# fferflo/semantic-meshes

Measured on AMD Instinct MI355X. Metric: views/sec fused (1080p, 19 classes, 1M-tri mesh), higher is better.
Workload: dtype f32; 1 GPU; cfg2: 1000000-triangle grid mesh, 11763 views/GPU at 1920x1080, 19 classes, probs resident in HBM; views_per_call=8, group_pipeline=True, repeats=1, allreduce=none, exchange=allreduce, nranks=1, allreduce_bytes=0, exchange_parts=1, held_views=0

## Files before the change

semantic_meshes_amd/_lib.py:

```python
import ctypes
import os
import threading

_HERE = os.path.dirname(os.path.abspath(__file__))
LIB_PATH = os.environ.get("SMESH_LIB_PATH") or os.path.join(_HERE, "csrc", "libsmesh_hip.so")

OK, ERR_INVALID, ERR_RUNTIME, ERR_NODEVICE = 0, 1, 2, 3
MEM_HOST, MEM_DEVICE = 0, 1
IDX_U32, IDX_I32, IDX_U64, IDX_I64 = 0, 1, 2, 3
AGG_KINDS = {"Sum": 0, "Summax": 1, "Mul": 2}
PROF_FUSE_SCATTER, PROF_FUSE_HIST, PROF_RASTER, PROF_FINALIZE, PROF_EXCHANGE = 0, 1, 2, 3, 4

c_void_p, c_int, c_u64, c_u32, c_float = ctypes.c_void_p, ctypes.c_int, ctypes.c_uint64, ctypes.c_uint32, ctypes.c_float
P = ctypes.POINTER


class CameraPOD(ctypes.Structure):
    _fields_ = [
        ("rotation", ctypes.c_float * 9),
        ("translation", ctypes.c_float * 3),
        ("focal", ctypes.c_double * 2),
        ("principal", ctypes.c_double * 2),
        ("width", ctypes.c_uint64),
        ("height", ctypes.c_uint64),
    ]


SIGNATURES = {
    "smesh_backend": (ctypes.c_char_p, []),
    "smesh_last_error": (ctypes.c_char_p, []),
    "smesh_device_count": (c_int, [P(c_int)]),
    "smesh_synchronize": (c_int, [c_int]),
    "smesh_stream_wait": (c_int, [c_int, c_void_p]),
    "smesh_stream_release": (c_int, [c_int, c_void_p]),
    "smesh_stream_handle": (c_int, [c_int, P(c_void_p)]),
    "smesh_token_record": (c_int, [c_int, P(c_u64)]),
    "smesh_token_done": (c_int, [c_int, c_u64, P(c_int)]),
    "smesh_stream_mark": (c_int, [c_int, c_int]),
    "smesh_stream_mark_elapsed": (c_int, [c_int, c_int, c_int, P(ctypes.c_double)]),
    "smesh_renderer_create_triangles": (c_int, [c_void_p, c_u64, c_void_p, c_u64, c_int, P(c_void_p)]),
    "smesh_renderer_create_texels": (c_int, [c_void_p, c_u64, c_void_p, c_u64, c_void_p, c_u64, c_float, c_int, P(c_void_p)]),
    "smesh_renderer_destroy": (c_int, [c_void_p]),
    "smesh_renderer_num_primitives": (c_int, [c_void_p, P(c_u64)]),
    "smesh_renderer_texel_layout": (c_int, [c_void_p, c_void_p, c_void_p, c_void_p]),
    "smesh_renderer_render": (c_int, [c_void_p, P(CameraPOD), c_void_p, c_void_p]),
    "smesh_renderer_render_device": (c_int, [c_void_p, P(CameraPOD), P(c_void_p), P(c_void_p)]),
    "smesh_renderer_release_image": (c_int, [c_void_p, c_void_p, c_void_p]),
    "smesh_aggregator_create": (c_int, [c_u64, c_u32, c_int, c_float, c_int, P(c_void_p)]),
    "smesh_aggregator_destroy": (c_int, [c_void_p]),
    "smesh_aggregator_reset": (c_int, [c_void_p]),
    "smesh_aggregator_add": (c_int, [c_void_p, c_void_p, c_int, P(ctypes.c_int64), c_int,
                                     c_void_p, P(ctypes.c_int64), c_int,
                                     c_void_p, P(ctypes.c_int64), c_int, c_u64, c_u64]),
    "smesh_aggregator_add_async": (c_int, [c_void_p, c_void_p, c_int, P(ctypes.c_int64), c_int,
                                           c_void_p, P(ctypes.c_int64), c_int,
                                           c_void_p, P(ctypes.c_int64), c_int, c_u64, c_u64]),
    "smesh_aggregator_add_many": (c_int, [c_void_p, c_u64, P(c_void_p), c_int, P(ctypes.c_int64), c_int,
                                          P(c_void_p), P(ctypes.c_int64), c_int,
                                          P(c_void_p), P(ctypes.c_int64), c_int, c_u64, c_u64]),
    "smesh_aggregator_add_rendered": (c_int, [c_void_p, c_void_p, c_void_p,
                                              c_void_p, P(ctypes.c_int64), c_int,
                                              c_void_p, P(ctypes.c_int64), c_int, c_u64, c_u64]),
    "smesh_aggregator_get": (c_int, [c_void_p, c_void_p, c_int]),
    "smesh_aggregator_get_rows": (c_int, [c_void_p, c_u64, c_u64, c_void_p, c_int]),
    "smesh_aggregator_get_raw": (c_int, [c_void_p, c_void_p, c_int]),
    "smesh_aggregator_set_raw": (c_int, [c_void_p, c_void_p, c_int]),
    "smesh_aggregator_raw_pointer": (c_int, [c_void_p, P(c_void_p), P(c_u64)]),
    "smesh_aggregator_row_stride": (c_int, [c_void_p, P(c_u32)]),
    "smesh_comm_unique_id": (c_int, [c_void_p]),
    "smesh_comm_create": (c_int, [c_int, c_int, c_int, c_void_p, P(c_void_p)]),
    "smesh_comm_create_all": (c_int, [P(c_int), c_int, P(c_void_p)]),
    "smesh_comm_destroy": (c_int, [c_void_p]),
    "smesh_comm_rank": (c_int, [c_void_p, P(c_int), P(c_int)]),
    "smesh_allreduce": (c_int, [P(c_void_p), P(c_void_p), c_int]),
    "smesh_reduce_scatter": (c_int, [c_void_p, c_void_p, P(c_u64), P(c_u64)]),
    "smesh_fuse_views_begin": (c_int, [c_void_p, c_void_p, c_void_p, c_u64, P(c_void_p), P(c_void_p), c_int, c_int, P(c_u64), P(c_u64)]),
    "smesh_fuse_views_continue": (c_int, [c_void_p, c_void_p, c_int, P(c_u64), P(c_u64)]),
    "smesh_allreduce_rows": (c_int, [c_void_p, c_void_p, c_u64, c_u64]),
    "smesh_exchange_join": (c_int, [c_void_p]),
    "smesh_aggregator_get_raw_rows": (c_int, [c_void_p, c_u64, c_u64, c_int, c_void_p, c_int]),
    "smesh_aggregator_set_raw_rows": (c_int, [c_void_p, c_u64, c_u64, c_int, c_void_p, c_int]),
    "smesh_comm_allreduce_f64": (c_int, [c_void_p, P(ctypes.c_double), c_int, c_int]),
    "smesh_aggregator_renderer": (c_int, [c_void_p, P(c_void_p)]),
    "smesh_annotation_renderer_render": (c_int, [c_void_p, c_void_p, c_int, P(ctypes.c_int64), c_int, c_void_p, c_void_p, c_int, c_u64, c_u64]),
    "smesh_annotation_renderer_destroy": (c_int, [c_void_p]),
    "smesh_fuse_view": (c_int, [c_void_p, c_void_p, P(CameraPOD), c_void_p, c_void_p, c_int]),
    "smesh_fuse_views": (c_int, [c_void_p, c_void_p, P(CameraPOD), c_u64, P(c_void_p), P(c_void_p), c_int]),
    "smesh_aggregator_add_matched": (c_int, [c_void_p, c_void_p, c_void_p, c_int, P(ctypes.c_int64), c_int,
                                             c_void_p, P(ctypes.c_int64), c_int,
                                             c_void_p, P(ctypes.c_int64), c_int, c_u64, c_u64, P(c_int)]),
    "smesh_renderer_seal_render": (c_int, [c_void_p, c_void_p]),
    "smesh_renderer_render_stats": (c_int, [c_void_p, c_void_p, c_void_p, c_void_p]),
    "smesh_box_extent_bound": (c_int, [c_void_p, c_u64, c_void_p, c_u64, c_void_p, c_void_p]),
    "smesh_last_fuse_kernel": (ctypes.c_char_p, []),
    "smesh_last_add_path": (ctypes.c_char_p, []),
    "smesh_profile_enable": (c_int, [c_int, c_int]),
    "smesh_profile_sample_every": (c_int, [c_int, ctypes.c_uint32]),
    "smesh_profile_read": (c_int, [c_int, c_int, P(ctypes.c_double), P(c_u64)]),
    "smesh_profile_read_ex": (c_int, [c_int, c_int, P(ctypes.c_double), P(c_u64), P(c_u64), P(c_u64)]),
    "smesh_profile_regions": (c_int, [c_int, c_int, P(c_u64)]),
    "smesh_profile_reset": (c_int, [c_int]),
    "smesh_synth_probs": (c_int, [c_void_p, c_u64, c_u32, c_u64, c_float, c_int, c_int]),
    "smesh_device_malloc": (c_int, [c_int, c_u64, P(c_void_p)]),
    "smesh_device_free": (c_int, [c_int, c_void_p]),
    "smesh_device_trim": (c_int, [c_int, P(c_u64)]),
    "smesh_set_option": (c_int, [ctypes.c_char_p, ctypes.c_int64]),
    "smesh_get_option": (c_int, [ctypes.c_char_p, P(ctypes.c_int64)]),
    "smesh_host_malloc": (c_int, [c_u64, P(c_void_p)]),
    "smesh_host_free": (c_int, [c_void_p]),
    "smesh_memcpy": (c_int, [c_void_p, c_void_p, c_u64, c_int, c_int, c_int]),
}

LBL_CODES = {"uint8": 0, "int8": 1, "uint16": 2, "int16": 3, "uint32": 4, "int32": 5, "uint64": 6, "int64": 7}

VTX_SUMS, VTX_ANNOTATIONS = 0, 1

EXT_SIGNATURES = {
    "smesh_fuse_view_labels": (c_int, [c_void_p, c_void_p, P(CameraPOD), c_void_p, c_int, P(ctypes.c_int64), c_void_p, c_int]),
    "smesh_fuse_views_labels": (c_int, [c_void_p, c_void_p, P(CameraPOD), c_u64, P(c_void_p), c_int, P(ctypes.c_int64), P(c_void_p), c_int]),
    "smesh_aggregator_add_labels": (c_int, [c_void_p, c_void_p, c_void_p, c_int, P(ctypes.c_int64), c_int,
                                            c_void_p, c_int, P(ctypes.c_int64), c_int,
                                            c_void_p, P(ctypes.c_int64), c_int, c_u64, c_u64]),
}

VERTEX_SIGNATURES = {
    "smesh_vertex_map_create": (c_int, [c_void_p, c_u64, c_u64, c_int, P(c_void_p)]),
    "smesh_vertex_map_destroy": (c_int, [c_void_p]),
    "smesh_vertex_map_size": (c_int, [c_void_p, P(c_u64), P(c_u64), P(c_u64)]),
    "smesh_vertex_map_adjacency": (c_int, [c_void_p, c_void_p, c_void_p]),
    "smesh_vertex_map_gather": (c_int, [c_void_p, c_void_p, c_int, c_u32, c_int, c_float, c_void_p, c_void_p, c_int]),
    "smesh_aggregator_vertex_annotations": (c_int, [c_void_p, c_void_p, c_int, c_float, c_void_p, c_void_p, c_int]),
    "smesh_renderer_texel_face_rows": (c_int, [c_void_p, c_void_p, c_int, c_u32, c_int, c_float, c_void_p, c_int]),
}

PROF_CONFUSION = 5
EVAL_SIGNATURES = {
    "smesh_confusion_create": (c_int, [c_u32, c_int, P(c_void_p)]),
    "smesh_confusion_destroy": (c_int, [c_void_p]),
    "smesh_confusion_reset": (c_int, [c_void_p]),
    "smesh_confusion_get": (c_int, [c_void_p, c_void_p, P(c_u64)]),
    "smesh_confusion_add_counts": (c_int, [c_void_p, c_void_p, c_u64]),
    "smesh_confusion_add_labels": (c_int, [c_void_p, c_void_p, c_int, c_void_p, c_int, c_int, c_u64]),
    "smesh_aggregator_labels": (c_int, [c_void_p, c_float, c_void_p, c_int]),
    "smesh_confusion_add_image": (c_int, [c_void_p, c_void_p, c_int, P(ctypes.c_int64), c_int, c_void_p, c_u64, c_int,
                                          c_void_p, c_int, P(ctypes.c_int64), c_int, c_u64, c_u64]),
    "smesh_confusion_add_view": (c_int, [c_void_p, c_void_p, P(CameraPOD), c_void_p, c_u64, c_void_p, c_int, P(ctypes.c_int64), c_int]),
    "smesh_confusion_add_views": (c_int, [c_void_p, c_void_p, P(CameraPOD), c_u64, c_void_p, c_u64, P(c_void_p), c_int,
                                          P(ctypes.c_int64), c_int]),
}

PROF_LABEL_IMAGES = 6
LAYOUT_WH, LAYOUT_HW = 0, 1
LABEL_IMAGE_SIGNATURES = {
    "smesh_label_renderer_create": (c_int, [c_void_p, c_u64, c_int, c_u32, c_int, c_u32, c_void_p, c_void_p, c_int, P(c_void_p)]),
    "smesh_label_renderer_destroy": (c_int, [c_void_p]),
    "smesh_label_renderer_render_image": (c_int, [c_void_p, c_void_p, c_int, P(ctypes.c_int64), c_int, c_u64, c_u64, c_int,
                                                  c_void_p, c_void_p, c_int]),
    "smesh_label_renderer_render_views": (c_int, [c_void_p, c_void_p, P(CameraPOD), c_u64, c_int, P(c_void_p), P(c_void_p), c_int]),
}

_lib = None
_lock = threading.Lock()


def _elf_dynamic_strings(path):
    import struct
    with open(path, "rb") as f:
        data = f.read()
    try:
        if data[:6] != b"\x7fELF\x02\x01":
            raise ValueError("not a little-endian ELF64 file")
        phoff, = struct.unpack_from("<Q", data, 0x20)
        phentsize, phnum = struct.unpack_from("<HH", data, 0x36)
        loads, dyn = [], None
        for k in range(phnum):
            typ, flags, off, vaddr, paddr, filesz, memsz, align = struct.unpack_from("<IIQQQQQQ", data, phoff + k * phentsize)
            if typ == 1:
                loads.append((vaddr, off, filesz))
            elif typ == 2:
                dyn = (off, filesz)
        if dyn is None:
            return None, []
        entries = []
        for e in range(dyn[0], dyn[0] + dyn[1], 16):
            tag, val = struct.unpack_from("<qQ", data, e)
            if tag == 0:
                break
            entries.append((tag, val))
        strtab = next((v for t, v in entries if t == 5), None)
        if strtab is None:
            return None, []
        stroff = next((off + strtab - vaddr for vaddr, off, filesz in loads if vaddr <= strtab < vaddr + filesz), None)
        if stroff is None:
            raise ValueError("DT_STRTAB outside every PT_LOAD segment")

        def cstr(o):
            end = data.index(b"\0", stroff + o)
            return data[stroff + o:end].decode()

        soname, needed = None, []
        for tag, val in entries:
            if tag == 1:
                needed.append(cstr(val))
            elif tag == 14:
                soname = cstr(val)
        return soname, needed
    except (struct.error, IndexError, UnicodeDecodeError) as e:
        raise ValueError("malformed ELF file %s: %s" % (path, e))


def _preload_note(msg):
    global PRELOAD_NOTE
    PRELOAD_NOTE = msg
    if os.environ.get("SMESH_DEBUG"):
        import sys
        print("semantic_meshes_amd: " + msg, file=sys.stderr)


PRELOAD_NOTE = None


def _preload_hip_runtime():
    import importlib.util
    import sys
    choice = os.environ.get("SMESH_HIP_RUNTIME", "auto")
    if choice == "system" or "torch" in sys.modules:
        return
    libdir = choice if choice not in ("auto", "torch") else None
    if libdir is None:
        try:
            spec = importlib.util.find_spec("torch")
        except (ImportError, ValueError):
            spec = None
        if spec is None or not spec.origin:
            return
        libdir = os.path.join(os.path.dirname(spec.origin), "lib")
    hip = os.path.join(libdir, "libamdhip64.so")
    if not os.path.exists(hip):
        return
    try:
        wanted = [n for n in _elf_dynamic_strings(LIB_PATH)[1] if n.startswith("libamdhip64.so")]
        offered = _elf_dynamic_strings(hip)[0]
    except (OSError, ValueError) as e:
        _preload_note("HIP runtime preload skipped: %s" % e)
        return
    if not wanted or offered != wanted[0]:
        _preload_note("HIP runtime preload skipped: %s offers SONAME %r, libsmesh_hip.so needs %r" % (hip, offered, wanted[:1]))
        return
    for name in ("libhsa-runtime64.so", "libamdhip64.so"):
        path = os.path.join(libdir, name)
        if os.path.exists(path):
            try:
                ctypes.CDLL(path, mode=ctypes.RTLD_GLOBAL)
            except OSError:
                return
    rccl = os.path.join(libdir, "librccl.so")
    if os.path.exists(rccl):
        os.environ.setdefault("SMESH_RCCL_LIB", rccl)


def lib():
    global _lib
    if _lib is None:
        with _lock:
            if _lib is None:
                if not os.path.exists(LIB_PATH):
                    raise RuntimeError(
                        "semantic_meshes_amd: %s not found -- build it with `make -C semantic_meshes_amd/csrc` "
                        "(or `python -c 'import __graft_entry__ as g; g.build()'`). There is no CPU fallback." % LIB_PATH)
                _preload_hip_runtime()
                L = ctypes.CDLL(LIB_PATH)
                for name, (res, args) in list(SIGNATURES.items()) + list(EXT_SIGNATURES.items()) + list(VERTEX_SIGNATURES.items()) + list(EVAL_SIGNATURES.items()) + list(LABEL_IMAGE_SIGNATURES.items()):
                    fn = getattr(L, name)
                    fn.restype = res
                    fn.argtypes = args
                _lib = L
    return _lib


def check(status):
    if status == OK:
        return
    msg = lib().smesh_last_error().decode(errors="replace")
    if status == ERR_INVALID:
        raise ValueError(msg)
    raise RuntimeError(msg)


def device_count():
    n = c_int(0)
    check(lib().smesh_device_count(ctypes.byref(n)))
    return n.value


_flush_hooks = []


def flush_pending(device=None):
    for hook in list(_flush_hooks):
        hook(device)


def last_fuse_kernel():
    flush_pending()
    return lib().smesh_last_fuse_kernel().decode()


def last_add_path():
    flush_pending()
    return lib().smesh_last_add_path().decode()


def synchronize(device=0):
    flush_pending(device)
    check(lib().smesh_synchronize(device))
```

semantic_meshes_amd/csrc/common.hpp:

```cpp
#pragma once

#include <hip/hip_runtime.h>

#include <cstdint>
#include <cstdio>
#include <cstdlib>
#include <functional>
#include <mutex>
#include <string>
#include <vector>

#include "../../include/smesh.h"

namespace smesh {

int fail(int code, const std::string& msg);
int fail_hip(hipError_t e, const char* what, const char* file, int line);

#define SMESH_HIP(expr)                                                         \
  do {                                                                          \
    hipError_t _e = (expr);                                                     \
    if (_e != hipSuccess) return ::smesh::fail_hip(_e, #expr, __FILE__, __LINE__); \
  } while (0)

#define SMESH_TRY(expr)              \
  do {                               \
    int _s = (expr);                 \
    if (_s != SMESH_OK) return _s;   \
  } while (0)

struct ProfSlot {
  std::vector<std::pair<hipEvent_t, hipEvent_t>> pending;
  std::vector<std::pair<hipEvent_t, hipEvent_t>> pool;
  double total_ms = 0.0;
  uint64_t launches = 0;
  uint64_t seen = 0;
  int depth = 0;
  bool open_timed = false;
  uint64_t timed_launches = 0;
  uint64_t timed_views = 0;
};

struct DeviceCtx {
  int device = -1;
  hipStream_t stream = nullptr;
  hipStream_t raster_stream = nullptr;
  hipStream_t exchange_stream = nullptr;
  hipEvent_t ev_order = nullptr;
  hipEvent_t ev_release = nullptr;
  int num_cus = 256;
  unsigned profiling = 0;
  unsigned profile_every = 1;
  ProfSlot slots[SMESH_PROF_SLOTS];
  hipEvent_t marks[SMESH_STREAM_MARKS] = {};
  std::vector<hipEvent_t> token_pool;
  std::recursive_mutex mu;
};

int get_ctx(int device, DeviceCtx** out);

struct ProfScope {
  DeviceCtx* ctx;
  int slot;
  hipEvent_t start = nullptr, stop = nullptr;
  hipStream_t st;
  bool counted = false;
  ProfScope(DeviceCtx* c, int s, hipStream_t stream = nullptr);
  ~ProfScope();
};

void prof_note(DeviceCtx* ctx, int slot, uint64_t launches, uint64_t views);

hipError_t dev_malloc(void** out, size_t bytes);
hipError_t dev_free(void* p, bool foreign = false);
uint64_t dev_cached_bytes(int device);
void dev_trim(int device);
void dev_cache_stats(uint64_t* live_blocks, uint64_t* cached_blocks, uint64_t* cached_bytes);

bool opt_group_pipeline();
bool opt_confusion_wave_aggregate();

constexpr uint32_t kConfusionLdsMaxC = 180;

struct Scratch {
  void* ptr = nullptr;
  size_t bytes = 0;
  int reserve(size_t need);
  void release();
};

inline uint64_t div_up(uint64_t a, uint64_t b) { return (a + b - 1) / b; }

inline int env_int(const char* name, int def) {
  const char* e = getenv(name);
  return e ? atoi(e) : def;
}

struct TriFrag {
  uint16_t x0, y0;
  uint16_t kind;
  uint16_t pad;
  unsigned long long mask;
};
static_assert(sizeof(TriFrag) == 16, "TriFrag must be 16 bytes");

struct TriFuseArgs {
  const TriFrag* frags;
  const uint32_t* idx;
  const float* probs;
  const float* weights;
  float* acc;
  float* acc_lo;
  uint64_t F;
  uint32_t C, W, H;
  float iew;
  const uint32_t* big_queue;
  const uint32_t* big_len;
  uint32_t big_capacity;
  uint32_t tri_blocks;
  uint32_t big_blocks;
  const uint32_t* prim_id;
  const uint32_t* tex_first;
  const uint32_t* tex_res;
  const uint8_t* tex_kinds;
  uint32_t* count;
  double* acc_d;
  int mid;
  uint32_t ps0, ps1;
  uint32_t blk_first;
  uint32_t f_lo, f_hi;
  uint32_t lds_pad;
};

struct TriView {
  const TriFrag* frags;
  const uint32_t* idx;
  const float* probs;
  const float* weights;
  const uint32_t* big_queue;
  const uint32_t* big_len;
  uint32_t W, H;
  uint32_t ps0, ps1;
  const uint8_t* kinds;
};
template <int NV>
struct TriViews {
  TriView v[NV];
};

struct RenderedView {
  const TriFrag* frags;
  const uint32_t* big_queue;
  const uint32_t* big_len;
  const uint32_t* idx;
  const float* probs;
  const float* weights;
  uint64_t W, H;
  int64_t ps0 = 0, ps1 = 0;
  bool mid_queue = false;
  bool no_big = false;
  const uint8_t* kinds = nullptr;
  bool fine = false;
  const void* labels = nullptr;
};

constexpr int kMidBox = 256;

struct ImageRecords {
  TriFrag* frags = nullptr;
  uint32_t* cand = nullptr;
  uint4* big4 = nullptr;
  uint32_t* big_queue = nullptr;
  uint32_t* big_count = nullptr;
  unsigned long long* mom = nullptr;
  uint64_t P = 0;
  bool clean = false;
  bool moments = false;
  uint32_t tag = 2;
  void release();
};
int image_records_build(DeviceCtx* ctx, ImageRecords& r, const uint32_t* d_idx, uint64_t W, uint64_t H, uint64_t P);
int image_records_pending(DeviceCtx* ctx, ImageRecords& r, const uint32_t* d_idx, uint64_t W, uint64_t H, hipStream_t st);
int image_records_scatter_sparse(DeviceCtx* ctx, ImageRecords& r, int kind, const uint32_t* d_idx, const float* d_probs, const float* d_w,
                                 uint64_t W, uint64_t H, uint32_t C, float iew, float* acc, float* acc_lo, double* acc_d, hipStream_t st);
int image_records_clear(DeviceCtx* ctx, ImageRecords& r, const uint32_t* d_idx, uint64_t W, uint64_t H, hipStream_t st);
bool image_records_build_group(DeviceCtx* ctx, ImageRecords* const* recs, const uint32_t* const* d_idx, int n, uint64_t W, uint64_t H, uint64_t P,
                               int* status);
int image_records_scatter_sparse_group(DeviceCtx* ctx, ImageRecords* const* recs, int n, int kind, const uint32_t* const* d_idx,
                                       const float* const* d_probs, const float* const* d_w, uint64_t W, uint64_t H, uint32_t C, float iew,
                                       float* acc, float* acc_lo, double* acc_d, hipStream_t st);

}

struct smesh_aggregator;
struct smesh_renderer;
int smesh_aggregator_with_final_rows(smesh_aggregator* a,
                                     const std::function<int(smesh::DeviceCtx* ctx, const float* rows, uint64_t P, uint32_t C)>& use);
int smesh_renderer_texel_tables(const smesh_renderer* r, smesh::DeviceCtx** ctx, uint64_t* F, uint64_t* P, const uint32_t** first,
                                const uint32_t** res);
int smesh_rows_labels(smesh::DeviceCtx* ctx, const float* d_rows, uint64_t n, uint32_t C, float dont_care_threshold, int32_t* out_labels,
                      int out_memkind);
int smesh_renderer_with_index_planes(smesh_renderer* r, const smesh_camera_t* cams, int n, uint64_t P, smesh::DeviceCtx* ctx,
                                     const std::function<int(int view, const uint32_t* idx, uint64_t W, uint64_t H)>& use);
```

semantic_meshes_amd/csrc/context.cpp:

```cpp
#include "common.hpp"
#include "labels_scratch.hpp"

#include <algorithm>
#include <atomic>

#include <cstdlib>
#include <cstring>
#include <map>
#include <memory>
#include <unordered_map>
#include <vector>

namespace smesh {

static thread_local std::string g_err;

int fail(int code, const std::string& msg) {
  g_err = msg;
  return code;
}

int fail_hip(hipError_t e, const char* what, const char* file, int line) {
  char buf[512];
  snprintf(buf, sizeof buf, "HIP error %d (%s) at %s:%d: %s", (int)e, hipGetErrorString(e), file, line, what);
  g_err = buf;
  (void)hipGetLastError();
  return (e == hipErrorNoDevice || e == hipErrorInvalidDevice) ? SMESH_ERR_NODEVICE : SMESH_ERR_RUNTIME;
}

static std::atomic<int> g_confusion_wave_aggregate{1};
bool opt_confusion_wave_aggregate() { return g_confusion_wave_aggregate.load() != 0; }

static std::atomic<int> g_group_pipeline{-1};
bool opt_group_pipeline() {
  int v = g_group_pipeline.load();
  if (v < 0) {
    const char* e = getenv("SMESH_GROUP_PIPELINE");
    v = e ? (atoi(e) != 0 ? 1 : 0) : 1;
    g_group_pipeline.store(v);
  }
  return v != 0;
}

static std::mutex g_ctx_mu;
static std::vector<std::unique_ptr<DeviceCtx>> g_ctx;

DeviceCtx* peek_ctx(int device) {
  std::lock_guard<std::mutex> lock(g_ctx_mu);
  return (device >= 0 && device < (int)g_ctx.size()) ? g_ctx[device].get() : nullptr;
}

int get_ctx(int device, DeviceCtx** out) {
  std::lock_guard<std::mutex> lock(g_ctx_mu);
  int n = 0;
  hipError_t e = hipGetDeviceCount(&n);
  if (e != hipSuccess || n <= 0) {
    (void)hipGetLastError();
    return fail(SMESH_ERR_NODEVICE, "no HIP device available (libsmesh_hip has no CPU fallback)");
  }
  if (device < 0 || device >= n) return fail(SMESH_ERR_INVALID, "device index out of range");
  if ((int)g_ctx.size() < n) g_ctx.resize(n);
  if (!g_ctx[device]) {
    SMESH_HIP(hipSetDevice(device));
    auto ctx = std::make_unique<DeviceCtx>();
    ctx->device = device;
    hipDeviceProp_t prop;
    SMESH_HIP(hipGetDeviceProperties(&prop, device));
    ctx->num_cus = prop.multiProcessorCount > 0 ? prop.multiProcessorCount : 256;
    SMESH_HIP(hipStreamCreateWithFlags(&ctx->stream, hipStreamNonBlocking));
    SMESH_HIP(hipStreamCreateWithFlags(&ctx->raster_stream, hipStreamNonBlocking));
    {
      int least = 0, greatest = 0;
      if (hipDeviceGetStreamPriorityRange(&least, &greatest) != hipSuccess) { (void)hipGetLastError(); least = greatest = 0; }
      if (hipStreamCreateWithPriority(&ctx->exchange_stream, hipStreamNonBlocking, greatest) != hipSuccess) {
        (void)hipGetLastError();
        SMESH_HIP(hipStreamCreateWithFlags(&ctx->exchange_stream, hipStreamNonBlocking));
      }
    }
    g_ctx[device] = std::move(ctx);
  }
  *out = g_ctx[device].get();
  return SMESH_OK;
}

ProfScope::ProfScope(DeviceCtx* c, int s, hipStream_t stream) : ctx(c), slot(s), st(stream ? stream : c->stream) {
  if (!(ctx->profiling & (1u << slot))) return;
  ProfSlot& ps = ctx->slots[slot];
  if (ps.depth++ > 0) { counted = true; return; }
  counted = true;
  if (ps.seen++ % (slot <= SMESH_PROF_RASTER ? std::max(1u, ctx->profile_every) : 1u) != 0) return;
  if (!ps.pool.empty()) {
    start = ps.pool.back().first;
    stop = ps.pool.back().second;
    ps.pool.pop_back();
  } else {
    if (hipEventCreate(&start) != hipSuccess || hipEventCreate(&stop) != hipSuccess) {
      start = stop = nullptr;
      return;
    }
  }
  (void)hipEventRecord(start, st);
  ps.open_timed = true;
}

void prof_note(DeviceCtx* ctx, int slot, uint64_t launches, uint64_t views) {
  ProfSlot& ps = ctx->slots[slot];
  if (ps.depth > 0 && ps.open_timed) { ps.timed_launches += launches; ps.timed_views += views; }
}

ProfScope::~ProfScope() {
  if (counted && --ctx->slots[slot].depth == 0 && !start) ctx->slots[slot].open_timed = false;
  if (!start) return;
  ctx->slots[slot].open_timed = false;
  (void)hipEventRecord(stop, st);
  ctx->slots[slot].pending.emplace_back(start, stop);
}

namespace {
struct DevBlock { int device; size_t bytes; };
struct CachedBlock { void* ptr; int device; unsigned long long stamp; };
std::mutex g_alloc_mu;
std::unordered_map<void*, DevBlock> g_live;
std::multimap<size_t, CachedBlock> g_cached;
std::map<int, size_t> g_cached_bytes;
unsigned long long g_alloc_stamp = 0;

size_t size_class(size_t n) {
  if (n == 0) n = 1;
  const size_t g = n <= (1u << 20) ? (size_t)4096 : (size_t)2 << 20;
  return (n + g - 1) / g * g;
}
size_t cache_cap(int device) {
  static std::map<int, size_t> caps;
  auto it = caps.find(device);
  if (it != caps.end()) return it->second;
  size_t cap;
  if (const char* e = getenv("SMESH_ALLOC_CACHE_MB")) cap = (size_t)std::max(0ll, atoll(e)) << 20;
  else {
    int cur = 0;
    (void)hipGetDevice(&cur);
    if (cur != device) (void)hipSetDevice(device);
    size_t free_b = 0, total = 0;
    if (hipMemGetInfo(&free_b, &total) != hipSuccess) { (void)hipGetLastError(); total = (size_t)64 << 30; }
    if (cur != device) (void)hipSetDevice(cur);
    cap = std::min<size_t>(total / 16, (size_t)8 << 30);
  }
  caps[device] = cap;
  return cap;
}
void really_free_locked(std::multimap<size_t, CachedBlock>::iterator it) {
  int cur = 0;
  (void)hipGetDevice(&cur);
  if (cur != it->second.device) (void)hipSetDevice(it->second.device);
  (void)hipFree(it->second.ptr);
  if (cur != it->second.device) (void)hipSetDevice(cur);
  g_cached_bytes[it->second.device] -= it->first;
  g_cached.erase(it);
}
void evict_locked(int device, size_t need, size_t cap) {
  for (;;) {
    size_t held = 0;
    if (device >= 0) held = g_cached_bytes[device];
    else for (auto& kv : g_cached_bytes) held += kv.second;
    if (held == 0 || held + need <= cap) return;
    auto oldest = g_cached.end();
    for (auto it = g_cached.begin(); it != g_cached.end(); ++it)
      if ((device < 0 || it->second.device == device) && (oldest == g_cached.end() || it->second.stamp < oldest->second.stamp)) oldest = it;
    if (oldest == g_cached.end()) return;
    really_free_locked(oldest);
  }
}
}

hipError_t dev_malloc(void** out, size_t bytes) {
  *out = nullptr;
  int dev = 0;
  hipError_t e = hipGetDevice(&dev);
  if (e != hipSuccess) return e;
  const size_t sz = size_class(bytes);
  std::lock_guard<std::mutex> lock(g_alloc_mu);
  for (auto it = g_cached.lower_bound(sz); it != g_cached.end() && it->first <= sz + sz / 8; ++it) {
    if (it->second.device != dev) continue;
    *out = it->second.ptr;
    g_live[*out] = DevBlock{dev, it->first};
    g_cached_bytes[dev] -= it->first;
    g_cached.erase(it);
    return hipSuccess;
  }
  e = hipMalloc(out, sz);
  if (e != hipSuccess) {
    (void)hipGetLastError();
    evict_locked(dev, 0, 0);
    e = hipMalloc(out, sz);
  }
  if (e == hipSuccess) g_live[*out] = DevBlock{dev, sz};
  return e;
}

hipError_t dev_free(void* p, bool foreign) {
  if (!p) return hipSuccess;
  int owner = -1;
  {
    std::lock_guard<std::mutex> lock(g_alloc_mu);
    auto it = g_live.find(p);
    if (it != g_live.end()) owner = it->second.device;
  }
  int cur = 0;
  (void)hipGetDevice(&cur);
  if (owner >= 0 && owner != cur) (void)hipSetDevice(owner);
  DeviceCtx* ctx = (owner >= 0 && !foreign) ? peek_ctx(owner) : nullptr;
  hipError_t e = hipSuccess;
  if (ctx) {
    for (hipStream_t st : {ctx->raster_stream, ctx->stream, ctx->exchange_stream})
      if (st && e == hipSuccess) e = hipStreamSynchronize(st);
  } else {
    e = hipDeviceSynchronize();
  }
  if (e != hipSuccess) (void)hipGetLastError();
  hipError_t ret = hipSuccess;
  {
    std::lock_guard<std::mutex> lock(g_alloc_mu);
    auto it = g_live.find(p);
    if (it == g_live.end()) ret = hipFree(p);
    else {
      const DevBlock b = it->second;
      g_live.erase(it);
      const size_t cap = cache_cap(b.device);
      if (b.bytes > cap) ret = hipFree(p);
      else {
        evict_locked(b.device, b.bytes, cap);
        g_cached.emplace(b.bytes, CachedBlock{p, b.device, g_alloc_stamp++});
        g_cached_bytes[b.device] += b.bytes;
      }
    }
  }
  if (owner >= 0 && owner != cur) (void)hipSetDevice(cur);
  return ret;
}

void dev_trim(int device) {
  std::lock_guard<std::mutex> lock(g_alloc_mu);
  for (auto it = g_cached.begin(); it != g_cached.end();) {
    if (device >= 0 && it->second.device != device) { ++it; continue; }
    auto victim = it++;
    really_free_locked(victim);
  }
}

void dev_cache_stats(uint64_t* live_blocks, uint64_t* cached_blocks, uint64_t* cached_bytes) {
  std::lock_guard<std::mutex> lock(g_alloc_mu);
  if (live_blocks) *live_blocks = g_live.size();
  if (cached_blocks) *cached_blocks = g_cached.size();
  if (cached_bytes) { *cached_bytes = 0; for (auto& kv : g_cached_bytes) *cached_bytes += kv.second; }
}
uint64_t dev_cached_bytes(int device) {
  std::lock_guard<std::mutex> lock(g_alloc_mu);
  uint64_t n = 0;
  for (auto& kv : g_cached_bytes) if (device < 0 || kv.first == device) n += kv.second;
  return n;
}

int Scratch::reserve(size_t need) {
  if (need <= bytes) return SMESH_OK;
  if (ptr) SMESH_HIP(dev_free(ptr));
  ptr = nullptr;
  bytes = 0;
  size_t want = need + need / 8 + 256;
  SMESH_HIP(dev_malloc(&ptr, want));
  bytes = want;
  return SMESH_OK;
}

void Scratch::release() {
  if (ptr) (void)dev_free(ptr);
  ptr = nullptr;
  bytes = 0;
}

}

using namespace smesh;

void smesh_last_fuse_instance(int* slot, int* views);

extern "C" {

const char* smesh_backend(void) { return "hip-gfx950"; }

const char* smesh_last_error(void) { return g_err.c_str(); }

int smesh_set_option(const char* name, int64_t value) {
  if (!name) return fail(SMESH_ERR_INVALID, "option name is NULL");
  if (!strcmp(name, "group_pipeline")) { g_group_pipeline.store(value != 0 ? 1 : 0); return SMESH_OK; }
  if (!strcmp(name, "confusion_wave_aggregate")) { g_confusion_wave_aggregate.store(value != 0 ? 1 : 0); return SMESH_OK; }
  return fail(SMESH_ERR_INVALID, std::string("unknown option: ") + name);
}
int smesh_get_option(const char* name, int64_t* value) {
  if (!name || !value) return fail(SMESH_ERR_INVALID, "NULL argument");
  if (!strcmp(name, "group_pipeline")) { *value = opt_group_pipeline() ? 1 : 0; return SMESH_OK; }
  if (!strcmp(name, "labels_lds_max_classes")) { *value = (int64_t)kLabelsLdsMaxC; return SMESH_OK; }
  if (!strcmp(name, "confusion_lds_max_classes")) { *value = (int64_t)kConfusionLdsMaxC; return SMESH_OK; }
  if (!strcmp(name, "confusion_wave_aggregate")) { *value = opt_confusion_wave_aggregate() ? 1 : 0; return SMESH_OK; }
  const bool want_slot = !strcmp(name, "last_fuse_slot");
  if (want_slot || !strcmp(name, "last_fuse_views")) {
    int slot, views;
    smesh_last_fuse_instance(&slot, &views);
    *value = want_slot ? slot : views;
    return SMESH_OK;
  }
  return fail(SMESH_ERR_INVALID, std::string("unknown option: ") + name);
}

int smesh_device_count(int* count) {
  if (!count) return fail(SMESH_ERR_INVALID, "count is NULL");
  int n = 0;
  if (hipGetDeviceCount(&n) != hipSuccess) {
    (void)hipGetLastError();
    n = 0;
  }
  *count = n;
  return SMESH_OK;
}

int smesh_synchronize(int device) {
  DeviceCtx* ctx;
  SMESH_TRY(get_ctx(device, &ctx));
  SMESH_HIP(hipSetDevice(device));
  SMESH_HIP(hipStreamSynchronize(ctx->raster_stream));
  SMESH_HIP(hipStreamSynchronize(ctx->stream));
  SMESH_HIP(hipStreamSynchronize(ctx->exchange_stream));
  return SMESH_OK;
}

int smesh_stream_wait(int device, void* producer_stream) {
  DeviceCtx* ctx;
  SMESH_TRY(get_ctx(device, &ctx));
  std::lock_guard<std::recursive_mutex> lock(ctx->mu);
  SMESH_HIP(hipSetDevice(device));
  hipStream_t ps = static_cast<hipStream_t>(producer_stream);
  if (ps == ctx->raster_stream) return SMESH_OK;
  if (!ctx->ev_order) SMESH_HIP(hipEventCreateWithFlags(&ctx->ev_order, hipEventDisableTiming));
  SMESH_HIP(hipEventRecord(ctx->ev_order, ps));
  if (ps != ctx->stream) SMESH_HIP(hipStreamWaitEvent(ctx->stream, ctx->ev_order, 0));
  SMESH_HIP(hipStreamWaitEvent(ctx->raster_stream, ctx->ev_order, 0));
  return SMESH_OK;
}

int smesh_stream_release(int device, void* consumer_stream) {
  DeviceCtx* ctx;
  SMESH_TRY(get_ctx(device, &ctx));
  std::lock_guard<std::recursive_mutex> lock(ctx->mu);
  SMESH_HIP(hipSetDevice(device));
  hipStream_t cs = static_cast<hipStream_t>(consumer_stream);
  if (cs == ctx->stream) return SMESH_OK;
  if (!ctx->ev_release) SMESH_HIP(hipEventCreateWithFlags(&ctx->ev_release, hipEventDisableTiming));
  SMESH_HIP(hipEventRecord(ctx->ev_release, ctx->stream));
  SMESH_HIP(hipStreamWaitEvent(cs, ctx->ev_release, 0));
  return SMESH_OK;
}

int smesh_stream_handle(int device, void** stream) {
  if (!stream) return fail(SMESH_ERR_INVALID, "stream is NULL");
  DeviceCtx* ctx;
  SMESH_TRY(get_ctx(device, &ctx));
  *stream = ctx->stream;
  return SMESH_OK;
}

int smesh_stream_mark(int device, int id) {
  if (id < 0 || id >= SMESH_STREAM_MARKS) return fail(SMESH_ERR_INVALID, "bad mark id");
  DeviceCtx* ctx;
  SMESH_TRY(get_ctx(device, &ctx));
  std::lock_guard<std::recursive_mutex> lock(ctx->mu);
  SMESH_HIP(hipSetDevice(device));
  if (!ctx->marks[id]) SMESH_HIP(hipEventCreate(&ctx->marks[id]));
  SMESH_HIP(hipEventRecord(ctx->marks[id], ctx->stream));
  return SMESH_OK;
}

int smesh_stream_mark_elapsed(int device, int from, int to, double* ms) {
  if (from < 0 || from >= SMESH_STREAM_MARKS || to < 0 || to >= SMESH_STREAM_MARKS || !ms) return fail(SMESH_ERR_INVALID, "bad mark id");
  DeviceCtx* ctx;
  SMESH_TRY(get_ctx(device, &ctx));
  hipEvent_t a, b;
  {
    std::lock_guard<std::recursive_mutex> lock(ctx->mu);
    a = ctx->marks[from];
    b = ctx->marks[to];
  }
  if (!a || !b) return fail(SMESH_ERR_INVALID, "mark was never recorded");
  SMESH_HIP(hipSetDevice(device));
  SMESH_HIP(hipEventSynchronize(b));
  float f = 0.f;
  SMESH_HIP(hipEventElapsedTime(&f, a, b));
  *ms = (double)f;
  return SMESH_OK;
}

int smesh_token_record(int device, uint64_t* token) {
  if (!token) return fail(SMESH_ERR_INVALID, "token is NULL");
  *token = 0;
  DeviceCtx* ctx;
  SMESH_TRY(get_ctx(device, &ctx));
  std::lock_guard<std::recursive_mutex> lock(ctx->mu);
  SMESH_HIP(hipSetDevice(device));
  hipEvent_t ev = nullptr;
  if (!ctx->token_pool.empty()) { ev = ctx->token_pool.back(); ctx->token_pool.pop_back(); }
  else SMESH_HIP(hipEventCreateWithFlags(&ev, hipEventDisableTiming));
  SMESH_HIP(hipEventRecord(ev, ctx->stream));
  *token = (uint64_t)reinterpret_cast<uintptr_t>(ev);
  return SMESH_OK;
}

int smesh_token_done(int device, uint64_t token, int* done) {
  if (!done) return fail(SMESH_ERR_INVALID, "done is NULL");
  *done = 1;
  if (!token) return SMESH_OK;
  DeviceCtx* ctx;
  SMESH_TRY(get_ctx(device, &ctx));
  std::lock_guard<std::recursive_mutex> lock(ctx->mu);
  hipEvent_t ev = reinterpret_cast<hipEvent_t>((uintptr_t)token);
  const hipError_t e = hipEventQuery(ev);
  if (e == hipErrorNotReady) { (void)hipGetLastError(); *done = 0; return SMESH_OK; }
  if (e != hipSuccess) return fail_hip(e, "hipEventQuery", __FILE__, __LINE__);
  ctx->token_pool.push_back(ev);
  return SMESH_OK;
}

int smesh_profile_enable(int device, int enabled) {
  DeviceCtx* ctx;
  SMESH_TRY(get_ctx(device, &ctx));
  std::lock_guard<std::recursive_mutex> lock(ctx->mu);
  ctx->profiling = enabled < 0 ? 0xFFu : (unsigned)enabled;
  return SMESH_OK;
}

int smesh_profile_sample_every(int device, uint32_t n) {
  DeviceCtx* ctx;
  SMESH_TRY(get_ctx(device, &ctx));
  std::lock_guard<std::recursive_mutex> lock(ctx->mu);
  ctx->profile_every = n ? n : 1u;
  return SMESH_OK;
}

static int drain(DeviceCtx* ctx) {
  SMESH_HIP(hipSetDevice(ctx->device));
  SMESH_HIP(hipStreamSynchronize(ctx->raster_stream));
  SMESH_HIP(hipStreamSynchronize(ctx->stream));
  SMESH_HIP(hipStreamSynchronize(ctx->exchange_stream));
  for (auto& ps : ctx->slots) {
    for (auto& ev : ps.pending) {
      float ms = 0.f;
      if (hipEventElapsedTime(&ms, ev.first, ev.second) == hipSuccess) {
        ps.total_ms += ms;
        ps.launches += 1;
      }
      ps.pool.push_back(ev);
    }
    ps.pending.clear();
  }
  return SMESH_OK;
}

int smesh_profile_read(int device, int slot, double* total_ms, uint64_t* launches) {
  if (slot < 0 || slot >= SMESH_PROF_SLOTS) return fail(SMESH_ERR_INVALID, "bad profile slot");
  DeviceCtx* ctx;
  SMESH_TRY(get_ctx(device, &ctx));
  std::lock_guard<std::recursive_mutex> lock(ctx->mu);
  SMESH_TRY(drain(ctx));
  if (total_ms) *total_ms = ctx->slots[slot].total_ms;
  if (launches) *launches = ctx->slots[slot].launches;
  return SMESH_OK;
}

int smesh_profile_read_ex(int device, int slot, double* total_ms, uint64_t* regions, uint64_t* launches, uint64_t* views) {
  if (slot < 0 || slot >= SMESH_PROF_SLOTS) return fail(SMESH_ERR_INVALID, "bad profile slot");
  DeviceCtx* ctx;
  SMESH_TRY(get_ctx(device, &ctx));
  std::lock_guard<std::recursive_mutex> lock(ctx->mu);
  SMESH_TRY(drain(ctx));
  const ProfSlot& ps = ctx->slots[slot];
  if (total_ms) *total_ms = ps.total_ms;
  if (regions) *regions = ps.launches;
  if (launches) *launches = ps.timed_launches;
  if (views) *views = ps.timed_views;
  return SMESH_OK;
}

int smesh_profile_regions(int device, int slot, uint64_t* entered) {
  if (slot < 0 || slot >= SMESH_PROF_SLOTS) return fail(SMESH_ERR_INVALID, "bad profile slot");
  DeviceCtx* ctx;
  SMESH_TRY(get_ctx(device, &ctx));
  std::lock_guard<std::recursive_mutex> lock(ctx->mu);
  if (entered) *entered = ctx->slots[slot].seen;
  return SMESH_OK;
}

int smesh_profile_reset(int device) {
  DeviceCtx* ctx;
  SMESH_TRY(get_ctx(device, &ctx));
  std::lock_guard<std::recursive_mutex> lock(ctx->mu);
  SMESH_TRY(drain(ctx));
  for (auto& ps : ctx->slots) {
    ps.total_ms = 0.0;
    ps.launches = 0;
    ps.seen = 0;
    ps.timed_launches = 0;
    ps.timed_views = 0;
  }
  return SMESH_OK;
}

int smesh_device_malloc(int device, uint64_t bytes, void** out) {
  if (!out) return fail(SMESH_ERR_INVALID, "out is NULL");
  DeviceCtx* ctx;
  SMESH_TRY(get_ctx(device, &ctx));
  SMESH_HIP(hipSetDevice(device));
  SMESH_HIP(dev_malloc(out, bytes ? bytes : 1));
  return SMESH_OK;
}

int smesh_device_free(int device, void* ptr) {
  if (!ptr) return SMESH_OK;
  DeviceCtx* ctx;
  SMESH_TRY(get_ctx(device, &ctx));
  SMESH_HIP(hipSetDevice(device));
  SMESH_HIP(dev_free(ptr, true));
  return SMESH_OK;
}

int smesh_device_trim(int device, uint64_t* cached_bytes) {
  if (cached_bytes) *cached_bytes = dev_cached_bytes(device);
  if (device >= 0) {
    DeviceCtx* ctx;
    SMESH_TRY(get_ctx(device, &ctx));
    SMESH_HIP(hipSetDevice(device));
  }
  (void)hipDeviceSynchronize();
  dev_trim(device);
  return SMESH_OK;
}

int smesh_host_malloc(uint64_t bytes, void** out) {
  if (!out) return fail(SMESH_ERR_INVALID, "out is NULL");
  DeviceCtx* ctx;
  SMESH_TRY(get_ctx(0, &ctx));
  SMESH_HIP(hipHostMalloc(out, bytes ? bytes : 1, hipHostMallocDefault));
  return SMESH_OK;
}

int smesh_host_free(void* ptr) {
  if (!ptr) return SMESH_OK;
  SMESH_HIP(hipHostFree(ptr));
  return SMESH_OK;
}

int smesh_memcpy(void* dst, const void* src, uint64_t bytes, int dst_memkind, int src_memkind, int device) {
  if (bytes == 0) return SMESH_OK;
  if (!dst || !src) return fail(SMESH_ERR_INVALID, "NULL pointer");
  if (dst_memkind == SMESH_MEM_HOST && src_memkind == SMESH_MEM_HOST) {
    memmove(dst, src, bytes);
    return SMESH_OK;
  }
  DeviceCtx* ctx;
  SMESH_TRY(get_ctx(device, &ctx));
  std::lock_guard<std::recursive_mutex> lock(ctx->mu);
  SMESH_HIP(hipSetDevice(device));
  hipMemcpyKind kind = dst_memkind == SMESH_MEM_HOST ? hipMemcpyDeviceToHost
                       : (src_memkind == SMESH_MEM_HOST ? hipMemcpyHostToDevice : hipMemcpyDeviceToDevice);
  SMESH_HIP(hipMemcpyAsync(dst, src, bytes, kind, ctx->stream));
  SMESH_HIP(hipStreamSynchronize(ctx->stream));
  return SMESH_OK;
}

}
```

semantic_meshes_amd/csrc/raster.hip:

```cpp
#include "common.hpp"

#include <algorithm>
#include <cmath>
#include <cstdlib>
#include <cstring>
#include <new>
#include <string>
#include <utility>
#include <vector>

#pragma clang fp contract(off)

using namespace smesh;

struct smesh_aggregator;
int smesh_aggregator_add_device_contig(smesh_aggregator* a, const uint32_t* d_idx, const float* d_probs,
                                       const float* d_w, uint64_t W, uint64_t H);
bool smesh_aggregator_can_fuse_triangles(smesh_aggregator* a, uint64_t F);
bool smesh_aggregator_can_fuse_pair(smesh_aggregator* a);
int smesh_aggregator_max_fused_views(smesh_aggregator* a);
bool smesh_aggregator_takes_strided_probs(smesh_aggregator* a, int64_t ps0, int64_t ps1, int nviews);
int smesh_aggregator_dense_probs(smesh_aggregator* a, const float* d_probs, const int64_t ps[3], uint64_t W, uint64_t H, const float** out);
bool smesh_aggregator_fuses_small_views_by_mask(smesh_aggregator* a);
int smesh_aggregator_fuse_triangles(smesh_aggregator* a, uint64_t F, const uint32_t* prim_id, uint32_t big_capacity,
                                    const RenderedView* views, int nviews, int part = 0, int nparts = 1);
void smesh_fuse_part_rows(uint64_t F, int part, int nparts, uint64_t* f_lo, uint64_t* f_hi);
uint64_t smesh_aggregator_primitives(smesh_aggregator* a);
int smesh_aggregator_join_exchange(smesh_aggregator* a);
const char* smesh_aggregator_fuse_kernel_name(smesh_aggregator* a, bool reordered);
bool smesh_aggregator_can_fuse_texels(smesh_aggregator* a, uint64_t P);
int smesh_aggregator_fuse_texels(smesh_aggregator* a, const TriFrag* frags, const uint8_t* kinds, uint64_t F, const uint32_t* tex_first,
                                 const uint32_t* tex_res, const uint32_t* big_queue, const uint32_t* big_len,
                                 uint32_t big_capacity, const uint32_t* d_idx, const float* d_probs, const float* d_w, uint64_t H);
int smesh_aggregator_fuse_texels_multi(smesh_aggregator* a, uint64_t F, const uint32_t* tex_first, const uint32_t* tex_res, uint32_t big_capacity,
                                       const RenderedView* views, int nviews);
DeviceCtx* smesh_aggregator_ctx(smesh_aggregator* a);
uint32_t smesh_aggregator_classes(smesh_aggregator* a);
std::mutex& smesh_aggregator_mutex(smesh_aggregator* a);
Scratch& smesh_aggregator_stage_probs(smesh_aggregator* a);
Scratch& smesh_aggregator_stage_w(smesh_aggregator* a);
bool smesh_labels_native(smesh_aggregator* a, uint64_t F, uint64_t N);
int smesh_labels_fuse_triangles(smesh_aggregator* a, uint64_t F, uint32_t big_capacity, const RenderedView* views, int nviews, int label_bytes);
int smesh_labels_expand(smesh_aggregator* a, const void* plane, int label_bytes, uint64_t N, const float** probs);

namespace {

constexpr float kNear = 1e-6f;
constexpr unsigned long long kBackgroundKey = (0x7F800000ull << 32) | 0xFFFFFFFFull;

struct ScreenVertex {
  double u, v;
  double iz;
};
constexpr double kBehind = -1.0;

struct CameraArgs {
  float R[9];
  float t[3];
  double fx, fy, cx, cy;
  uint32_t W, H;
};

__device__ __forceinline__ ScreenVertex project_point(const CameraArgs& cam, const float X, const float Y, const float Z) {
  const float xc = ((cam.R[0] * X + cam.R[1] * Y) + cam.R[2] * Z) + cam.t[0];
  const float yc = ((cam.R[3] * X + cam.R[4] * Y) + cam.R[5] * Z) + cam.t[1];
  const float zc = ((cam.R[6] * X + cam.R[7] * Y) + cam.R[8] * Z) + cam.t[2];
  ScreenVertex s;
  s.u = 0.0; s.v = 0.0; s.iz = 0.0;
  const bool fin = isfinite(xc) && isfinite(yc) && isfinite(zc);
  if (zc > kNear && fin) {
    const double zd = (double)zc;
    const double u = cam.fx * ((double)xc / zd) + cam.cx;
    const double v = cam.fy * ((double)yc / zd) + cam.cy;
    if (isfinite(u) && isfinite(v)) {
      s.u = u; s.v = v; s.iz = 1.0 / zd;
    }
  } else if (fin) {
    s.iz = kBehind;
  }
  return s;
}

__device__ __forceinline__ void project_vertex(const float* __restrict__ verts, uint64_t V, const CameraArgs& cam,
                                               ScreenVertex* __restrict__ sv, uint32_t* __restrict__ big_count, const uint64_t i) {
  if (i == 0) { big_count[0] = 0u; big_count[1] = 0u; big_count[2] = 0u; big_count[3] = 0u; big_count[4] = 0u; big_count[5] = 0u; }
  if (i >= V) return;
  sv[i] = project_point(cam, verts[3 * i + 0], verts[3 * i + 1], verts[3 * i + 2]);
}

__global__ void k_project_vertices(const float* __restrict__ verts, uint64_t V, CameraArgs cam,
                                   ScreenVertex* __restrict__ sv, uint32_t* __restrict__ big_count) {
  project_vertex(verts, V, cam, sv, big_count, (uint64_t)blockIdx.x * blockDim.x + threadIdx.x);
}

constexpr int kMaxGroup = 8;
struct ProjectGroup {
  const float* verts;
  uint64_t V;
  CameraArgs cam[kMaxGroup];
  ScreenVertex* sv[kMaxGroup];
  uint32_t* big_count[kMaxGroup];
  uint32_t n;
};
__global__ void k_project_vertices_group(ProjectGroup g) {
  const uint64_t i = (uint64_t)blockIdx.x * blockDim.x + threadIdx.x;
  if (i == 0)
    for (uint32_t v = 0; v < g.n; v++)
      for (int k = 0; k < 6; k++) g.big_count[v][k] = 0u;
  if (i >= g.V) return;
  const float X = g.verts[3 * i + 0], Y = g.verts[3 * i + 1], Z = g.verts[3 * i + 2];
  for (uint32_t v = 0; v < g.n; v++) g.sv[v][i] = project_point(g.cam[v], X, Y, Z);
}

struct EdgeEq {
  double A, B, C;
};

__device__ __forceinline__ EdgeEq make_edge(double ax, double ay, double bx, double by) {
  EdgeEq e;
  const bool sw = (bx < ax) || (bx == ax && by < ay);
  const double lx = sw ? bx : ax, ly = sw ? by : ay;
  e.A = ay - by;
  e.B = bx - ax;
  const double c0 = e.B * ly;
  e.C = __builtin_fma(-e.A, lx, -c0);
  return e;
}

__device__ __forceinline__ double eval_edge(const EdgeEq& e, double px, double py) {
  return __builtin_fma(e.A, px, __builtin_fma(e.B, py, e.C));
}

__device__ __forceinline__ void flip_edge(EdgeEq& e) { e.A = -e.A; e.B = -e.B; e.C = -e.C; }

struct Tri {
  EdgeEq e0, e1, e2;
  int cls0, cls1, cls2;
  double iz0, iz1, iz2;
  int x0, x1, y0, y1;
};

__device__ __forceinline__ bool owns(const EdgeEq& e) { return e.A > 0.0 || (e.A == 0.0 && e.B > 0.0); }
constexpr int kClsPositive = 0x380, kClsZero = 0x060;
__device__ __forceinline__ int edge_classes(const EdgeEq& e) { return owns(e) ? (kClsPositive | kClsZero) : kClsPositive; }
__device__ __forceinline__ bool edge_accepts(double w, int cls) { return __builtin_amdgcn_class(w, cls); }

__device__ __forceinline__ bool setup_tri(const ScreenVertex& a, const ScreenVertex& b, const ScreenVertex& c,
                                          uint32_t W, uint32_t H, Tri& t) {
  if (!(a.iz > 0.0) || !(b.iz > 0.0) || !(c.iz > 0.0)) return false;
  const double minu = fmin(a.u, fmin(b.u, c.u)), maxu = fmax(a.u, fmax(b.u, c.u));
  const double minv = fmin(a.v, fmin(b.v, c.v)), maxv = fmax(a.v, fmax(b.v, c.v));
  t.x0 = max((int)ceil(minu - 0.5), 0); t.x1 = min((int)floor(maxu - 0.5), (int)W - 1);
  t.y0 = max((int)ceil(minv - 0.5), 0); t.y1 = min((int)floor(maxv - 0.5), (int)H - 1);
  if (t.x0 > t.x1 || t.y0 > t.y1) return false;
  t.e0 = make_edge(b.u, b.v, c.u, c.v);
  t.e1 = make_edge(c.u, c.v, a.u, a.v);
  t.e2 = make_edge(a.u, a.v, b.u, b.v);
  const double area2 = eval_edge(t.e2, c.u, c.v);
  if (!(area2 != 0.0) || !isfinite(area2)) return false;
  if (area2 < 0.0) { flip_edge(t.e0); flip_edge(t.e1); flip_edge(t.e2); }
  t.cls0 = edge_classes(t.e0);
  t.cls1 = edge_classes(t.e1);
  t.cls2 = edge_classes(t.e2);
  t.iz0 = a.iz; t.iz1 = b.iz; t.iz2 = c.iz;
  return true;
}

struct Shaded { bool ok; float z; double b1, b2; };
__device__ __forceinline__ Shaded shade(const Tri& t, int x, int y, bool want_bary) {
  Shaded r; r.ok = false; r.z = 0.0f; r.b1 = 0.0; r.b2 = 0.0;
  const double px = (double)x + 0.5, py = (double)y + 0.5;
  const double w0 = eval_edge(t.e0, px, py);
  if (!edge_accepts(w0, t.cls0)) return r;
  const double w1 = eval_edge(t.e1, px, py);
  if (!edge_accepts(w1, t.cls1)) return r;
  const double w2 = eval_edge(t.e2, px, py);
  if (!edge_accepts(w2, t.cls2)) return r;
  const double num = (w0 + w1) + w2;
  const double den = __builtin_fma(w2, t.iz2, __builtin_fma(w1, t.iz1, w0 * t.iz0));
  const float zf = (float)(num / den);
  if (!(zf > 0.0f) || !isfinite(zf)) return r;
  r.ok = true; r.z = zf;
  if (want_bary) { r.b1 = w1 / num; r.b2 = w2 / num; }
  return r;
}

__device__ __forceinline__ bool covered(const Tri& t, int x, int y) {
  const double px = (double)x + 0.5, py = (double)y + 0.5;
  const double w0 = eval_edge(t.e0, px, py);
  if (!edge_accepts(w0, t.cls0)) return false;
  const double w1 = eval_edge(t.e1, px, py);
  if (!edge_accepts(w1, t.cls1)) return false;
  const double w2 = eval_edge(t.e2, px, py);
  return edge_accepts(w2, t.cls2);
}

__device__ __forceinline__ uint32_t texel_of(uint32_t res, double b1, double b2) {
  const float u = (float)b1, v = (float)b2;
  const float fu = (u - 1e-6f) * (float)res, fv = (v - 1e-6f) * (float)res;
  int tu = (int)fu, tv = (int)fv;
  if (tu < 0) tu = 0;
  if (tv < 0) tv = 0;
  const int r1 = (int)res - 1;
  if (tu > r1) tu = r1;
  if (tv > r1 - tu) tv = r1 - tu;
  const int row = tu + tv;
  return (uint32_t)(row * (row + 1) / 2 + tu);
}

constexpr int kQW = 32, kQH = 64, kQPixels = kQW * kQH;
constexpr int kQSub = 4;
constexpr int kMedium = 64;
constexpr unsigned long long kNullKey = ~0ull;

struct FragQueues {
  unsigned long long* key = nullptr;
  uint16_t* pix = nullptr;
  uint32_t* count = nullptr;
  uint32_t* flag = nullptr;
  uint32_t cap = 0, tiles_y = 0;
};

struct RasterArgs {
  const int32_t* faces;
  const float* verts;
  CameraArgs cam;
  const ScreenVertex* sv;
  const uint32_t* prim_id;
  const uint32_t* tex_res;
  const uint32_t* tex_first;
  unsigned long long* keys;
  uint64_t F, V;
  uint32_t W, H;
  uint32_t* big_queue;
  uint32_t* huge_queue;
  uint32_t* big_count;
  uint32_t big_capacity;
  TriFrag* frags;
  uint8_t* kinds;
  FragQueues q;
  uint32_t tpw;
  uint32_t groups;
  uint32_t* med_queue;
  uint32_t balance;
  uint32_t wg_push;
  uint32_t spread;
  uint32_t idx_optional;
};

__device__ __forceinline__ uint64_t key_index(uint32_t x, uint32_t y, uint32_t H) { return (uint64_t)x * H + y; }

__device__ __forceinline__ bool load_tri(const RasterArgs& a, uint64_t f, Tri& t, const int32_t i0, const int32_t i1, const int32_t i2);
__device__ __forceinline__ bool load_tri(const RasterArgs& a, uint64_t f, Tri& t) {
  return load_tri(a, f, t, a.faces[3 * f + 0], a.faces[3 * f + 1], a.faces[3 * f + 2]);
}
__device__ __forceinline__ bool load_tri(const RasterArgs& a, uint64_t f, Tri& t, const int32_t i0, const int32_t i1, const int32_t i2) {
  if ((uint64_t)max((uint32_t)i0, max((uint32_t)i1, (uint32_t)i2)) >= a.V) return false;
  if (a.tex_res && a.tex_res[f] == 0) return false;
  const ScreenVertex va = a.sv[i0], vb = a.sv[i1], vc = a.sv[i2];
  return setup_tri(va, vb, vc, a.W, a.H, t);
}

struct CamPoint { float x, y, z; };
__device__ __forceinline__ CamPoint camera_point(const CameraArgs& cam, const float* __restrict__ verts, const int32_t i) {
  const float X = verts[3 * (uint64_t)i + 0], Y = verts[3 * (uint64_t)i + 1], Z = verts[3 * (uint64_t)i + 2];
  CamPoint c;
  c.x = ((cam.R[0] * X + cam.R[1] * Y) + cam.R[2] * Z) + cam.t[0];
  c.y = ((cam.R[3] * X + cam.R[4] * Y) + cam.R[5] * Z) + cam.t[1];
  c.z = ((cam.R[6] * X + cam.R[7] * Y) + cam.R[8] * Z) + cam.t[2];
  return c;
}
struct ClipVertex { ScreenVertex s; double b1, b2; };
__device__ __forceinline__ bool clip_edge(const CameraArgs& cam, const CamPoint& F, const double fb1, const double fb2,
                                          const CamPoint& B, const double bb1, const double bb2, ClipVertex& out) {
  const double zn = (double)kNear;
  const double t = ((double)F.z - zn) / ((double)F.z - (double)B.z);
  const double x = __builtin_fma(t, (double)B.x - (double)F.x, (double)F.x);
  const double y = __builtin_fma(t, (double)B.y - (double)F.y, (double)F.y);
  const double u = cam.fx * (x / zn) + cam.cx;
  const double v = cam.fy * (y / zn) + cam.cy;
  out.s.u = u; out.s.v = v; out.s.iz = 1.0 / zn;
  out.b1 = __builtin_fma(t, bb1 - fb1, fb1);
  out.b2 = __builtin_fma(t, bb2 - fb2, fb2);
  return isfinite(u) && isfinite(v);
}

__device__ __forceinline__ int clip_class(const ScreenVertex& va, const ScreenVertex& vb, const ScreenVertex& vc) {
  if (va.iz == 0.0 || vb.iz == 0.0 || vc.iz == 0.0) return -1;
  const int nfront = (va.iz > 0.0 ? 1 : 0) + (vb.iz > 0.0 ? 1 : 0) + (vc.iz > 0.0 ? 1 : 0);
  return nfront == 3 ? 0 : (nfront == 0 ? -1 : nfront);
}

__device__ __forceinline__ bool clip_piece(const RasterArgs& a, const int32_t i0, const int32_t i1, const int32_t i2,
                                           const ScreenVertex& va, const ScreenVertex& vb, const ScreenVertex& vc,
                                           const int nfront, const int p, ClipVertex& q0, ClipVertex& q1, ClipVertex& q2) {
  if (nfront == 1 && p != 0) return false;
  const int k = nfront == 1 ? (va.iz > 0.0 ? 0 : (vb.iz > 0.0 ? 1 : 2)) : (!(va.iz > 0.0) ? 0 : (!(vb.iz > 0.0) ? 1 : 2));
  const int32_t is = k == 0 ? i0 : (k == 1 ? i1 : i2), in = k == 0 ? i1 : (k == 1 ? i2 : i0), ip = k == 0 ? i2 : (k == 1 ? i0 : i1);
  const CamPoint cs = camera_point(a.cam, a.verts, is), cn = camera_point(a.cam, a.verts, in), cp = camera_point(a.cam, a.verts, ip);
  const double s1 = k == 1 ? 1.0 : 0.0, s2 = k == 2 ? 1.0 : 0.0;
  const double n1 = k == 0 ? 1.0 : 0.0, n2 = k == 1 ? 1.0 : 0.0;
  const double p1 = k == 2 ? 1.0 : 0.0, p2 = k == 0 ? 1.0 : 0.0;
  const ScreenVertex& ss = k == 0 ? va : (k == 1 ? vb : vc);
  const ScreenVertex& sn = k == 0 ? vb : (k == 1 ? vc : va);
  const ScreenVertex& sp = k == 0 ? vc : (k == 1 ? va : vb);
  if (nfront == 1) {
    q0.s = ss; q0.b1 = s1; q0.b2 = s2;
    const bool ok1 = clip_edge(a.cam, cs, s1, s2, cn, n1, n2, q1);
    const bool ok2 = clip_edge(a.cam, cs, s1, s2, cp, p1, p2, q2);
    return ok1 && ok2;
  }
  ClipVertex inb, ipb;
  const bool ok1 = clip_edge(a.cam, cn, n1, n2, cs, s1, s2, inb);
  const bool ok2 = clip_edge(a.cam, cp, p1, p2, cs, s1, s2, ipb);
  if (!ok1 || !ok2) return false;
  q0.s = sn; q0.b1 = n1; q0.b2 = n2;
  if (p == 0) { q1.s = sp; q1.b1 = p1; q1.b2 = p2; q2 = ipb; }
  else        { q1 = ipb; q2 = inb; }
  return true;
}

__device__ __forceinline__ bool clip_bbox(const RasterArgs& a, const int32_t i0, const int32_t i1, const int32_t i2,
                                          const ScreenVertex& va, const ScreenVertex& vb, const ScreenVertex& vc, const int nfront,
                                          int& x0, int& y0, int& x1, int& y1) {
  ClipVertex q0, q1, q2;
  if (!clip_piece(a, i0, i1, i2, va, vb, vc, nfront, nfront == 2 ? 1 : 0, q0, q1, q2)) return false;
  double minu = fmin(q0.s.u, fmin(q1.s.u, q2.s.u)), maxu = fmax(q0.s.u, fmax(q1.s.u, q2.s.u));
  double minv = fmin(q0.s.v, fmin(q1.s.v, q2.s.v)), maxv = fmax(q0.s.v, fmax(q1.s.v, q2.s.v));
  if (nfront == 2) {
    const int k = !(va.iz > 0.0) ? 0 : (!(vb.iz > 0.0) ? 1 : 2);
    const ScreenVertex& sp = k == 0 ? vc : (k == 1 ? va : vb);
    minu = fmin(minu, sp.u); maxu = fmax(maxu, sp.u); minv = fmin(minv, sp.v); maxv = fmax(maxv, sp.v);
  }
  x0 = max((int)ceil(minu - 0.5), 0); x1 = min((int)floor(maxu - 0.5), (int)a.W - 1);
  y0 = max((int)ceil(minv - 0.5), 0); y1 = min((int)floor(maxv - 0.5), (int)a.H - 1);
  return x0 <= x1 && y0 <= y1;
}

struct Piece {
  Tri t;
  double b1[3], b2[3];
  bool clipped;
};
__device__ __forceinline__ bool load_piece(const RasterArgs& a, const uint64_t f, const int p, Piece& pc) {
  const int32_t i0 = a.faces[3 * f + 0], i1 = a.faces[3 * f + 1], i2 = a.faces[3 * f + 2];
  if ((uint64_t)max((uint32_t)i0, max((uint32_t)i1, (uint32_t)i2)) >= a.V) return false;
  if (a.tex_res && a.tex_res[f] == 0) return false;
  const ScreenVertex va = a.sv[i0], vb = a.sv[i1], vc = a.sv[i2];
  const int cls = clip_class(va, vb, vc);
  pc.clipped = cls > 0;
  if (cls < 0) return false;
  if (cls == 0) return p == 0 && setup_tri(va, vb, vc, a.W, a.H, pc.t);
  ClipVertex q0, q1, q2;
  if (!clip_piece(a, i0, i1, i2, va, vb, vc, cls, p, q0, q1, q2)) return false;
  pc.b1[0] = q0.b1; pc.b1[1] = q1.b1; pc.b1[2] = q2.b1;
  pc.b2[0] = q0.b2; pc.b2[1] = q1.b2; pc.b2[2] = q2.b2;
  return setup_tri(q0.s, q1.s, q2.s, a.W, a.H, pc.t);
}

__device__ __forceinline__ unsigned long long shade_piece_key(const RasterArgs& a, const uint64_t f, const Piece& pc, const int x, const int y) {
  const Tri& t = pc.t;
  const double px = (double)x + 0.5, py = (double)y + 0.5;
  const double w0 = eval_edge(t.e0, px, py);
  if (!edge_accepts(w0, t.cls0)) return kNullKey;
  const double w1 = eval_edge(t.e1, px, py);
  if (!edge_accepts(w1, t.cls1)) return kNullKey;
  const double w2 = eval_edge(t.e2, px, py);
  if (!edge_accepts(w2, t.cls2)) return kNullKey;
  const double num = (w0 + w1) + w2;
  const double den = __builtin_fma(w2, t.iz2, __builtin_fma(w1, t.iz1, w0 * t.iz0));
  const float zf = (float)(num / den);
  if (!(zf > 0.0f) || !isfinite(zf)) return kNullKey;
  uint32_t prim = a.prim_id ? a.prim_id[f] : (uint32_t)f;
  if (a.tex_res) {
    double b1, b2;
    if (!pc.clipped) { b1 = w1 / num; b2 = w2 / num; }
    else {
      const double q0 = w0 * t.iz0, q1 = w1 * t.iz1, q2 = w2 * t.iz2;
      b1 = __builtin_fma(q2, pc.b1[2], __builtin_fma(q1, pc.b1[1], q0 * pc.b1[0])) / den;
      b2 = __builtin_fma(q2, pc.b2[2], __builtin_fma(q1, pc.b2[1], q0 * pc.b2[0])) / den;
    }
    prim = a.tex_first[f] + texel_of(a.tex_res[f], b1, b2);
  }
  return ((unsigned long long)__float_as_uint(zf) << 32) | prim;
}

__device__ __forceinline__ int load_tri_ex(const RasterArgs& a, uint64_t f, Tri& t, const int32_t i0, const int32_t i1, const int32_t i2) {
  if ((uint64_t)max((uint32_t)i0, max((uint32_t)i1, (uint32_t)i2)) >= a.V) return 0;
  if (a.tex_res && a.tex_res[f] == 0) return 0;
  const ScreenVertex va = a.sv[i0], vb = a.sv[i1], vc = a.sv[i2];
  const int cls = clip_class(va, vb, vc);
  if (cls == 0) return setup_tri(va, vb, vc, a.W, a.H, t) ? 1 : 0;
  if (cls < 0) return 0;
  return clip_bbox(a, i0, i1, i2, va, vb, vc, cls, t.x0, t.y0, t.x1, t.y1) ? 2 : 0;
}

__device__ __forceinline__ unsigned long long shade_key(const RasterArgs& a, uint64_t f, const Tri& t, int x, int y) {
  const Shaded sh = shade(t, x, y, a.tex_res != nullptr);
  if (!sh.ok) return kNullKey;
  uint32_t prim = a.prim_id ? a.prim_id[f] : (uint32_t)f;
  if (a.tex_res) prim = a.tex_first[f] + texel_of(a.tex_res[f], sh.b1, sh.b2);
  return ((unsigned long long)__float_as_uint(sh.z) << 32) | prim;
}

__device__ __forceinline__ void emit(const RasterArgs& a, uint64_t f, const Tri& t, int x, int y) {
  const unsigned long long key = shade_key(a, f, t, x, y);
  if (key == kNullKey) return;
  atomicMin(&a.keys[key_index((uint32_t)x, (uint32_t)y, a.H)], key);
}

__device__ __forceinline__ void push_mid(const RasterArgs& a, const uint64_t f, const int box_pixels) {
  if (box_pixels > kMidBox) return;
  const uint32_t slot = atomicAdd(a.big_count + 3, 1u);
  if (slot < a.big_capacity) a.big_queue[(uint64_t)a.big_capacity + slot] = (uint32_t)f;
}

__global__ void k_raster_small(RasterArgs a) {
  const uint64_t f = (uint64_t)blockIdx.x * blockDim.x + threadIdx.x;
  if (f >= a.F) return;
  TriFrag rec;
  rec.x0 = 0; rec.y0 = 0; rec.kind = 0; rec.pad = 0; rec.mask = 0ull;
  Tri t;
  const int have = load_tri_ex(a, f, t, a.faces[3 * f + 0], a.faces[3 * f + 1], a.faces[3 * f + 2]);
  if (have) {
    const int bw = t.x1 - t.x0 + 1, bh = t.y1 - t.y0 + 1;
    rec.x0 = (uint16_t)t.x0; rec.y0 = (uint16_t)t.y0;
    if (bw > 8 || bh > 8 || have == 2) {
      const uint32_t slot = atomicAdd(a.big_count, 1u);
      if (slot < a.big_capacity) a.big_queue[slot] = (uint32_t)f;
      push_mid(a, f, bw * bh);
      rec.kind = 2;
      rec.mask = (unsigned long long)(uint32_t)t.x1 | ((unsigned long long)(uint32_t)t.y1 << 16);
    } else {
      unsigned long long mask = 0ull;
      for (int dx = 0; dx < bw; dx++)
        for (int dy = 0; dy < bh; dy++) {
          const unsigned long long key = shade_key(a, f, t, t.x0 + dx, t.y0 + dy);
          if (key != kNullKey) {
            mask |= 1ull << (dx * 8 + dy);
            atomicMin(&a.keys[key_index((uint32_t)(t.x0 + dx), (uint32_t)(t.y0 + dy), a.H)], key);
          }
        }
      rec.kind = mask ? 1 : 0;
      rec.mask = mask;
    }
  }
  if (a.frags && (rec.kind != 0 || !a.kinds)) a.frags[f] = rec;
  if (a.kinds) a.kinds[f] = (uint8_t)rec.kind;
}

__global__ __launch_bounds__(256) void k_raster_big(RasterArgs a, uint32_t chunks_budget) {
  const uint32_t nbig = min(*a.big_count, a.big_capacity);
  for (uint32_t q = blockIdx.x; q < nbig; q += gridDim.x) {
    const uint64_t f = a.big_queue[q];
    for (int p = 0; p < 2; p++) {
      Piece pc;
      if (!load_piece(a, f, p, pc)) continue;
      const Tri& t = pc.t;
      const int bw = t.x1 - t.x0 + 1, bh = t.y1 - t.y0 + 1;
      const int ty = threadIdx.x & 63, tx = threadIdx.x >> 6;
      for (int cx = 0; cx < bw; cx += 4) {
        const int x = t.x0 + cx + tx;
        if (x > t.x1) continue;
        for (int cy = 0; cy < bh; cy += 64) {
          const int y = t.y0 + cy + ty;
          if (y > t.y1) continue;
          const unsigned long long key = shade_piece_key(a, f, pc, x, y);
          if (key != kNullKey) atomicMin(&a.keys[key_index((uint32_t)x, (uint32_t)y, a.H)], key);
        }
      }
    }
  }
  (void)chunks_budget;
}


__device__ __forceinline__ uint32_t wave_scan_incl(uint32_t v) {
  int s = (int)v;
  s += __builtin_amdgcn_update_dpp(0, s, 0x111, 0xF, 0xF, true);
  s += __builtin_amdgcn_update_dpp(0, s, 0x112, 0xF, 0xF, true);
  s += __builtin_amdgcn_update_dpp(0, s, 0x114, 0xF, 0xF, true);
  s += __builtin_amdgcn_update_dpp(0, s, 0x118, 0xF, 0xF, true);
  s += __builtin_amdgcn_update_dpp(0, s, 0x142, 0xA, 0xF, false);
  s += __builtin_amdgcn_update_dpp(0, s, 0x143, 0xC, 0xF, false);
  return (uint32_t)s;
}

struct Claim4 { uint32_t pre01, pre23, tot01, tot23; int leader; };
__device__ __forceinline__ Claim4 wave_claim_prepare4(uint32_t T0, uint32_t n01, uint32_t n23) {
  Claim4 c; c.pre01 = 0u; c.pre23 = 0u; c.tot01 = 0u; c.tot23 = 0u; c.leader = 0;
  const bool active = (n01 | n23) != 0u;
  unsigned long long todo = __ballot(active);
  while (todo) {
    const int first = __ffsll((long long)todo) - 1;
    const uint32_t t0 = (uint32_t)__builtin_amdgcn_readlane((int)T0, first);
    const bool in = active && T0 == t0;
    const unsigned long long same = __ballot(in);
    const uint32_t v01 = in ? n01 : 0u, v23 = in ? n23 : 0u;
    const uint32_t s01 = wave_scan_incl(v01), s23 = wave_scan_incl(v23);
    const uint32_t t01 = (uint32_t)__builtin_amdgcn_readlane((int)s01, 63), t23 = (uint32_t)__builtin_amdgcn_readlane((int)s23, 63);
    if (in) { c.pre01 = s01 - v01; c.pre23 = s23 - v23; c.tot01 = t01; c.tot23 = t23; c.leader = first; }
    todo &= ~same;
  }
  return c;
}

__device__ __forceinline__ unsigned long long walk_box(const Tri& t, const int X0, const int Y0, const int bw, const int bh) {
  unsigned long long cover = 0ull;
  const int area = bw * bh;
  int dx = 0, dy = 0;
  const double py0 = (double)Y0 + 0.5;
  double px = (double)X0 + 0.5, py = py0;
  for (int k = 0; k < area; k++) {
    const double w0 = eval_edge(t.e0, px, py);
    const double w1 = eval_edge(t.e1, px, py);
    const double w2 = eval_edge(t.e2, px, py);
    const bool in = edge_accepts(w0, t.cls0) && edge_accepts(w1, t.cls1) && edge_accepts(w2, t.cls2);
    if (in) cover |= 1ull << (dx * 8 + dy);
    py += 1.0;
    if (++dy == bh) { dy = 0; dx++; py = py0; px += 1.0; }
  }
  return cover;
}

template <bool TEX>
__device__ __forceinline__ unsigned long long emit_cover(const RasterArgs& a, const Tri& t, const uint64_t f, const uint32_t pid,
                                                         const int X0, const int Y0, unsigned long long cover, const uint32_t sub) {
  const int lane = threadIdx.x & 63;
  const uint32_t tx0 = (uint32_t)X0 / kQW, ty0 = (uint32_t)Y0 / kQH;
  const int bx = (int)(tx0 + 1) * kQW - X0, by = (int)(ty0 + 1) * kQH - Y0;
  const unsigned long long lox = bx >= 8 ? ~0ull : ((1ull << (8 * bx)) - 1ull);
  const unsigned long long loy = by >= 8 ? ~0ull : (0x0101010101010101ull * ((1ull << by) - 1ull));
  const uint32_t T0 = tx0 * a.q.tiles_y + ty0;
  const uint32_t n0 = (uint32_t)__popcll(cover & lox & loy), n1 = (uint32_t)__popcll(cover & ~lox & loy);
  const uint32_t n2 = (uint32_t)__popcll(cover & lox & ~loy), n3 = (uint32_t)__popcll(cover & ~lox & ~loy);
  const Claim4 c = wave_claim_prepare4(T0, n0 | (n1 << 16), n2 | (n3 << 16));
  const uint32_t tot0 = c.tot01 & 0xFFFFu, tot1 = c.tot01 >> 16, tot2 = c.tot23 & 0xFFFFu, tot3 = c.tot23 >> 16;
  uint32_t g0 = 0u, g1 = 0u, g2 = 0u, g3 = 0u;
  if (cover != 0ull && lane == c.leader) {
    if (tot0) g0 = atomicAdd(&a.q.count[T0 * kQSub + sub], tot0);
    if (tot1) g1 = atomicAdd(&a.q.count[(T0 + a.q.tiles_y) * kQSub + sub], tot1);
    if (tot2) g2 = atomicAdd(&a.q.count[(T0 + 1u) * kQSub + sub], tot2);
    if (tot3) g3 = atomicAdd(&a.q.count[(T0 + a.q.tiles_y + 1u) * kQSub + sub], tot3);
  }
  const uint32_t sq0 = (T0 * kQSub + sub) * a.q.cap, sq1 = ((T0 + a.q.tiles_y) * kQSub + sub) * a.q.cap,
                 sq2 = ((T0 + 1u) * kQSub + sub) * a.q.cap, sq3 = ((T0 + a.q.tiles_y + 1u) * kQSub + sub) * a.q.cap;
  uint32_t e0 = sq0 + (uint32_t)__shfl((int)g0, c.leader) + (c.pre01 & 0xFFFFu);
  uint32_t e1 = sq1 + (uint32_t)__shfl((int)g1, c.leader) + (c.pre01 >> 16);
  uint32_t e2 = sq2 + (uint32_t)__shfl((int)g2, c.leader) + (c.pre23 & 0xFFFFu);
  uint32_t e3 = sq3 + (uint32_t)__shfl((int)g3, c.leader) + (c.pre23 >> 16);
  unsigned long long mask = 0ull;
  for (unsigned long long m = cover; m; m &= m - 1ull) {
    const int bit = __ffsll((long long)m) - 1;
    const int dx = bit >> 3, dy = bit & 7;
    const int x = X0 + dx, y = Y0 + dy;
    const double px = (double)x + 0.5, py = (double)y + 0.5;
    const double w0 = eval_edge(t.e0, px, py);
    const double w1 = eval_edge(t.e1, px, py);
    const double w2 = eval_edge(t.e2, px, py);
    const double num = (w0 + w1) + w2;
    const double den = __builtin_fma(w2, t.iz2, __builtin_fma(w1, t.iz1, w0 * t.iz0));
    const float zf = (float)(num / den);
    unsigned long long key = kNullKey;
    if (zf > 0.0f && isfinite(zf)) {
      uint32_t prim = pid;
      if constexpr (TEX) prim = a.tex_first[f] + texel_of(a.tex_res[f], w1 / num, w2 / num);
      key = ((unsigned long long)__float_as_uint(zf) << 32) | prim;
      mask |= 1ull << bit;
    }
    const bool hx = dx >= bx, hy = dy >= by;
    const uint32_t e = hy ? (hx ? e3 : e2) : (hx ? e1 : e0);
    const uint32_t lim = (hy ? (hx ? sq3 : sq2) : (hx ? sq1 : sq0)) + a.q.cap;
    e0 += (!hx && !hy) ? 1u : 0u; e1 += (hx && !hy) ? 1u : 0u; e2 += (!hx && hy) ? 1u : 0u; e3 += (hx && hy) ? 1u : 0u;
    const uint16_t pin = (uint16_t)((((uint32_t)x & (kQW - 1)) * kQH) | ((uint32_t)y & (kQH - 1)));
    if (e < lim) {
      a.q.key[e] = key;
      a.q.pix[e] = pin;
    } else if (key != kNullKey) {
      atomicMin(&a.keys[key_index((uint32_t)x, (uint32_t)y, a.H)], key);
      atomicOr(&a.q.flag[(tx0 + (hx ? 1u : 0u)) * a.q.tiles_y + ty0 + (hy ? 1u : 0u)], 1u);
      a.big_count[1] = 1u;
    }
  }
  return mask;
}

constexpr int kLaneBox = 24;
constexpr int kLaneBoxMin = 20;
constexpr int kSpread = (kLaneBox / 8) * (kLaneBox / 8);
constexpr int kSpreadTris = 64 / kSpread;
__device__ __forceinline__ void coop_reserve(const RasterArgs& a, const Tri& t, const uint32_t sub, uint32_t (&rb)[6]) {
  const int tX0 = t.x0 / kQW, tY0 = t.y0 / kQH;
  const int ntx = t.x1 / kQW - tX0 + 1, nty = t.y1 / kQH - tY0 + 1;
  auto reserve = [&](int j) -> uint32_t {
    if (j >= ntx * nty) return 0u;
    const int jx = tX0 + j / nty, jy = tY0 + j % nty;
    const int wx = min(t.x1, jx * kQW + kQW - 1) - max(t.x0, jx * kQW) + 1, hy = min(t.y1, jy * kQH + kQH - 1) - max(t.y0, jy * kQH) + 1;
    return atomicAdd(&a.q.count[((uint32_t)jx * a.q.tiles_y + (uint32_t)jy) * kQSub + sub], (uint32_t)(wx * hy));
  };
#pragma unroll
  for (int j = 0; j < 6; j++) rb[j] = reserve(j);
}
template <bool TEX>
__device__ __forceinline__ void coop_walk(const RasterArgs& a, const Tri& t, const uint32_t (&rb)[6], const int src, const uint64_t fsrc,
                                          const uint32_t psrc, const uint32_t sub) {
  const int lane = threadIdx.x & 63;
  const uint32_t rb0 = rb[0], rb1 = rb[1], rb2 = rb[2], rb3 = rb[3], rb4 = rb[4], rb5 = rb[5];
    auto bi = [&](int v) -> int { return __builtin_amdgcn_readlane(v, src); };
    auto bd = [&](double v) -> double { return __hiloint2double(bi(__double2hiint(v)), bi(__double2loint(v))); };
    const int X0 = bi(t.x0), X1 = bi(t.x1), Y0 = bi(t.y0), Y1 = bi(t.y1);
    const double e0A = bd(t.e0.A), e0B = bd(t.e0.B), e0C = bd(t.e0.C);
    const double e1A = bd(t.e1.A), e1B = bd(t.e1.B), e1C = bd(t.e1.C);
    const double e2A = bd(t.e2.A), e2B = bd(t.e2.B), e2C = bd(t.e2.C);
    const double iz0 = bd(t.iz0), iz1 = bd(t.iz1), iz2 = bd(t.iz2);
    const int c0 = bi(t.cls0), c1 = bi(t.cls1), c2 = bi(t.cls2);
    const uint32_t fb = (uint32_t)bi((int)(uint32_t)fsrc);
    const uint32_t fbid = (uint32_t)bi((int)psrc);
    uint32_t tfirst = 0u, tres = 0u;
    if constexpr (TEX) { tfirst = a.tex_first[fb]; tres = a.tex_res[fb]; }
    const int tX0 = X0 / kQW, tY0 = Y0 / kQH, nty = Y1 / kQH - tY0 + 1;
    const uint32_t sb0 = (uint32_t)bi((int)rb0), sb1 = (uint32_t)bi((int)rb1), sb2 = (uint32_t)bi((int)rb2),
                   sb3 = (uint32_t)bi((int)rb3), sb4 = (uint32_t)bi((int)rb4), sb5 = (uint32_t)bi((int)rb5);
    const int bh = Y1 - Y0 + 1, area = (X1 - X0 + 1) * bh;
    const uint32_t bh_rcp = bh > 1 ? 0xFFFFFFFFu / (uint32_t)bh + 1u : 0u;
    for (int i = lane; i < area + lane; i += 64) {
      const bool in_box = i < area;
      const int col = bh > 1 ? (int)__umulhi((uint32_t)i, bh_rcp) : i;
      const int x = X0 + (in_box ? col : 0), y = Y0 + (in_box ? i - col * bh : 0);
      const double px = (double)x + 0.5, py = (double)y + 0.5;
      const double w0 = __builtin_fma(e0A, px, __builtin_fma(e0B, py, e0C));
      const double w1 = __builtin_fma(e1A, px, __builtin_fma(e1B, py, e1C));
      const double w2 = __builtin_fma(e2A, px, __builtin_fma(e2B, py, e2C));
      const bool cov = edge_accepts(w0, c0) && edge_accepts(w1, c1) && edge_accepts(w2, c2);
      unsigned long long key = kNullKey;
      if (in_box && cov) {
        const double num = (w0 + w1) + w2;
        const double den = __builtin_fma(w2, iz2, __builtin_fma(w1, iz1, w0 * iz0));
        const float zf = (float)(num / den);
        if (zf > 0.0f && isfinite(zf)) {
          uint32_t prim = fbid;
          if constexpr (TEX) prim = tfirst + texel_of(tres, w1 / num, w2 / num);
          key = ((unsigned long long)__float_as_uint(zf) << 32) | prim;
        }
      }
      const int jx = x / kQW, jy = y / kQH;
      const int xlo = max(X0, jx * kQW), ylo = max(Y0, jy * kQH), hy = min(Y1, jy * kQH + kQH - 1) - ylo + 1;
      const int jt = (jx - tX0) * nty + (jy - tY0);
      const uint32_t tb = jt == 0 ? sb0 : jt == 1 ? sb1 : jt == 2 ? sb2 : jt == 3 ? sb3 : jt == 4 ? sb4 : sb5;
      const uint32_t slot = tb + (uint32_t)((x - xlo) * hy + (y - ylo));
      const uint32_t tile = (uint32_t)jx * a.q.tiles_y + (uint32_t)jy;
      if (!in_box) continue;
      if (slot < a.q.cap) {
        const uint64_t e = ((uint64_t)tile * kQSub + sub) * a.q.cap + slot;
        a.q.key[e] = key;
        a.q.pix[e] = (uint16_t)((x - jx * kQW) * kQH + (y - jy * kQH));
      } else if (key != kNullKey) {
        atomicMin(&a.keys[key_index((uint32_t)x, (uint32_t)y, a.H)], key);
        atomicOr(&a.q.flag[tile], 1u);
        a.big_count[1] = 1u;
      }
    }
}

template <int MODE>
__device__ __forceinline__ void raster_frag_64(const RasterArgs& a, const uint64_t f, const int32_t i0, const int32_t i1, const int32_t i2,
                                               const uint32_t sub, const int part_in = -1, const bool listed = false) {
  constexpr bool kWgPush = (MODE & 1) != 0, kSpreadMode = (MODE & 2) != 0, kTex = (MODE & 4) != 0;
  const int lane = threadIdx.x & 63;
  const int part = kSpreadMode ? part_in : -1;
  const bool owner = part <= 0 && !listed;
  TriFrag rec;
  rec.x0 = 0; rec.y0 = 0; rec.kind = 0; rec.pad = 0; rec.mask = 0ull;
  Tri t;
  t.x0 = 0; t.y0 = 0; t.x1 = -1; t.y1 = -1;
  unsigned long long cover = 0ull;
  int CX0 = 0, CY0 = 0;
  bool medium = false, lanebox = false, small = false;
  bool q_big = false, q_mid = false, q_huge = false;
  const uint32_t pid = (a.prim_id && f < a.F) ? a.prim_id[f] : (uint32_t)f;
  const int have = f < a.F ? load_tri_ex(a, f, t, i0, i1, i2) : 0;
  if (have) {
    const int bw = t.x1 - t.x0 + 1, bh = t.y1 - t.y0 + 1;
    rec.x0 = (uint16_t)t.x0; rec.y0 = (uint16_t)t.y0;
    CX0 = t.x0; CY0 = t.y0;
    if (bw > 8 || bh > 8 || have == 2) {
      q_big = owner;
      q_mid = owner && bw * bh <= kMidBox;
      rec.kind = 2;
      rec.mask = (unsigned long long)(uint32_t)t.x1 | ((unsigned long long)(uint32_t)t.y1 << 16);
      if (bw <= kLaneBox && bh <= kLaneBox && have == 1) {
        if (part < 0) lanebox = true;
        else {
          constexpr int kSub = kLaneBox / 8;
          CX0 = t.x0 + 8 * (part / kSub); CY0 = t.y0 + 8 * (part % kSub);
          const int sw = min(t.x1 - CX0 + 1, 8), sh = min(t.y1 - CY0 + 1, 8);
          if (sw > 0 && sh > 0) cover = walk_box(t, CX0, CY0, sw, sh);
        }
      } else if (owner) {
        if (bw <= kMedium && bh <= kMedium && have == 1) medium = true;
        else q_huge = true;
      }
    } else if (owner) {
      small = true;
      cover = walk_box(t, t.x0, t.y0, bw, bh);
    }
  }
  {
    __shared__ uint32_t s_push[kWgPush ? 3 : 1][6];
    const int wv = (int)(threadIdx.x >> 6);
    (void)wv; (void)s_push;
    uint32_t* const counter[3] = {a.big_count, a.big_count + 3, a.big_count + 2};
    const bool want[3] = {q_big, q_mid, q_huge};
    uint32_t slot[3];
    if constexpr (kWgPush) {
      unsigned long long m[3];
#pragma unroll
      for (int q = 0; q < 3; q++) {
        m[q] = __ballot(want[q]);
        if (lane == 0) s_push[q][wv] = (uint32_t)__popcll(m[q]);
      }
      __syncthreads();
      if (threadIdx.x == 0u) {
        uint32_t total[3], base[3] = {0u, 0u, 0u};
#pragma unroll
        for (int q = 0; q < 3; q++) total[q] = s_push[q][0] + s_push[q][1] + s_push[q][2] + s_push[q][3];
        if (total[0]) base[0] = atomicAdd(a.big_count, total[0]);
        if (total[1]) base[1] = atomicAdd(a.big_count + 3, total[1]);
        if (total[2]) base[2] = atomicAdd(a.big_count + 2, total[2]);
#pragma unroll
        for (int q = 0; q < 3; q++) s_push[q][4] = base[q];
      }
      __syncthreads();
#pragma unroll
      for (int q = 0; q < 3; q++) {
        uint32_t before = s_push[q][4];
        for (int w = 0; w < wv; w++) before += s_push[q][w];
        slot[q] = want[q] ? before + (uint32_t)__popcll(m[q] & ((1ull << lane) - 1ull)) : 0xFFFFFFFFu;
      }
      __syncthreads();
    } else {
#pragma unroll
      for (int q = 0; q < 3; q++) {
        const unsigned long long m = __ballot(want[q]);
        slot[q] = 0xFFFFFFFFu;
        if (m == 0ull) continue;
        const int leader = __ffsll((long long)m) - 1;
        uint32_t base = 0u;
        if (lane == leader) base = atomicAdd(counter[q], (uint32_t)__popcll(m));
        base = (uint32_t)__shfl((int)base, leader);
        if (want[q]) slot[q] = base + (uint32_t)__popcll(m & ((1ull << lane) - 1ull));
      }
    }
    if (q_big && slot[0] < a.big_capacity) a.big_queue[slot[0]] = (uint32_t)f;
    if (q_mid && slot[1] < a.big_capacity) a.big_queue[(uint64_t)a.big_capacity + slot[1]] = (uint32_t)f;
    if (q_huge && slot[2] < a.big_capacity) a.huge_queue[slot[2]] = (uint32_t)f;
  }
  {
    const unsigned long long mask = emit_cover<kTex>(a, t, f, pid, CX0, CY0, cover, sub);
    if (mask && small) rec.kind = 1;
    if (rec.kind == 1) rec.mask = mask;
  }
  if (owner) {
    if (a.frags && f < a.F && (rec.kind != 0 || !a.kinds)) a.frags[f] = rec;
    if (a.kinds && f < a.F) a.kinds[f] = (uint8_t)rec.kind;
  }
  if constexpr (kWgPush && !kSpreadMode) {
    if (a.balance >= 2u) {
      const unsigned long long m = __ballot(lanebox);
      if (m != 0ull) {
        const int leader = __ffsll((long long)m) - 1;
        uint32_t base = 0u;
        if (lane == leader) base = atomicAdd(a.big_count + 5, (uint32_t)__popcll(m));
        base = (uint32_t)__shfl((int)base, leader);
        if (lanebox) a.med_queue[a.big_capacity - 1u - (base + (uint32_t)__popcll(m & ((1ull << lane) - 1ull)))] = (uint32_t)f;
      }
      lanebox = false;
    }
  }
  if ((int)__popcll(__ballot(lanebox)) < kLaneBoxMin) { medium = medium || lanebox; lanebox = false; }
  if (__ballot(lanebox) != 0ull) {
    constexpr int kSub = kLaneBox / 8;
    for (int k = 0; k < kSub * kSub; k++) {
      const int X0 = t.x0 + 8 * (k / kSub), Y0 = t.y0 + 8 * (k % kSub);
      const int bw = lanebox ? min(t.x1 - X0 + 1, 8) : 0, bh = lanebox ? min(t.y1 - Y0 + 1, 8) : 0;
      const bool on = bw > 0 && bh > 0;
      if (__ballot(on) == 0ull) continue;
      const unsigned long long cv = on ? walk_box(t, X0, Y0, bw, bh) : 0ull;
      (void)emit_cover<kTex>(a, t, f, pid, on ? X0 : 0, on ? Y0 : 0, cv, sub);
    }
  }

  uint32_t rb[6] = {0u, 0u, 0u, 0u, 0u, 0u};
  if constexpr (kWgPush) {
    if (a.balance) {
      const unsigned long long m = __ballot(medium);
      if (m != 0ull) {
        const int leader = __ffsll((long long)m) - 1;
        uint32_t base = 0u;
        if (lane == leader) base = atomicAdd(a.big_count + 4, (uint32_t)__popcll(m));
        base = (uint32_t)__shfl((int)base, leader);
        if (medium) a.med_queue[base + (uint32_t)__popcll(m & ((1ull << lane) - 1ull))] = (uint32_t)f;
      }
      return;
    }
  }
  if (medium) coop_reserve(a, t, sub, rb);
  unsigned long long todo = __ballot(medium);
  while (todo) {
    const int src = __ffsll((long long)todo) - 1;
    todo &= todo - 1ull;
    coop_walk<kTex>(a, t, rb, src, f, pid, sub);
  }
}

template <bool TEX>
__device__ __forceinline__ void raster_medium_wave(const RasterArgs& a, const uint32_t wave, const uint32_t nwaves) {
  const int lane = threadIdx.x & 63;
  const uint32_t n = min(a.big_count[4], a.big_capacity);
  for (uint32_t i = wave; i < n; i += nwaves) {
    const uint32_t g = a.med_queue[i];
    if (g >= a.F) continue;
    const int32_t g0 = a.faces[3 * (uint64_t)g + 0], g1 = a.faces[3 * (uint64_t)g + 1], g2 = a.faces[3 * (uint64_t)g + 2];
    Tri t;
    if (load_tri_ex(a, g, t, g0, g1, g2) != 1) continue;
    uint32_t rb[6] = {0u, 0u, 0u, 0u, 0u, 0u};
    if (lane == 0) coop_reserve(a, t, i & (kQSub - 1), rb);
    coop_walk<TEX>(a, t, rb, 0, g, a.prim_id ? a.prim_id[g] : g, i & (kQSub - 1));
  }
  constexpr int kLanes = kSpread, kTris = kSpreadTris;
  const uint32_t nl = min(a.big_count[5], a.big_capacity);
  const uint32_t turns = (nl + (uint32_t)kTris - 1u) / (uint32_t)kTris;
  for (uint32_t i = wave; i < turns; i += nwaves) {
    const int tri = lane / kLanes;
    const uint32_t e = i * (uint32_t)kTris + (uint32_t)tri;
    uint64_t fs = a.F;
    if (tri < kTris && e < nl) fs = a.med_queue[a.big_capacity - 1u - e];
    int32_t s0 = 0, s1 = 0, s2 = 0;
    if (fs < a.F) { s0 = a.faces[3 * fs + 0]; s1 = a.faces[3 * fs + 1]; s2 = a.faces[3 * fs + 2]; }
    raster_frag_64<TEX ? 6 : 2>(a, fs, s0, s1, s2, i & (kQSub - 1), lane % kLanes, true);
  }
}
template <bool TEX>
__global__ __launch_bounds__(256) void k_raster_medium(RasterArgs a) {
  raster_medium_wave<TEX>(a, (blockIdx.x * blockDim.x + threadIdx.x) >> 6, (gridDim.x * blockDim.x) >> 6);
}

template <bool LOOP, int MODE>
__device__ __forceinline__ void raster_frag_wave(const RasterArgs& a, const uint64_t wave_id) {
  const int lane = threadIdx.x & 63;
  if constexpr ((MODE & 2) != 0) {
    const int tri = lane / kSpread;
    uint64_t fs = wave_id * (uint64_t)kSpreadTris + (uint64_t)tri;
    if (tri >= kSpreadTris || fs >= a.F) fs = a.F;
    int32_t s0 = 0, s1 = 0, s2 = 0;
    if (fs < a.F) { s0 = a.faces[3 * fs + 0]; s1 = a.faces[3 * fs + 1]; s2 = a.faces[3 * fs + 2]; }
    raster_frag_64<MODE>(a, fs, s0, s1, s2, (uint32_t)wave_id & (kQSub - 1), lane % kSpread);
    return;
  } else {
  const uint32_t G = LOOP ? a.groups : 1u;
  uint64_t f = lane < (int)a.tpw ? wave_id * G * a.tpw + lane : a.F;
  int32_t n0 = 0, n1 = 0, n2 = 0;
  if (f < a.F) { n0 = a.faces[3 * f + 0]; n1 = a.faces[3 * f + 1]; n2 = a.faces[3 * f + 2]; }
  for (uint32_t g = 0; g < G; g++) {
    const int32_t i0 = n0, i1 = n1, i2 = n2;
    const uint64_t fn = f + 64u;
    if (g + 1 < G && fn < a.F) { n0 = a.faces[3 * fn + 0]; n1 = a.faces[3 * fn + 1]; n2 = a.faces[3 * fn + 2]; }
    raster_frag_64<MODE>(a, f, i0, i1, i2, (uint32_t)(wave_id * G + g) & (kQSub - 1));
    f = fn < a.F ? fn : a.F;
  }
  }
}

__device__ __forceinline__ uint32_t xcd_block(const uint32_t xcd, const uint32_t s, const uint32_t run) {
  const uint32_t q = s / run;
  return (q * 8u + xcd) * run + (s - q * run);
}
inline uint32_t xcd_slots(uint32_t nblocks, uint32_t run) { return (uint32_t)div_up(nblocks, 8u * run) * run; }

template <int MODE>
__global__ __launch_bounds__(256) __attribute__((amdgpu_waves_per_eu((MODE & 3) ? 4 : 5, 5))) void k_raster_frag(RasterArgs a, uint32_t nblocks, uint32_t chunk) {
  const uint32_t tb = chunk ? xcd_block(blockIdx.x & 7u, blockIdx.x >> 3, chunk) : blockIdx.x;
  if (tb >= nblocks) return;
  raster_frag_wave<false, MODE>(a, ((uint64_t)tb * blockDim.x + threadIdx.x) >> 6);
}
int raster_mode(const RasterArgs& a) { return (a.spread ? 3 : a.wg_push ? 1 : 0) | (a.tex_res ? 4 : 0); }

struct RasterGroup {
  RasterArgs view[kMaxGroup];
  uint32_t* idx[kMaxGroup];
  uint32_t tile_end[kMaxGroup];
  uint32_t n, blocks_per_view;
  uint32_t chunk;
};
template <int MODE>
__global__ __launch_bounds__(256) __attribute__((amdgpu_waves_per_eu((MODE & 3) ? 4 : 5, 5))) void k_raster_frag_group(RasterGroup g) {
  uint32_t v, tb;
  if (g.chunk) {
    const uint32_t k = blockIdx.x >> 3, sq = k / g.n;
    v = k - sq * g.n;
    tb = xcd_block(blockIdx.x & 7u, sq, g.chunk);
    if (tb >= g.blocks_per_view) return;
  } else {
    v = blockIdx.x / g.blocks_per_view;
    tb = blockIdx.x - v * g.blocks_per_view;
  }
  raster_frag_wave<true, MODE>(g.view[v], ((uint64_t)tb * blockDim.x + threadIdx.x) >> 6);
}
template <bool TEX>
__global__ __launch_bounds__(256) void k_raster_medium_group(RasterGroup g, uint32_t blocks_per_view) {
  const uint32_t v = blockIdx.x / blocks_per_view;
  raster_medium_wave<TEX>(g.view[v], ((blockIdx.x - v * blocks_per_view) * blockDim.x + threadIdx.x) >> 6, (blocks_per_view * blockDim.x) >> 6);
}
__device__ __forceinline__ void raster_huge_block(const RasterArgs& a, const uint32_t tile) {
  __shared__ uint32_t s_hits[256];
  __shared__ uint32_t s_nhits;
  const uint32_t nbig = min(a.big_count[2], a.big_capacity);
  if (nbig == 0u) return;
  const FragQueues& q = a.q;
  const int t = threadIdx.x;
  const uint32_t tx = tile / q.tiles_y, ty = tile - tx * q.tiles_y;
  const uint32_t x0 = tx * kQW, y0 = ty * kQH;
  const int tx1 = (int)min(x0 + kQW, a.W) - 1, ty1 = (int)min(y0 + kQH, a.H) - 1;
  bool any = false;
  if (t == 0) s_nhits = 0u;
  __syncthreads();
  for (uint32_t qb = 0; qb < nbig; qb += 256u) {
    const uint32_t qi = qb + (uint32_t)t;
    if (qi < nbig) {
      const uint32_t f = a.huge_queue[qi];
      const TriFrag rec = a.frags[f];
      const int bx1 = (int)(rec.mask & 0xFFFFu), by1 = (int)((rec.mask >> 16) & 0xFFFFu);
      if (rec.kind == 2 && (int)rec.x0 <= tx1 && bx1 >= (int)x0 && (int)rec.y0 <= ty1 && by1 >= (int)y0)
        s_hits[atomicAdd(&s_nhits, 1u)] = f;
    }
    __syncthreads();
    const uint32_t nh = s_nhits;
    for (uint32_t h = 0; h < nh; h++) {
      const uint64_t f = s_hits[h];
      for (int p = 0; p < 2; p++) {
        Piece pc;
        if (!load_piece(a, f, p, pc)) continue;
        const Tri& tr = pc.t;
        const int xa = max(tr.x0, (int)x0), xb = min(tr.x1, tx1), ya = max(tr.y0, (int)y0), yb = min(tr.y1, ty1);
        const int hh = yb - ya + 1, area = (xb - xa + 1) * hh;
        if (hh <= 0) continue;
        for (int i = t; i < area; i += 256) {
          const int x = xa + i / hh, y = ya + i % hh;
          const unsigned long long key = shade_piece_key(a, f, pc, x, y);
          if (key != kNullKey) { atomicMin(&a.keys[key_index((uint32_t)x, (uint32_t)y, a.H)], key); any = true; }
        }
      }
    }
    __syncthreads();
    if (t == 0) s_nhits = 0u;
    __syncthreads();
  }
  if (any) atomicOr(&q.flag[tile], 2u);
}

__global__ __launch_bounds__(256) void k_raster_huge(RasterArgs a, uint32_t ntiles) {
  if (min(a.big_count[2], a.big_capacity) == 0u) return;
  for (uint32_t tile = blockIdx.x; tile < ntiles; tile += gridDim.x) { raster_huge_block(a, tile); __syncthreads(); }
}

template <typename PlanesWanted>
__device__ __forceinline__ void tile_resolve_block(const RasterArgs& a, uint32_t* __restrict__ idx_out, float* __restrict__ depth_out,
                                                   const uint32_t tile, PlanesWanted planes_wanted) {
  __shared__ unsigned long long skeys[kQPixels];
  __shared__ uint32_t scount[kQSub];
  const FragQueues& q = a.q;
  const int t = threadIdx.x;
  const uint32_t W = a.W, H = a.H;
  const uint32_t tx = tile / q.tiles_y, ty = tile - tx * q.tiles_y;
  const uint32_t x0 = tx * kQW, y0 = ty * kQH;
  constexpr uint32_t kGroup = 256u / kQSub, kSpec = 6;
  const uint32_t sq = (uint32_t)t / kGroup, sq_lane = (uint32_t)t % kGroup;
  const uint64_t qbase = ((uint64_t)tile * kQSub + sq) * q.cap;
  unsigned long long spec_key[kSpec];
  uint16_t spec_pix[kSpec];
#pragma unroll
  for (uint32_t k = 0; k < kSpec; k++) {
    const uint32_t i = min(sq_lane + k * kGroup, q.cap - 1u);
    spec_key[k] = q.key[qbase + i];
    spec_pix[k] = q.pix[qbase + i];
  }
  const uint32_t n = min(q.count[tile * kQSub + sq], q.cap);
  if (sq_lane == 0u) scount[sq] = n;
  const uint32_t tile_flag = q.flag[tile];
  const bool merge = tile_flag != 0u;
  for (int p = t; p < kQPixels; p += 256) {
    const uint32_t gx = x0 + (uint32_t)(p >> 6), gy = y0 + (uint32_t)(p & 63);
    unsigned long long k = kBackgroundKey;
    if (merge && gx < W && gy < H) {
      const uint64_t g = key_index(gx, gy, H);
      k = a.keys[g];
      a.keys[g] = kBackgroundKey;
    }
    skeys[p] = k;
  }
  __syncthreads();
#pragma unroll
  for (uint32_t k = 0; k < kSpec; k++)
    if (sq_lane + k * kGroup < n) atomicMin(&skeys[spec_pix[k]], spec_key[k]);
  constexpr uint32_t kHead = kSpec * kGroup;
  uint32_t rest[kQSub], total = 0u;
#pragma unroll
  for (int s = 0; s < kQSub; s++) { rest[s] = scount[s] > kHead ? scount[s] - kHead : 0u; total += rest[s]; }
  auto entry_of = [&](uint32_t j) -> uint64_t {
    uint32_t sub = 0u;
#pragma unroll
    for (int s = 0; s < kQSub - 1; s++) if (sub == (uint32_t)s && j >= rest[s]) { j -= rest[s]; sub = (uint32_t)s + 1u; }
    return ((uint64_t)tile * kQSub + sub) * q.cap + kHead + j;
  };
  for (uint32_t j0 = (uint32_t)t; j0 < total; j0 += 4u * 256u) {
    unsigned long long k4[4];
    uint16_t p4[4];
#pragma unroll
    for (uint32_t u = 0; u < 4u; u++) {
      const uint32_t j = j0 + u * 256u;
      const uint64_t e = j < total ? entry_of(j) : qbase;
      k4[u] = q.key[e];
      p4[u] = q.pix[e];
    }
#pragma unroll
    for (uint32_t u = 0; u < 4u; u++)
      if (j0 + u * 256u < total) atomicMin(&skeys[p4[u]], k4[u]);
  }
  __syncthreads();
  if (a.frags && !a.prim_id && !a.tex_res) {
    if (tile_flag & 1u) {
      if (t == 0) a.big_count[1] = 1u;
    } else {
      auto lost = [&](const unsigned long long key, const uint32_t pin) {
        if (key == kNullKey || skeys[pin] == key) return;
        const uint32_t f = (uint32_t)(key & 0xFFFFFFFFull);
        const TriFrag rec = a.frags[f];
        if (rec.kind != 1) return;
        const int bit = (int)(x0 + (pin >> 6) - rec.x0) * 8 + (int)(y0 + (pin & 63u) - rec.y0);
        atomicAnd(&a.frags[f].mask, ~(1ull << bit));
      };
#pragma unroll
      for (uint32_t k = 0; k < kSpec; k++)
        if (sq_lane + k * kGroup < n) lost(spec_key[k], spec_pix[k]);
      for (uint32_t j0 = (uint32_t)t; j0 < total; j0 += 4u * 256u) {
        unsigned long long k4[4];
        uint16_t p4[4];
#pragma unroll
        for (uint32_t u = 0; u < 4u; u++) {
          const uint32_t j = j0 + u * 256u;
          const uint64_t e = j < total ? entry_of(j) : qbase;
          k4[u] = q.key[e];
          p4[u] = q.pix[e];
        }
#pragma unroll
        for (uint32_t u = 0; u < 4u; u++)
          if (j0 + u * 256u < total) lost(k4[u], p4[u]);
      }
    }
  }
  if (planes_wanted())
  for (int p = t; p < kQPixels; p += 256) {
    const uint32_t gx = x0 + (uint32_t)(p >> 6), gy = y0 + (uint32_t)(p & 63);
    if (gx < W && gy < H) {
      const unsigned long long k = skeys[p];
      const uint64_t g = (uint64_t)gx * H + gy;
      idx_out[g] = (uint32_t)(k & 0xFFFFFFFFull);
      if (depth_out) depth_out[g] = __uint_as_float((uint32_t)(k >> 32));
    }
  }
  if (t < kQSub) q.count[tile * kQSub + t] = 0u;
  if (t == 0) q.flag[tile] = 0u;
}

__device__ __forceinline__ bool view_needs_planes(const RasterArgs& a) { return !a.idx_optional || a.big_count[0] != 0u || a.big_count[1] != 0u; }

__global__ __launch_bounds__(256) void k_tile_resolve(RasterArgs a, uint32_t* __restrict__ idx_out, float* __restrict__ depth_out) {
  tile_resolve_block(a, idx_out, depth_out, blockIdx.x, [&] { return view_needs_planes(a); });
}

__global__ __launch_bounds__(256) void k_raster_huge_group(RasterGroup g) {
  bool any = false;
  for (uint32_t v = 0; v < g.n; v++) any = any || min(g.view[v].big_count[2], g.view[v].big_capacity) != 0u;
  if (!any) return;
  for (uint32_t tile = blockIdx.x; tile < g.tile_end[g.n - 1]; tile += gridDim.x) {
    uint32_t v = 0;
    while (v + 1 < g.n && tile >= g.tile_end[v]) v++;
    raster_huge_block(g.view[v], tile - (v ? g.tile_end[v - 1] : 0u));
    __syncthreads();
  }
}

__global__ __launch_bounds__(256) void k_tile_resolve_group(RasterGroup g) {
  uint32_t v = 0;
  while (v + 1 < g.n && blockIdx.x >= g.tile_end[v]) v++;
  tile_resolve_block(g.view[v], g.idx[v], nullptr, blockIdx.x - (v ? g.tile_end[v - 1] : 0u), [&] {
    if (g.view[v].idx_optional == 2u) return view_needs_planes(g.view[v]);
    bool planes = false;
    for (uint32_t u = 0; u < g.n; u++) planes = planes || view_needs_planes(g.view[u]);
    return planes;
  });
}

__global__ void k_resolve(unsigned long long* __restrict__ keys, uint32_t* __restrict__ idx, float* __restrict__ depth,
                          uint32_t W, uint32_t H) {
  const uint64_t i = (uint64_t)blockIdx.x * blockDim.x + threadIdx.x;
  if (i >= (uint64_t)W * H) return;
  const uint32_t x = (uint32_t)(i / H), y = (uint32_t)(i - (uint64_t)x * H);
  const uint64_t g = key_index(x, y, H);
  const unsigned long long k = keys[g];
  keys[g] = kBackgroundKey;
  idx[i] = (uint32_t)(k & 0xFFFFFFFFull);
  if (depth) depth[i] = __uint_as_float((uint32_t)(k >> 32));
}

__global__ void k_fill_keys(unsigned long long* __restrict__ keys, uint64_t N) {
  const uint64_t i = (uint64_t)blockIdx.x * blockDim.x + threadIdx.x;
  if (i < N) keys[i] = kBackgroundKey;
}

__global__ void k_texel_area(const float* __restrict__ verts, const int32_t* __restrict__ faces, uint64_t F, uint64_t V,
                             const smesh_camera_t* __restrict__ cams, uint32_t K, float* __restrict__ best_area) {
  const uint64_t f = (uint64_t)blockIdx.x * blockDim.x + threadIdx.x;
  if (f >= F) return;
  const int32_t id[3] = {faces[3 * f], faces[3 * f + 1], faces[3 * f + 2]};
  float best = 0.0f;
  bool valid = true;
  for (int k = 0; k < 3; k++) if (id[k] < 0 || (uint64_t)id[k] >= V) valid = false;
  if (valid) {
    float P[3][3];
    for (int k = 0; k < 3; k++)
      for (int d = 0; d < 3; d++) P[k][d] = verts[3 * (uint64_t)id[k] + d];
    for (uint32_t ci = 0; ci < K; ci++) {
      const smesh_camera_t& cam = cams[ci];
      float pu[3], pv[3];
      bool in_front = false;
      for (int k = 0; k < 3; k++) {
        const float xc = ((cam.rotation[0] * P[k][0] + cam.rotation[1] * P[k][1]) + cam.rotation[2] * P[k][2]) + cam.translation[0];
        const float yc = ((cam.rotation[3] * P[k][0] + cam.rotation[4] * P[k][1]) + cam.rotation[5] * P[k][2]) + cam.translation[1];
        const float zc = ((cam.rotation[6] * P[k][0] + cam.rotation[7] * P[k][1]) + cam.rotation[8] * P[k][2]) + cam.translation[2];
        in_front |= zc > 0.0f;
        pu[k] = (float)(cam.focal[0] * ((double)xc / (double)zc) + cam.principal[0]);
        pv[k] = (float)(cam.focal[1] * ((double)yc / (double)zc) + cam.principal[1]);
      }
      const float border = 0.5f;
      const float rw = (float)(int)cam.width, rh = (float)(int)cam.height;
      bool inside = in_front;
      for (int k = 0; k < 3; k++)
        inside = inside && (-border * rw <= pu[k]) && (pu[k] < (1 + border) * rw) &&
                 (-border * rh <= pv[k]) && (pv[k] < (1 + border) * rh);
      if (inside) {
        const float area = 0.5f * fabsf((pu[0] * (pv[1] - pv[2]) + pu[1] * (pv[2] - pv[0])) + pu[2] * (pv[0] - pv[1]));
        if (area > best) best = area;
      }
    }
  }
  best_area[f] = best;
}

}

constexpr int kSlots = 2 * kMaxGroup;
constexpr int kHeld = 32;
constexpr int kSides = kSlots + kHeld;
constexpr int kRecordSides = 6;

struct ImagePair {
  uint32_t* idx;
  float* depth;
  uint64_t pixels;
  bool idx_out, depth_out;
};

struct smesh_renderer {
  DeviceCtx* ctx = nullptr;
  uint64_t V = 0, F = 0, num_primitives = 0;
  float* verts = nullptr;
  int32_t* faces = nullptr;
  struct Bounds { bool valid = false; double lo[3] = {0, 0, 0}, hi[3] = {0, 0, 0}, max_edge = 0, mean_edge = 0; } bounds;
  uint32_t* prim_id = nullptr;
  struct ViewScratch {
    ScreenVertex* sv = nullptr;
    uint32_t* huge_queue = nullptr;
    uint32_t* med_queue = nullptr;
    unsigned long long* keys = nullptr;
    uint64_t keys_pixels = 0;
    FragQueues fq;
    uint64_t fq_tiles = 0;
  } vs[kSlots];
  bool texels = false;
  uint32_t* tex_res = nullptr;
  uint32_t* tex_first = nullptr;
  std::vector<int32_t> h_faces;
  std::vector<uint32_t> h_res, h_first;
  struct Side {
    uint32_t* big_queue = nullptr;
    uint32_t* big_count = nullptr;
    TriFrag* frags = nullptr;
    uint8_t* kinds = nullptr;
  } side[kSides];
  uint32_t big_capacity = 0;
  std::vector<ImagePair> images;
  Scratch own_idx;
  Scratch fused[kSides];
  struct HeldJob {
    int n = 0, nparts = 0, next_part = 0;
    bool ranged = false;
    smesh_aggregator* agg = nullptr;
    const float* probs[kHeld] = {};
    const float* weights[kHeld] = {};
    uint64_t W[kHeld] = {}, H[kHeld] = {};
  } held;
  hipEvent_t ev_bank_rendered[2] = {nullptr, nullptr}, ev_bank_consumed[2] = {nullptr, nullptr}, ev_main_fence = nullptr;
  hipEvent_t ev_raster_done = nullptr;
  uint64_t group_seq = 0;
  bool bank_used[2] = {false, false};
  uint64_t fused_seq = 0;
  const uint32_t* last_idx[kRecordSides] = {};
  uint64_t last_W[kRecordSides] = {}, last_H[kRecordSides] = {};
  uint64_t render_seq = 0;
  bool rec_valid[kRecordSides] = {};
  bool hash_valid[kRecordSides] = {};
  unsigned long long* d_hash = nullptr;
  hipEvent_t hash_ev[kRecordSides] = {};
  Scratch match_stage;
  int last_render_side = 0;
  bool raster_pending = false;
  bool main_pending = false;
  std::mutex mu;
};

namespace {
__device__ __forceinline__ unsigned long long mix64(unsigned long long z) {
  z = (z ^ (z >> 30)) * 0xBF58476D1CE4E5B9ull;
  z = (z ^ (z >> 27)) * 0x94D049BB133111EBull;
  return z ^ (z >> 31);
}
__global__ __launch_bounds__(256) void k_plane_checksum(const uint32_t* __restrict__ img, uint64_t N, unsigned long long* __restrict__ out) {
  __shared__ unsigned long long part[4];
  unsigned long long h = 0ull;
  for (uint64_t i = (uint64_t)blockIdx.x * blockDim.x + threadIdx.x; i < N; i += (uint64_t)gridDim.x * blockDim.x)
    h += mix64((i << 32) | (unsigned long long)img[i]);
  for (int off = 32; off > 0; off >>= 1) h += __shfl_down(h, off);
  if ((threadIdx.x & 63) == 0) part[threadIdx.x >> 6] = h;
  __syncthreads();
  if (threadIdx.x == 0) atomicAdd(out, ((part[0] + part[1]) + part[2]) + part[3]);
}
int plane_checksum(DeviceCtx* ctx, hipStream_t st, const uint32_t* d_img, uint64_t N, unsigned long long* d_out) {
  SMESH_HIP(hipMemsetAsync(d_out, 0, sizeof(unsigned long long), st));
  const uint32_t blocks = (uint32_t)std::max<uint64_t>(1, std::min<uint64_t>(div_up(N, 256 * 16), (uint64_t)ctx->num_cus));
  hipLaunchKernelGGL(k_plane_checksum, dim3(blocks), dim3(256), 0, st, d_img, N, d_out);
  SMESH_HIP(hipGetLastError());
  return SMESH_OK;
}
}

namespace {
bool no_huge_possible(const smesh_renderer* r, const smesh_camera_t* cam);
bool no_big_possible(const smesh_renderer* r, const smesh_camera_t* cam);
void mesh_bounds(const float* v, uint64_t V, const int32_t* f, uint64_t F, smesh_renderer::Bounds& b);

int ensure_keys(smesh_renderer::ViewScratch& vs, uint64_t W, uint64_t H, hipStream_t st) {
  const uint64_t N = div_up(W, 4) * div_up(H, 4) * 16;
  if (N <= vs.keys_pixels) return SMESH_OK;
  if (vs.keys) SMESH_HIP(dev_free(vs.keys));
  vs.keys = nullptr;
  vs.keys_pixels = 0;
  SMESH_HIP(dev_malloc(reinterpret_cast<void**>(&vs.keys), N * 8));
  vs.keys_pixels = N;
  hipLaunchKernelGGL(k_fill_keys, dim3((uint32_t)div_up(N, 256)), dim3(256), 0, st, vs.keys, N);
  SMESH_HIP(hipGetLastError());
  return SMESH_OK;
}

int main_after_raster(smesh_renderer* r) {
  if (!r->raster_pending) return SMESH_OK;
  if (!r->ev_raster_done) SMESH_HIP(hipEventCreateWithFlags(&r->ev_raster_done, hipEventDisableTiming));
  SMESH_HIP(hipEventRecord(r->ev_raster_done, r->ctx->raster_stream));
  SMESH_HIP(hipStreamWaitEvent(r->ctx->stream, r->ev_raster_done, 0));
  r->raster_pending = false;
  return SMESH_OK;
}

enum class RasterPath { Frag, Direct };

RasterPath raster_path() {
  static const RasterPath p = [] {
    const char* e = getenv("SMESH_RASTER");
    const std::string v = e ? e : "";
    if (v == "direct") return RasterPath::Direct;
    return RasterPath::Frag;
  }();
  return p;
}

bool plane_optional_allowed(const smesh_renderer* r) {
  return !r->texels && !r->prim_id && raster_path() == RasterPath::Frag;
}

int plane_optional_level(smesh_renderer* r, smesh_aggregator* a) {
  if (r->texels || !smesh_aggregator_can_fuse_triangles(a, r->F)) return 0;
  return smesh_aggregator_fuses_small_views_by_mask(a) ? 2 : 1;
}

constexpr uint32_t kRasterXcdRun = 8;

uint64_t frag_cap_forced() {
  const char* e = getenv("SMESH_FRAG_CAP");
  return e ? std::max<uint64_t>(1, (uint64_t)atoll(e)) : 0u;
}

bool ensure_queues(smesh_renderer* r, smesh_renderer::ViewScratch& vs, uint64_t W, uint64_t H, hipStream_t st, int* status) {
  *status = SMESH_OK;
  const uint64_t tiles_x = div_up(W, kQW), tiles_y = div_up(H, kQH), ntiles = tiles_x * tiles_y;
  uint64_t cap = frag_cap_forced();
  if (!cap) {
    cap = 16ull * kQPixels / kQSub;
    const uint64_t budget = 8ull << 30;
    if (ntiles * kQSub * cap * 10 > budget) cap = budget / (ntiles * kQSub * 10);
    if (cap < 256) return false;
  }
  if (ntiles > vs.fq_tiles || (uint32_t)cap != vs.fq.cap) {
    (void)hipStreamSynchronize(r->ctx->stream);
    (void)hipStreamSynchronize(r->ctx->raster_stream);
    for (void* p : {(void*)vs.fq.key, (void*)vs.fq.pix, (void*)vs.fq.count, (void*)vs.fq.flag})
      if (p) (void)dev_free(p);
    vs.fq = FragQueues();
    vs.fq_tiles = 0;
    hipError_t e = dev_malloc(reinterpret_cast<void**>(&vs.fq.key), ntiles * kQSub * cap * 8);
    if (e == hipSuccess) e = dev_malloc(reinterpret_cast<void**>(&vs.fq.pix), ntiles * kQSub * cap * 2);
    if (e == hipSuccess) e = dev_malloc(reinterpret_cast<void**>(&vs.fq.count), ntiles * kQSub * 4);
    if (e == hipSuccess) e = dev_malloc(reinterpret_cast<void**>(&vs.fq.flag), ntiles * 4);
    if (e == hipSuccess) e = hipMemsetAsync(vs.fq.count, 0, ntiles * kQSub * 4, st);
    if (e == hipSuccess) e = hipMemsetAsync(vs.fq.flag, 0, ntiles * 4, st);
    if (e != hipSuccess) { *status = fail_hip(e, "fragment queue allocation", __FILE__, __LINE__); return false; }
    vs.fq.cap = (uint32_t)cap;
    vs.fq_tiles = ntiles;
  }
  vs.fq.tiles_y = (uint32_t)tiles_y;
  return true;
}

CameraArgs camera_args(const smesh_camera_t* cam) {
  CameraArgs ca;
  memcpy(ca.R, cam->rotation, sizeof ca.R);
  memcpy(ca.t, cam->translation, sizeof ca.t);
  ca.fx = cam->focal[0]; ca.fy = cam->focal[1]; ca.cx = cam->principal[0]; ca.cy = cam->principal[1];
  ca.W = (uint32_t)cam->width; ca.H = (uint32_t)cam->height;
  return ca;
}

double typical_edge_pixels(const smesh_renderer* r, const smesh_camera_t* cam) {
  const smesh_renderer::Bounds& b = r->bounds;
  if (!b.valid || !(b.mean_edge > 0.0)) return 0.0;
  double z = cam->translation[2];
  for (int d = 0; d < 3; d++) z += (double)cam->rotation[6 + d] * 0.5 * (b.lo[d] + b.hi[d]);
  if (!(z > 1e-3)) return 0.0;
  const double e = b.mean_edge * std::max(std::fabs(cam->focal[0]), std::fabs(cam->focal[1])) / z;
  return std::isfinite(e) ? e : 0.0;
}
double depth_spread(const smesh_renderer* r, const smesh_camera_t* cam) {
  const smesh_renderer::Bounds& b = r->bounds;
  if (!b.valid) return 1.0;
  double zmin = INFINITY, zmax = -INFINITY;
  for (int c = 0; c < 8; c++) {
    double z = cam->translation[2];
    for (int d = 0; d < 3; d++) z += (double)cam->rotation[6 + d] * ((c >> d) & 1 ? b.hi[d] : b.lo[d]);
    zmin = std::min(zmin, z); zmax = std::max(zmax, z);
  }
  if (!(zmax > 0.0)) return 1.0;
  return zmin > 1e-3 * zmax ? zmax / zmin : INFINITY;
}
bool want_spread(const smesh_renderer* r, const smesh_camera_t* cam, int nviews) {
  static const int knob = env_int("SMESH_RASTER_SPREAD", -1);
  if (knob == 0 || !cam) return false;
  if (knob == 1) return true;
  if (nviews > 1) return false;
  if (depth_spread(r, cam) > 6.0) return false;
  const double e = typical_edge_pixels(r, cam);
  return e >= 10.5 && e <= 19.0;
}

RasterArgs raster_args(smesh_renderer* r, smesh_renderer::ViewScratch& vs, int side, uint64_t W, uint64_t H, int nviews = 1,
                       const smesh_camera_t* cam = nullptr) {
  RasterArgs a;
  a.faces = r->faces; a.verts = r->verts; a.sv = vs.sv; a.tex_res = r->texels ? r->tex_res : nullptr; a.tex_first = r->tex_first;
  a.prim_id = r->prim_id;
  a.keys = vs.keys; a.F = r->F; a.V = r->V; a.W = (uint32_t)W; a.H = (uint32_t)H;
  a.big_queue = r->side[side].big_queue; a.big_count = r->side[side].big_count; a.big_capacity = r->big_capacity;
  a.huge_queue = vs.huge_queue;
  a.med_queue = vs.med_queue;
  {
    static const int knob = env_int("SMESH_RASTER_BALANCE", -1);
    a.balance = (vs.med_queue && (knob >= 0 ? knob != 0 : (cam && depth_spread(r, cam) > 6.0))) ? (nviews > 1 ? 1u : 2u) : 0u;
  }
  a.frags = r->side[side].frags;
  a.kinds = r->side[side].kinds;
  a.q = FragQueues();
  a.idx_optional = 0u;
  a.tpw = 64;
  const bool fine = r->F >= 32768u;
  const uint64_t min_waves = fine ? 1024u : 2048u;
  const uint64_t launch_views = fine ? (uint64_t)std::max(1, nviews) : 1u;
  while (a.tpw > 1 && launch_views * r->F / a.tpw < min_waves) a.tpw >>= 1;
  a.groups = 1;
  a.spread = 0u;
  {
    static const int knob = env_int("SMESH_RASTER_WG_PUSH", -1);
    a.wg_push = knob >= 0 ? (uint32_t)(knob != 0) : (cam && typical_edge_pixels(r, cam) >= 5.0 ? 1u : 0u);
  }
  if (want_spread(r, cam, nviews)) { a.spread = (uint32_t)kSpread; a.tpw = (uint32_t)kSpreadTris; }
  return a;
}

uint32_t frag_groups(uint64_t F, int views, uint32_t tpw) {
  static const int knob = env_int("SMESH_RASTER_GROUPS", 0);
  if (tpw != 64u) return 1u;
  if (knob >= 1) return (uint32_t)knob;
  return (F >= 4000000u && (uint64_t)views * div_up(F, 256u) >= 20480u) ? 4u : 1u;
}

int render_into(smesh_renderer* r, const smesh_camera_t* cam, uint32_t* d_idx, float* d_depth, hipStream_t st = nullptr,
                int side = 0, int idx_optional = 0) {
  DeviceCtx* ctx = r->ctx;
  r->last_render_side = side;
  if (!st) {
    st = ctx->stream;
    SMESH_TRY(main_after_raster(r));
    r->main_pending = true;
  }
  const uint64_t W = cam->width, H = cam->height, N = W * H;
  smesh_renderer::ViewScratch& vs = r->vs[0];
  SMESH_TRY(ensure_keys(vs, W, H, st));
  ProfScope prof(ctx, SMESH_PROF_RASTER, st);
  const CameraArgs ca = camera_args(cam);
  RasterArgs a = raster_args(r, vs, side, W, H, 1, cam);
  a.cam = ca;
  if (r->V) {
    hipLaunchKernelGGL(k_project_vertices, dim3((uint32_t)div_up(r->V, 256)), dim3(256), 0, st, r->verts, r->V, ca, vs.sv,
                       r->side[side].big_count);
    SMESH_HIP(hipGetLastError());
  } else {
    SMESH_HIP(hipMemsetAsync(r->side[side].big_count, 0, 32, st));
  }
  if (r->F) {
    a.idx_optional = (idx_optional && plane_optional_allowed(r)) ? (uint32_t)idx_optional : 0u;
    const uint32_t big_grid = (uint32_t)std::min<uint64_t>(r->F, (uint64_t)ctx->num_cus);
    int qs = SMESH_OK;
    if (raster_path() == RasterPath::Frag && ensure_queues(r, vs, W, H, st, &qs)) {
      a.q = vs.fq;
      {
        const uint32_t nblocks = (uint32_t)div_up(div_up(r->F, a.tpw), 4);
        const uint32_t chunk = nblocks >= 64u ? kRasterXcdRun : 0u;
        const dim3 grid(chunk ? 8u * xcd_slots(nblocks, chunk) : nblocks);
        switch (raster_mode(a)) {
          case 7:  hipLaunchKernelGGL(k_raster_frag<7>, grid, dim3(256), 0, st, a, nblocks, chunk); break;
          case 5:  hipLaunchKernelGGL(k_raster_frag<5>, grid, dim3(256), 0, st, a, nblocks, chunk); break;
          case 4:  hipLaunchKernelGGL(k_raster_frag<4>, grid, dim3(256), 0, st, a, nblocks, chunk); break;
          case 3:  hipLaunchKernelGGL(k_raster_frag<3>, grid, dim3(256), 0, st, a, nblocks, chunk); break;
          case 1:  hipLaunchKernelGGL(k_raster_frag<1>, grid, dim3(256), 0, st, a, nblocks, chunk); break;
          default: hipLaunchKernelGGL(k_raster_frag<0>, grid, dim3(256), 0, st, a, nblocks, chunk); break;
        }
        if ((raster_mode(a) & 3) != 0 && a.balance) {
          const dim3 mgrid(4u * (uint32_t)std::max(1, ctx->num_cus));
          if (a.tex_res) hipLaunchKernelGGL(k_raster_medium<true>, mgrid, dim3(256), 0, st, a);
          else hipLaunchKernelGGL(k_raster_medium<false>, mgrid, dim3(256), 0, st, a);
        }
      }
      SMESH_HIP(hipGetLastError());
      const uint32_t ntiles = (uint32_t)(div_up(W, kQW) * div_up(H, kQH));
      if (!no_huge_possible(r, cam)) hipLaunchKernelGGL(k_raster_huge, dim3(std::min<uint32_t>(ntiles, 2u * (uint32_t)ctx->num_cus)), dim3(256), 0, st, a, ntiles);
      SMESH_HIP(hipGetLastError());
      hipLaunchKernelGGL(k_tile_resolve, dim3((uint32_t)(div_up(W, kQW) * div_up(H, kQH))), dim3(256), 0, st, a, d_idx, d_depth);
      SMESH_HIP(hipGetLastError());
      return SMESH_OK;
    }
    SMESH_TRY(qs);
    hipLaunchKernelGGL(k_raster_small, dim3((uint32_t)div_up(r->F, 256)), dim3(256), 0, st, a);
    SMESH_HIP(hipGetLastError());
    hipLaunchKernelGGL(k_raster_big, dim3(big_grid), dim3(256), 0, st, a, 0u);
    SMESH_HIP(hipGetLastError());
  }
  hipLaunchKernelGGL(k_resolve, dim3((uint32_t)div_up(N, 256)), dim3(256), 0, st, vs.keys, d_idx, d_depth, (uint32_t)W, (uint32_t)H);
  SMESH_HIP(hipGetLastError());
  SMESH_HIP(hipMemsetAsync(r->side[side].big_count + 1, 0xFF, 4, st));
  return SMESH_OK;
}

hipError_t alloc_side(smesh_renderer* r, int i);

hipError_t alloc_scratch(smesh_renderer* r, int i) {
  smesh_renderer::ViewScratch& vs = r->vs[i];
  hipError_t e = hipSuccess;
  if (!vs.sv) e = dev_malloc(reinterpret_cast<void**>(&vs.sv), std::max<uint64_t>(r->V * sizeof(ScreenVertex), 16));
  if (e == hipSuccess && !vs.huge_queue) e = dev_malloc(reinterpret_cast<void**>(&vs.huge_queue), (size_t)r->big_capacity * 4);
  if (e == hipSuccess && !vs.med_queue) e = dev_malloc(reinterpret_cast<void**>(&vs.med_queue), (size_t)r->big_capacity * 4);
  return e;
}

bool queues_fit_group(uint64_t W, uint64_t H) {
  if (raster_path() != RasterPath::Frag) return false;
  if (frag_cap_forced()) return true;
  const uint64_t ntiles = div_up(W, kQW) * div_up(H, kQH);
  const uint64_t cap = 16ull * kQPixels / kQSub;
  return ntiles * kQSub * cap * 10 <= (2ull << 30);
}

int prepare_group_slots(smesh_renderer* r, const smesh_camera_t* cams, int n, hipStream_t st, int base) {
  for (int v = 0; v < n; v++) {
    const uint64_t W = cams[v].width, H = cams[v].height, N = W * H;
    SMESH_HIP(alloc_side(r, base + v));
    SMESH_HIP(alloc_scratch(r, base + v));
    smesh_renderer::ViewScratch& vs = r->vs[base + v];
    SMESH_TRY(ensure_keys(vs, W, H, st));
    int qs = SMESH_OK;
    if (!ensure_queues(r, vs, W, H, st, &qs)) return qs != SMESH_OK ? qs : fail(SMESH_ERR_RUNTIME, "fragment queues unavailable");
    if (r->fused[base + v].bytes < N * 8) {
      SMESH_HIP(hipStreamSynchronize(st));
      SMESH_HIP(hipStreamSynchronize(r->ctx->stream));
      SMESH_TRY(r->fused[base + v].reserve(N * 8));
    }
  }
  return SMESH_OK;
}

int render_group_into(smesh_renderer* r, const smesh_camera_t* cams, int n, hipStream_t st, int base = 0, int side_base = -1,
                      int idx_optional = 0) {
  if (side_base < 0) side_base = base;
  if (!plane_optional_allowed(r)) idx_optional = 0;
  DeviceCtx* ctx = r->ctx;
  ProjectGroup pg;
  RasterGroup rg;
  memset(&pg, 0, sizeof pg);
  memset(&rg, 0, sizeof rg);
  uint32_t tiles = 0;
  for (int v = 0; v < n; v++) {
    const uint64_t W = cams[v].width, H = cams[v].height, N = W * H;
    SMESH_HIP(alloc_side(r, side_base + v));
    SMESH_HIP(alloc_scratch(r, base + v));
    smesh_renderer::ViewScratch& vs = r->vs[base + v];
    SMESH_TRY(ensure_keys(vs, W, H, st));
    int qs = SMESH_OK;
    if (!ensure_queues(r, vs, W, H, st, &qs)) return qs != SMESH_OK ? qs : fail(SMESH_ERR_RUNTIME, "fragment queues unavailable");
    if (r->fused[side_base + v].bytes < N * 8) {
      SMESH_HIP(hipStreamSynchronize(st));
      SMESH_HIP(hipStreamSynchronize(r->ctx->stream));
      SMESH_TRY(r->fused[side_base + v].reserve(N * 8));
    }
    if (side_base + v < kRecordSides) { r->last_idx[side_base + v] = nullptr; r->rec_valid[side_base + v] = false; }
    pg.cam[v] = camera_args(&cams[v]);
    pg.sv[v] = vs.sv;
    pg.big_count[v] = r->side[side_base + v].big_count;
    rg.view[v] = raster_args(r, vs, side_base + v, W, H, n);
    { const RasterArgs own = raster_args(r, vs, side_base + v, W, H, 1, &cams[v]); rg.view[v].wg_push = own.wg_push; rg.view[v].balance = own.balance; }
    rg.view[v].cam = pg.cam[v];
    rg.view[v].q = vs.fq;
    rg.view[v].idx_optional = (uint32_t)idx_optional;
    rg.idx[v] = static_cast<uint32_t*>(r->fused[side_base + v].ptr);
    tiles += (uint32_t)(div_up(W, kQW) * div_up(H, kQH));
    rg.tile_end[v] = tiles;
  }
  pg.verts = r->verts; pg.V = r->V;
  pg.n = (uint32_t)n;
  rg.n = (uint32_t)n;
  {
    int votes = 0;
    for (int v = 0; v < n; v++) votes += want_spread(r, &cams[v], n) ? 1 : 0;
    if (2 * votes >= n && votes > 0)
      for (int v = 0; v < n; v++) { rg.view[v].spread = (uint32_t)kSpread; rg.view[v].tpw = (uint32_t)kSpreadTris; }
    int push_votes = 0;
    for (int v = 0; v < n; v++) push_votes += rg.view[v].wg_push ? 1 : 0;
    for (int v = 0; v < n; v++) rg.view[v].wg_push = 2 * push_votes >= n && push_votes > 0 ? 1u : 0u;
    int balance_votes = 0;
    for (int v = 0; v < n; v++) balance_votes += rg.view[v].balance ? 1 : 0;
    for (int v = 0; v < n; v++) rg.view[v].balance = 2 * balance_votes >= n && balance_votes > 0 ? (n > 1 ? 1u : 2u) : 0u;
  }
  for (int v = 0; v < n; v++) rg.view[v].groups = frag_groups(r->F, n, rg.view[0].tpw);
  rg.blocks_per_view = (uint32_t)div_up(div_up(r->F, rg.view[0].tpw * rg.view[0].groups), 4);
  ProfScope prof(ctx, SMESH_PROF_RASTER, st);
  hipLaunchKernelGGL(k_project_vertices_group, dim3((uint32_t)div_up(r->V, 256)), dim3(256), 0, st, pg);
  SMESH_HIP(hipGetLastError());
  {
    rg.chunk = rg.blocks_per_view >= 64u ? kRasterXcdRun : 0u;
    const dim3 grid(rg.chunk ? 8u * xcd_slots(rg.blocks_per_view, rg.chunk) * (uint32_t)n : (uint32_t)n * rg.blocks_per_view);
    switch (raster_mode(rg.view[0])) {
      case 7:  hipLaunchKernelGGL(k_raster_frag_group<7>, grid, dim3(256), 0, st, rg); break;
      case 5:  hipLaunchKernelGGL(k_raster_frag_group<5>, grid, dim3(256), 0, st, rg); break;
      case 4:  hipLaunchKernelGGL(k_raster_frag_group<4>, grid, dim3(256), 0, st, rg); break;
      case 3:  hipLaunchKernelGGL(k_raster_frag_group<3>, grid, dim3(256), 0, st, rg); break;
      case 1:  hipLaunchKernelGGL(k_raster_frag_group<1>, grid, dim3(256), 0, st, rg); break;
      default: hipLaunchKernelGGL(k_raster_frag_group<0>, grid, dim3(256), 0, st, rg); break;
    }
    if ((raster_mode(rg.view[0]) & 3) != 0 && rg.view[0].balance) {
      const uint32_t per_view = std::max(64u, 4u * (uint32_t)std::max(1, ctx->num_cus) / (uint32_t)n);
      if (rg.view[0].tex_res) hipLaunchKernelGGL(k_raster_medium_group<true>, dim3((uint32_t)n * per_view), dim3(256), 0, st, rg, per_view);
      else hipLaunchKernelGGL(k_raster_medium_group<false>, dim3((uint32_t)n * per_view), dim3(256), 0, st, rg, per_view);
    }
  }
  SMESH_HIP(hipGetLastError());
  bool huge_needed = false;
  for (int v = 0; v < n; v++) huge_needed = huge_needed || !no_huge_possible(r, &cams[v]);
  if (huge_needed) hipLaunchKernelGGL(k_raster_huge_group, dim3(std::min<uint32_t>(tiles, 4u * (uint32_t)ctx->num_cus)), dim3(256), 0, st, rg);
  SMESH_HIP(hipGetLastError());
  hipLaunchKernelGGL(k_tile_resolve_group, dim3(tiles), dim3(256), 0, st, rg);
  SMESH_HIP(hipGetLastError());
  return SMESH_OK;
}

int acquire_image(smesh_renderer* r, uint64_t N, ImagePair** out) {
  for (auto& im : r->images)
    if (!im.idx_out && !im.depth_out && im.pixels == N) { *out = &im; return SMESH_OK; }
  for (size_t i = 0; i < r->images.size();) {
    ImagePair& im = r->images[i];
    if (!im.idx_out && !im.depth_out) {
      SMESH_HIP(hipStreamSynchronize(r->ctx->stream));
      (void)dev_free(im.idx);
      (void)dev_free(im.depth);
      r->images.erase(r->images.begin() + i);
    } else {
      i++;
    }
  }
  ImagePair im{nullptr, nullptr, N, false, false};
  SMESH_HIP(dev_malloc(reinterpret_cast<void**>(&im.idx), N * 4));
  hipError_t e = dev_malloc(reinterpret_cast<void**>(&im.depth), N * 4);
  if (e != hipSuccess) { (void)dev_free(im.idx); return fail_hip(e, "hipMalloc depth plane", __FILE__, __LINE__); }
  r->images.push_back(im);
  *out = &r->images.back();
  return SMESH_OK;
}

int check_camera(const smesh_camera_t* cam) {
  if (!cam) return fail(SMESH_ERR_INVALID, "camera is NULL");
  if (cam->width == 0 || cam->height == 0 || cam->width > 65536 || cam->height > 65536)
    return fail(SMESH_ERR_INVALID, "camera resolution must be in [1, 65536]");
  if (cam->width * cam->height >= 0x7FFFFFFFull / 4) return fail(SMESH_ERR_INVALID, "image too large");
  return SMESH_OK;
}

hipError_t alloc_side(smesh_renderer* r, int i) {
  smesh_renderer::Side& sd = r->side[i];
  if (sd.frags) return hipSuccess;
  hipError_t e = dev_malloc(reinterpret_cast<void**>(&sd.big_queue), (size_t)r->big_capacity * 8);
  if (e == hipSuccess) e = dev_malloc(reinterpret_cast<void**>(&sd.big_count), 32);
  if (e == hipSuccess) e = dev_malloc(reinterpret_cast<void**>(&sd.frags), std::max<uint64_t>(r->F * sizeof(TriFrag), 16));
  if (e == hipSuccess && r->texels) e = dev_malloc(reinterpret_cast<void**>(&sd.kinds), std::max<uint64_t>(r->F, 16));
  if (e == hipSuccess) e = hipMemsetAsync(sd.big_count, 0, 32, r->ctx->stream);
  if (e == hipSuccess) e = hipStreamSynchronize(r->ctx->stream);
  return e;
}

void mesh_bounds(const float* v, uint64_t V, const int32_t* f, uint64_t F, smesh_renderer::Bounds& b) {
  b.valid = false;
  if (!V || !F) return;
  float lo[3] = {INFINITY, INFINITY, INFINITY}, hi[3] = {-INFINITY, -INFINITY, -INFINITY};
  bool finite = true;
  for (uint64_t i = 0; i < V; i++)
    for (int d = 0; d < 3; d++) {
      const float x = v[3 * i + d];
      finite = finite && std::isfinite(x);
      lo[d] = std::min(lo[d], x); hi[d] = std::max(hi[d], x);
    }
  if (!finite) return;
  double m2 = 0.0, sum_edges = 0.0;
  uint64_t edges = 0;
  for (uint64_t i = 0; i < F; i++) {
    const int32_t a = f[3 * i], c = f[3 * i + 1], e = f[3 * i + 2];
    if (a < 0 || c < 0 || e < 0 || (uint64_t)a >= V || (uint64_t)c >= V || (uint64_t)e >= V) continue;
    const float* p[3] = {v + 3 * (uint64_t)a, v + 3 * (uint64_t)c, v + 3 * (uint64_t)e};
    for (int k = 0; k < 3; k++) {
      const float* q = p[k]; const float* w = p[(k + 1) % 3];
      const double dx = (double)q[0] - w[0], dy = (double)q[1] - w[1], dz = (double)q[2] - w[2];
      m2 = std::max(m2, dx * dx + dy * dy + dz * dz);
      sum_edges += std::sqrt(dx * dx + dy * dy + dz * dz);
      edges++;
    }
  }
  b.mean_edge = edges ? sum_edges / (double)edges : 0.0;
  for (int d = 0; d < 3; d++) { b.lo[d] = lo[d]; b.hi[d] = hi[d]; }
  b.max_edge = std::sqrt(m2);
  b.valid = std::isfinite(b.max_edge);
}

double box_extent_bound(const smesh_renderer::Bounds& b, const smesh_camera_t* cam) {
  if (!b.valid) return INFINITY;
  const double W = (double)cam->width, H = (double)cam->height;
  double zmin = INFINITY, mag = 0.0, frob2 = 0.0;
  for (int row = 0; row < 3; row++) {
    double m = std::fabs((double)cam->translation[row]);
    for (int d = 0; d < 3; d++) {
      const double R = cam->rotation[3 * row + d];
      m += std::fabs(R) * std::max(std::fabs(b.lo[d]), std::fabs(b.hi[d]));
      frob2 += R * R;
    }
    mag = std::max(mag, m);
  }
  for (int c = 0; c < 8; c++) {
    double z = cam->translation[2];
    for (int d = 0; d < 3; d++) z += (double)cam->rotation[6 + d] * ((c >> d) & 1 ? b.hi[d] : b.lo[d]);
    zmin = std::min(zmin, z);
  }
  const double eps = 32.0 * 5.9604644775390625e-08 * mag;
  const double z_lo = zmin - eps;
  const double L = std::sqrt(frob2) * b.max_edge + 4.0 * eps;
  if (!(z_lo > 1e-3) || !std::isfinite(mag) || !std::isfinite(L)) return INFINITY;
  const double ratio = L / z_lo;
  if (!(ratio < 0.25)) return INFINITY;
  const double fx = std::fabs(cam->focal[0]), fy = std::fabs(cam->focal[1]);
  const double ax = std::max(std::fabs(cam->principal[0]), std::fabs(W - cam->principal[0])) + 1.0;
  const double ay = std::max(std::fabs(cam->principal[1]), std::fabs(H - cam->principal[1])) + 1.0;
  const double du = (fx + ax) * ratio / (1.0 - ratio), dv = (fy + ay) * ratio / (1.0 - ratio);
  if (!std::isfinite(du) || !std::isfinite(dv)) return INFINITY;
  return std::max(du, dv);
}
bool no_huge_possible(const smesh_renderer* r, const smesh_camera_t* cam) { return box_extent_bound(r->bounds, cam) <= (double)kMedium - 4.0; }
bool no_big_possible(const smesh_renderer* r, const smesh_camera_t* cam) { return box_extent_bound(r->bounds, cam) <= 6.5; }

int create_common(const float* vertices, uint64_t V, const int32_t* faces, uint64_t F, int device,
                  smesh_renderer** out) {
  if (!out) return fail(SMESH_ERR_INVALID, "out is NULL");
  *out = nullptr;
  if ((V && !vertices) || (F && !faces)) return fail(SMESH_ERR_INVALID, "NULL mesh arrays");
  if (F >= 0xFFFFFFFFull || V >= 0x7FFFFFFFull) return fail(SMESH_ERR_INVALID, "mesh too large for 32-bit indices");
  DeviceCtx* ctx;
  SMESH_TRY(get_ctx(device, &ctx));
  SMESH_HIP(hipSetDevice(device));
  auto* r = new (std::nothrow) smesh_renderer();
  if (!r) return fail(SMESH_ERR_RUNTIME, "out of memory");
  r->ctx = ctx; r->V = V; r->F = F; r->num_primitives = F;
  r->big_capacity = (uint32_t)std::max<uint64_t>(F, 1);
  mesh_bounds(vertices, V, faces, F, r->bounds);
  hipError_t e = dev_malloc(reinterpret_cast<void**>(&r->verts), std::max<uint64_t>(V * 12, 16));
  if (e == hipSuccess) e = dev_malloc(reinterpret_cast<void**>(&r->faces), std::max<uint64_t>(F * 12, 16));
  if (e == hipSuccess) e = dev_malloc(reinterpret_cast<void**>(&r->vs[0].sv), std::max<uint64_t>(V * sizeof(ScreenVertex), 16));
  if (e == hipSuccess) e = alloc_side(r, 0);
  if (e == hipSuccess) e = dev_malloc(reinterpret_cast<void**>(&r->vs[0].huge_queue), (size_t)r->big_capacity * 4);
  if (e == hipSuccess) e = dev_malloc(reinterpret_cast<void**>(&r->vs[0].med_queue), (size_t)r->big_capacity * 4);
  if (e == hipSuccess && V) e = hipMemcpyAsync(r->verts, vertices, V * 12, hipMemcpyHostToDevice, ctx->stream);
  if (e == hipSuccess && F) e = hipMemcpyAsync(r->faces, faces, F * 12, hipMemcpyHostToDevice, ctx->stream);
  if (e == hipSuccess) e = hipStreamSynchronize(ctx->stream);
  if (e != hipSuccess) {
    smesh_renderer_destroy(r);
    return fail_hip(e, "renderer allocation/upload", __FILE__, __LINE__);
  }
  *out = r;
  return SMESH_OK;
}

}

static bool spatial_order(const float* v, uint64_t V, const int32_t* f, uint64_t F, std::vector<uint32_t>& order) {
  const char* env = getenv("SMESH_REORDER");
  if (env && atoi(env) == 0) return false;
  const bool force = env && atoi(env) == 1;
  if (F < 4096 && !force) return false;
  std::vector<float> cx(F), cy(F), cz(F);
  double lo[3] = {1e300, 1e300, 1e300}, hi[3] = {-1e300, -1e300, -1e300}, edge_sum = 0.0;
  uint64_t edges = 0;
  for (uint64_t i = 0; i < F; i++) {
    const int32_t a = f[3 * i], b = f[3 * i + 1], c = f[3 * i + 2];
    if (a < 0 || b < 0 || c < 0 || (uint64_t)a >= V || (uint64_t)b >= V || (uint64_t)c >= V) { cx[i] = cy[i] = cz[i] = 0.f; continue; }
    const float* pa = v + 3 * (uint64_t)a; const float* pb = v + 3 * (uint64_t)b; const float* pc = v + 3 * (uint64_t)c;
    cx[i] = (pa[0] + pb[0] + pc[0]) / 3.f; cy[i] = (pa[1] + pb[1] + pc[1]) / 3.f; cz[i] = (pa[2] + pb[2] + pc[2]) / 3.f;
    if (!std::isfinite(cx[i]) || !std::isfinite(cy[i]) || !std::isfinite(cz[i])) { cx[i] = cy[i] = cz[i] = 0.f; continue; }
    const double c3[3] = {cx[i], cy[i], cz[i]};
    for (int d = 0; d < 3; d++) { lo[d] = std::min(lo[d], c3[d]); hi[d] = std::max(hi[d], c3[d]); }
    if ((i & 15) == 0) { edge_sum += std::sqrt((double)(pa[0] - pb[0]) * (pa[0] - pb[0]) + (double)(pa[1] - pb[1]) * (pa[1] - pb[1]) + (double)(pa[2] - pb[2]) * (pa[2] - pb[2])); edges++; }
  }
  if (!(lo[0] <= hi[0]) || !edges) return false;
  auto spread = [&](const uint32_t* ord) {
    double total = 0.0;
    for (uint64_t g = 0; g < F; g += 64) {
      float l0 = 1e30f, l1 = 1e30f, l2 = 1e30f, h0 = -1e30f, h1 = -1e30f, h2 = -1e30f;
      const uint64_t e = std::min<uint64_t>(F, g + 64);
      for (uint64_t i = g; i < e; i++) {
        const uint64_t j = ord ? ord[i] : i;
        l0 = std::min(l0, cx[j]); h0 = std::max(h0, cx[j]); l1 = std::min(l1, cy[j]); h1 = std::max(h1, cy[j]);
        l2 = std::min(l2, cz[j]); h2 = std::max(h2, cz[j]);
      }
      total += (double)(h0 - l0) + (double)(h1 - l1) + (double)(h2 - l2);
    }
    return total;
  };
  const double before = spread(nullptr);
  const double neighbours = (double)((F + 63) / 64) * 16.0 * (edge_sum / (double)edges);
  if (!force && before <= 6.0 * neighbours) return false;
  std::vector<std::pair<uint64_t, uint32_t>> keyed(F);
  auto spread_bits = [](uint64_t x) {
    x &= 0x1FFFFFull;
    x = (x | x << 32) & 0x1F00000000FFFFull; x = (x | x << 16) & 0x1F0000FF0000FFull; x = (x | x << 8) & 0x100F00F00F00F00Full;
    x = (x | x << 4) & 0x10C30C30C30C30C3ull; x = (x | x << 2) & 0x1249249249249249ull;
    return x;
  };
  const double sx = hi[0] > lo[0] ? 2097151.0 / (hi[0] - lo[0]) : 0.0, sy = hi[1] > lo[1] ? 2097151.0 / (hi[1] - lo[1]) : 0.0,
               sz = hi[2] > lo[2] ? 2097151.0 / (hi[2] - lo[2]) : 0.0;
  for (uint64_t i = 0; i < F; i++) {
    const uint64_t qx = (uint64_t)std::min(2097151.0, std::max(0.0, (cx[i] - lo[0]) * sx)), qy = (uint64_t)std::min(2097151.0, std::max(0.0, (cy[i] - lo[1]) * sy)),
                   qz = (uint64_t)std::min(2097151.0, std::max(0.0, (cz[i] - lo[2]) * sz));
    keyed[i] = {spread_bits(qx) | (spread_bits(qy) << 1) | (spread_bits(qz) << 2), (uint32_t)i};
  }
  std::sort(keyed.begin(), keyed.end());
  order.resize(F);
  for (uint64_t i = 0; i < F; i++) order[i] = keyed[i].second;
  if (!force && spread(order.data()) * 2.0 > before) { order.clear(); return false; }
  return true;
}

static thread_local const char* g_last_fuse_kernel = "none";
static thread_local const char* g_last_add_path = "none";
void smesh_note_fuse(const char* kernel, const char* path) { g_last_fuse_kernel = kernel; g_last_add_path = path; }

static bool labels_native(smesh_renderer* r, smesh_aggregator* a, uint64_t N) {
  return !r->texels && !r->prim_id && smesh_labels_native(a, r->F, N);
}

constexpr int kLabelsPlaneLevel = 1;

static int fuse_rendered(smesh_renderer* r, smesh_aggregator* a, int slot, const uint32_t* d_idx, const float* probs,
                         const float* weights, int memkind, uint64_t W, uint64_t H, int64_t ps0 = 0, int64_t ps1 = 0, int label_bytes = 0) {
  DeviceCtx* ctx = r->ctx;
  const uint64_t N = W * H;
  const float* d_probs = probs;
  const float* d_w = weights;
  if (label_bytes) {
    if (labels_native(r, a, N)) {
      RenderedView rv{r->side[slot].frags, r->side[slot].big_queue, r->side[slot].big_count, d_idx, nullptr, d_w, W, H, 0, 0, true};
      rv.labels = probs;
      SMESH_TRY(smesh_labels_fuse_triangles(a, r->F, r->big_capacity, &rv, 1, label_bytes));
      smesh_note_fuse("k_fuse_tri_labels", "render-records");
      return SMESH_OK;
    }
    SMESH_TRY(smesh_labels_expand(a, probs, label_bytes, N, &d_probs));
  }
  if (memkind == SMESH_MEM_HOST) {
    const uint32_t C = smesh_aggregator_classes(a);
    Scratch& sp = smesh_aggregator_stage_probs(a);
    SMESH_TRY(sp.reserve(N * C * 4));
    SMESH_HIP(hipMemcpyAsync(sp.ptr, probs, N * C * 4, hipMemcpyHostToDevice, ctx->stream));
    d_probs = static_cast<const float*>(sp.ptr);
    if (weights) {
      Scratch& sw = smesh_aggregator_stage_w(a);
      SMESH_TRY(sw.reserve(N * 4));
      SMESH_HIP(hipMemcpyAsync(sw.ptr, weights, N * 4, hipMemcpyHostToDevice, ctx->stream));
      d_w = static_cast<const float*>(sw.ptr);
    }
    SMESH_HIP(hipStreamSynchronize(ctx->stream));
  }
  if (!r->texels && smesh_aggregator_can_fuse_triangles(a, r->F)) {
    const RenderedView rv{r->side[slot].frags, r->side[slot].big_queue, r->side[slot].big_count, d_idx, d_probs, d_w, W, H, ps0, ps1, true};
    SMESH_TRY(smesh_aggregator_fuse_triangles(a, r->F, r->prim_id, r->big_capacity, &rv, 1));
    smesh_note_fuse(smesh_aggregator_fuse_kernel_name(a, r->prim_id != nullptr), "render-records");
  } else if (r->texels && smesh_aggregator_can_fuse_texels(a, r->num_primitives)) {
    SMESH_TRY(smesh_aggregator_fuse_texels(a, r->side[slot].frags, r->side[slot].kinds, r->F, r->tex_first, r->tex_res, r->side[slot].big_queue,
                                           r->side[slot].big_count, r->big_capacity, d_idx, d_probs, d_w, H));
    smesh_note_fuse("k_fuse_texel", "render-records");
  } else {
    SMESH_TRY(smesh_aggregator_add_device_contig(a, d_idx, d_probs, d_w, W, H));
  }
  return SMESH_OK;
}

extern "C" {

const char* smesh_last_fuse_kernel(void) { return g_last_fuse_kernel; }
const char* smesh_last_add_path(void) { return g_last_add_path; }

int smesh_renderer_create_triangles(const float* vertices, uint64_t V, const int32_t* faces, uint64_t F, int device,
                                    smesh_renderer_t** out) {
  DeviceCtx* ctx;
  SMESH_TRY(get_ctx(device, &ctx));
  std::lock_guard<std::recursive_mutex> lock(ctx->mu);
  if ((V && !vertices) || (F && !faces)) return fail(SMESH_ERR_INVALID, "NULL mesh arrays");
  std::vector<uint32_t> order;
  if (!spatial_order(vertices, V, faces, F, order)) return create_common(vertices, V, faces, F, device, out);
  std::vector<int32_t> hf(3 * F);
  for (uint64_t i = 0; i < F; i++)
    for (int k = 0; k < 3; k++) hf[3 * i + k] = faces[3 * (uint64_t)order[i] + k];
  smesh_renderer* r = nullptr;
  SMESH_TRY(create_common(vertices, V, hf.data(), F, device, &r));
  hipError_t e = dev_malloc(reinterpret_cast<void**>(&r->prim_id), F * 4);
  if (e == hipSuccess) e = hipMemcpyAsync(r->prim_id, order.data(), F * 4, hipMemcpyHostToDevice, ctx->stream);
  if (e == hipSuccess) e = hipStreamSynchronize(ctx->stream);
  if (e != hipSuccess) { smesh_renderer_destroy(r); return fail_hip(e, "primitive id table upload", __FILE__, __LINE__); }
  *out = r;
  return SMESH_OK;
}

int smesh_renderer_create_texels(const float* vertices, uint64_t V, const int32_t* faces, uint64_t F,
                                 const smesh_camera_t* cameras, uint64_t K, float tpp, int device,
                                 smesh_renderer_t** out) {
  if (K && !cameras) return fail(SMESH_ERR_INVALID, "NULL cameras");
  if (K > 0xFFFFFFFFull) return fail(SMESH_ERR_INVALID, "too many cameras");
  DeviceCtx* ctx;
  SMESH_TRY(get_ctx(device, &ctx));
  std::lock_guard<std::recursive_mutex> lock(ctx->mu);

  std::vector<int32_t> hf(faces, faces + 3 * F);
  for (uint64_t f = 0; f < F; f++) {
    int32_t* face = &hf[3 * f];
    bool valid = true;
    for (int k = 0; k < 3; k++) if (face[k] < 0 || (uint64_t)face[k] >= V) valid = false;
    if (!valid) continue;
    float diffs[3];
    for (int k = 0; k < 3; k++) {
      const float* p0 = vertices + 3 * (size_t)face[k];
      const float* p1 = vertices + 3 * (size_t)face[(k + 1) % 3];
      const float* p2 = vertices + 3 * (size_t)face[(k + 2) % 3];
      const float ax = p1[0] - p0[0], ay = p1[1] - p0[1], az = p1[2] - p0[2];
      const float bx = p2[0] - p0[0], by = p2[1] - p0[1], bz = p2[2] - p0[2];
      const float dot = ax * bx + ay * by + az * bz;
      const float la = std::sqrt(ax * ax + ay * ay + az * az), lb = std::sqrt(bx * bx + by * by + bz * bz);
      float cosv = dot / (la * lb);
      cosv = cosv > 1.0f ? 1.0f : (cosv < -1.0f ? -1.0f : cosv);
      diffs[k] = std::fabs(std::acos(cosv) - 1.57079632679489661923f);
    }
    int best = 0;
    for (int k = 1; k < 3; k++) if (diffs[k] < diffs[best]) best = k;
    if (best != 0) { std::swap(face[0], face[best]); std::swap(diffs[0], diffs[best]); }
    if (diffs[1] >= diffs[2]) std::swap(face[1], face[2]);
  }

  smesh_renderer* r = nullptr;
  SMESH_TRY(create_common(vertices, V, hf.data(), F, device, &r));
  r->texels = true;
  if (!r->side[0].kinds && dev_malloc(reinterpret_cast<void**>(&r->side[0].kinds), std::max<uint64_t>(F, 16)) != hipSuccess) {
    smesh_renderer_destroy(r);
    return fail(SMESH_ERR_RUNTIME, "texel renderer: allocation of the kind bytes failed");
  }
  r->h_faces = std::move(hf);
  r->h_res.assign(F, 0);
  r->h_first.assign(F, 0);

  std::vector<float> best(F, 0.0f);
  if (F && K) {
    smesh_camera_t* d_cams = nullptr;
    float* d_best = nullptr;
    int32_t* d_faces = nullptr;
    hipError_t e = dev_malloc(reinterpret_cast<void**>(&d_cams), K * sizeof(smesh_camera_t));
    if (e == hipSuccess) e = dev_malloc(reinterpret_cast<void**>(&d_best), F * 4);
    if (e == hipSuccess) e = dev_malloc(reinterpret_cast<void**>(&d_faces), F * 12);
    if (e == hipSuccess) e = hipMemcpyAsync(d_cams, cameras, K * sizeof(smesh_camera_t), hipMemcpyHostToDevice, ctx->stream);
    if (e == hipSuccess) e = hipMemcpyAsync(d_faces, faces, F * 12, hipMemcpyHostToDevice, ctx->stream);
    if (e == hipSuccess) {
      hipLaunchKernelGGL(k_texel_area, dim3((uint32_t)div_up(F, 128)), dim3(128), 0, ctx->stream, r->verts, d_faces, F, V,
                         d_cams, (uint32_t)K, d_best);
      e = hipGetLastError();
    }
    if (e == hipSuccess) e = hipMemcpyAsync(best.data(), d_best, F * 4, hipMemcpyDeviceToHost, ctx->stream);
    if (e == hipSuccess) e = hipStreamSynchronize(ctx->stream);
    if (d_cams) (void)dev_free(d_cams);
    if (d_best) (void)dev_free(d_best);
    if (d_faces) (void)dev_free(d_faces);
    if (e != hipSuccess) { smesh_renderer_destroy(r); return fail_hip(e, "texel area reduction", __FILE__, __LINE__); }
  }
  uint64_t total = 0;
  for (uint64_t f = 0; f < F; f++) {
    const uint32_t res = (uint32_t)std::ceil(tpp * std::sqrt(best[f]));
    r->h_res[f] = res;
    r->h_first[f] = (uint32_t)total;
    total += (uint64_t)res * (res + 1) / 2;
  }
  if (total >= 0xFFFFFFFFull) { smesh_renderer_destroy(r); return fail(SMESH_ERR_INVALID, "texel count overflows uint32"); }
  r->num_primitives = total;
  hipError_t e = dev_malloc(reinterpret_cast<void**>(&r->tex_res), std::max<uint64_t>(F * 4, 16));
  if (e == hipSuccess) e = dev_malloc(reinterpret_cast<void**>(&r->tex_first), std::max<uint64_t>(F * 4, 16));
  if (e == hipSuccess && F) e = hipMemcpyAsync(r->tex_res, r->h_res.data(), F * 4, hipMemcpyHostToDevice, ctx->stream);
  if (e == hipSuccess && F) e = hipMemcpyAsync(r->tex_first, r->h_first.data(), F * 4, hipMemcpyHostToDevice, ctx->stream);
  if (e == hipSuccess) e = hipStreamSynchronize(ctx->stream);
  if (e != hipSuccess) { smesh_renderer_destroy(r); return fail_hip(e, "texel table upload", __FILE__, __LINE__); }
  *out = r;
  return SMESH_OK;
}

int smesh_renderer_destroy(smesh_renderer_t* r) {
  if (!r) return SMESH_OK;
  (void)hipSetDevice(r->ctx->device);
  (void)hipStreamSynchronize(r->ctx->raster_stream);
  (void)hipStreamSynchronize(r->ctx->stream);
  for (void* p : {(void*)r->prim_id, (void*)r->verts, (void*)r->faces, (void*)r->tex_res, (void*)r->tex_first})
    if (p) (void)dev_free(p);
  for (auto& sd : r->side)
    for (void* p : {(void*)sd.big_queue, (void*)sd.big_count, (void*)sd.frags, (void*)sd.kinds})
      if (p) (void)dev_free(p);
  for (auto& vs : r->vs)
    for (void* p : {(void*)vs.sv, (void*)vs.huge_queue, (void*)vs.med_queue, (void*)vs.keys, (void*)vs.fq.key, (void*)vs.fq.pix, (void*)vs.fq.count, (void*)vs.fq.flag})
      if (p) (void)dev_free(p);
  for (auto& im : r->images) { (void)dev_free(im.idx); (void)dev_free(im.depth); }
  r->own_idx.release();
  r->match_stage.release();
  if (r->d_hash) (void)dev_free(r->d_hash);
  for (int sd = 0; sd < kRecordSides; sd++)
    if (r->hash_ev[sd]) (void)hipEventDestroy(r->hash_ev[sd]);
  for (auto& f : r->fused) f.release();
  for (int i = 0; i < 2; i++) {
    if (i == 0 && r->ev_main_fence) (void)hipEventDestroy(r->ev_main_fence);
    if (r->ev_bank_rendered[i]) (void)hipEventDestroy(r->ev_bank_rendered[i]);
    if (r->ev_bank_consumed[i]) (void)hipEventDestroy(r->ev_bank_consumed[i]);
  }
  delete r;
  return SMESH_OK;
}

int smesh_renderer_num_primitives(const smesh_renderer_t* r, uint64_t* out) {
  if (!r || !out) return fail(SMESH_ERR_INVALID, "NULL argument");
  *out = r->num_primitives;
  return SMESH_OK;
}

int smesh_renderer_texel_layout(const smesh_renderer_t* r, int32_t* faces_out, uint32_t* res_out, uint32_t* first_out) {
  if (!r) return fail(SMESH_ERR_INVALID, "NULL renderer");
  if (!r->texels) return fail(SMESH_ERR_INVALID, "not a texel renderer");
  if (faces_out && r->F) memcpy(faces_out, r->h_faces.data(), r->F * 12);
  if (res_out && r->F) memcpy(res_out, r->h_res.data(), r->F * 4);
  if (first_out && r->F) memcpy(first_out, r->h_first.data(), r->F * 4);
  return SMESH_OK;
}

}

int smesh_renderer_texel_tables(const smesh_renderer* r, DeviceCtx** ctx, uint64_t* F, uint64_t* P, const uint32_t** first, const uint32_t** res) {
  if (!r) return fail(SMESH_ERR_INVALID, "NULL renderer");
  if (!r->texels) return fail(SMESH_ERR_INVALID, "not a texel renderer");
  *ctx = r->ctx;
  *F = r->F;
  *P = r->num_primitives;
  *first = r->tex_first;
  *res = r->tex_res;
  return SMESH_OK;
}

extern "C" {

int smesh_renderer_render_device(smesh_renderer_t* r, const smesh_camera_t* cam, uint32_t** indices_dev, float** depth_dev) {
  if (!r || !indices_dev || !depth_dev) return fail(SMESH_ERR_INVALID, "NULL argument");
  SMESH_TRY(check_camera(cam));
  std::lock_guard<std::mutex> g(r->mu);
  std::lock_guard<std::recursive_mutex> lock(r->ctx->mu);
  SMESH_HIP(hipSetDevice(r->ctx->device));
  ImagePair* im;
  SMESH_TRY(acquire_image(r, cam->width * cam->height, &im));
  const int side = (int)(r->render_seq++ % (uint64_t)kRecordSides);
  if (side != 0) SMESH_HIP(alloc_side(r, side));
  r->last_idx[side] = nullptr; r->rec_valid[side] = false;
  SMESH_TRY(render_into(r, cam, im->idx, im->depth, nullptr, side));
  for (int sd = 0; sd < kRecordSides; sd++)
    if (r->last_idx[sd] == im->idx) r->last_idx[sd] = nullptr;
  r->last_idx[side] = im->idx; r->last_W[side] = cam->width; r->last_H[side] = cam->height;
  r->rec_valid[side] = true;
  r->hash_valid[side] = false;
  im->idx_out = im->depth_out = true;
  *indices_dev = im->idx;
  *depth_dev = im->depth;
  return SMESH_OK;
}

int smesh_renderer_release_image(smesh_renderer_t* r, void* indices_dev, void* depth_dev) {
  if (!r) return fail(SMESH_ERR_INVALID, "NULL renderer");
  std::lock_guard<std::mutex> g(r->mu);
  for (auto& im : r->images) {
    if (indices_dev && im.idx == indices_dev) im.idx_out = false;
    if (depth_dev && im.depth == depth_dev) im.depth_out = false;
  }
  return SMESH_OK;
}

int smesh_renderer_render(smesh_renderer_t* r, const smesh_camera_t* cam, uint32_t* indices_out, float* depth_out) {
  if (!r || !indices_out) return fail(SMESH_ERR_INVALID, "NULL argument");
  SMESH_TRY(check_camera(cam));
  std::lock_guard<std::mutex> g(r->mu);
  DeviceCtx* ctx = r->ctx;
  std::lock_guard<std::recursive_mutex> lock(ctx->mu);
  SMESH_HIP(hipSetDevice(ctx->device));
  const uint64_t N = cam->width * cam->height;
  SMESH_TRY(r->own_idx.reserve(N * 8));
  uint32_t* d_idx = static_cast<uint32_t*>(r->own_idx.ptr);
  float* d_depth = reinterpret_cast<float*>(d_idx + N);
  r->last_idx[0] = nullptr; r->rec_valid[0] = false;
  SMESH_TRY(render_into(r, cam, d_idx, d_depth));
  SMESH_HIP(hipMemcpyAsync(indices_out, d_idx, N * 4, hipMemcpyDeviceToHost, ctx->stream));
  if (depth_out) SMESH_HIP(hipMemcpyAsync(depth_out, d_depth, N * 4, hipMemcpyDeviceToHost, ctx->stream));
  SMESH_HIP(hipStreamSynchronize(ctx->stream));
  return SMESH_OK;
}

static int fuse_view_impl(smesh_renderer_t* r, smesh_aggregator_t* a, const smesh_camera_t* cam, const float* probs,
                          const float* weights, int memkind, int label_bytes) {
  if (!r || !a || !probs) return fail(SMESH_ERR_INVALID, "NULL argument");
  SMESH_TRY(check_camera(cam));
  DeviceCtx* ctx = r->ctx;
  if (smesh_aggregator_ctx(a) != ctx) return fail(SMESH_ERR_INVALID, "renderer and aggregator live on different devices");
  std::lock_guard<std::mutex> g(r->mu);
  std::lock_guard<std::mutex> g2(smesh_aggregator_mutex(a));
  std::lock_guard<std::recursive_mutex> lock(ctx->mu);
  SMESH_HIP(hipSetDevice(ctx->device));
  SMESH_TRY(smesh_aggregator_join_exchange(a));
  const uint64_t W = cam->width, H = cam->height, N = W * H;
  const int slot = 0;
  SMESH_TRY(main_after_raster(r));
  r->main_pending = true;
  if (r->fused[slot].bytes < N * 8) {
    SMESH_HIP(hipStreamSynchronize(ctx->raster_stream));
    SMESH_HIP(hipStreamSynchronize(ctx->stream));
    SMESH_TRY(r->fused[slot].reserve(N * 8));
  }
  uint32_t* d_idx = static_cast<uint32_t*>(r->fused[slot].ptr);
  r->last_idx[slot] = nullptr; r->rec_valid[slot] = false;
  const int tri_path = (label_bytes && labels_native(r, a, N)) ? kLabelsPlaneLevel : plane_optional_level(r, a);
  SMESH_TRY(render_into(r, cam, d_idx, nullptr, ctx->stream, slot, tri_path));
  SMESH_TRY(fuse_rendered(r, a, slot, d_idx, probs, weights, memkind, W, H, 0, 0, label_bytes));
  r->fused_seq++;
  return SMESH_OK;
}

int smesh_fuse_view(smesh_renderer_t* r, smesh_aggregator_t* a, const smesh_camera_t* cam, const float* probs,
                    const float* weights, int memkind) {
  return fuse_view_impl(r, a, cam, probs, weights, memkind, 0);
}

static int fuse_views_impl(smesh_renderer_t* r, smesh_aggregator_t* a, const smesh_camera_t* cams, uint64_t n,
                           const float* const* probs, const float* const* weights, int memkind, int label_bytes) {
  if (!r || !a || (n && (!cams || !probs))) return fail(SMESH_ERR_INVALID, "NULL argument");
  for (uint64_t i = 0; i < n; i++) {
    SMESH_TRY(check_camera(&cams[i]));
    if (!probs[i]) return fail(SMESH_ERR_INVALID, "NULL probs image");
  }
  DeviceCtx* ctx = r->ctx;
  if (smesh_aggregator_ctx(a) != ctx) return fail(SMESH_ERR_INVALID, "renderer and aggregator live on different devices");
  static const bool pairs_off = env_int("SMESH_FUSE_PAIRS", 1) == 0;
  bool pairable;
  int tri_path;
  {
    std::lock_guard<std::mutex> g2(smesh_aggregator_mutex(a));
    tri_path = plane_optional_level(r, a);
    pairable = !pairs_off && memkind == SMESH_MEM_DEVICE && !r->texels && r->F != 0 && smesh_aggregator_can_fuse_triangles(a, r->F) &&
               smesh_aggregator_can_fuse_pair(a);
    if (label_bytes) {
      tri_path = kLabelsPlaneLevel;
      pairable = !pairs_off && memkind == SMESH_MEM_DEVICE && r->F != 0;
    }
  }
  static const bool raster_pairs_off = env_int("SMESH_RASTER_PAIRS", 1) == 0;
  uint64_t i = 0;
  while (i < n) {
    int gn = (int)std::min<uint64_t>((uint64_t)kMaxGroup, n - i);
    bool grouped = !raster_pairs_off && memkind == SMESH_MEM_DEVICE && r->F != 0 && r->V != 0 && gn >= 2;
    for (int v = 0; v < gn && grouped; v++) grouped = queues_fit_group(cams[i + v].width, cams[i + v].height);
    if ((!pairable && !grouped) || i + 1 >= n) {
      SMESH_TRY(fuse_view_impl(r, a, &cams[i], probs[i], weights ? weights[i] : nullptr, memkind, label_bytes));
      i += 1;
      continue;
    }
    std::lock_guard<std::mutex> g(r->mu);
    std::lock_guard<std::mutex> g2(smesh_aggregator_mutex(a));
    std::lock_guard<std::recursive_mutex> lock(ctx->mu);
    SMESH_HIP(hipSetDevice(ctx->device));
    SMESH_TRY(smesh_aggregator_join_exchange(a));
    const bool group_pipeline_on = opt_group_pipeline();
    const bool use_pipeline = grouped && group_pipeline_on;
    if (!use_pipeline) {
      SMESH_TRY(main_after_raster(r));
      r->main_pending = true;
    }
    const bool group_pipeline = group_pipeline_on;
    int base = 0;
    if (use_pipeline) {
      const int bank = (int)(r->group_seq++ & 1u);
      base = bank * kMaxGroup;
      for (int b = 0; b < 2; b++) {
        if (!r->ev_bank_rendered[b]) SMESH_HIP(hipEventCreateWithFlags(&r->ev_bank_rendered[b], hipEventDisableTiming));
        if (!r->ev_bank_consumed[b]) SMESH_HIP(hipEventCreateWithFlags(&r->ev_bank_consumed[b], hipEventDisableTiming));
      }
      if (r->bank_used[bank]) SMESH_HIP(hipStreamWaitEvent(ctx->raster_stream, r->ev_bank_consumed[bank], 0));
      if (r->main_pending || !r->bank_used[bank]) {
        if (!r->ev_main_fence) SMESH_HIP(hipEventCreateWithFlags(&r->ev_main_fence, hipEventDisableTiming));
        SMESH_HIP(hipEventRecord(r->ev_main_fence, ctx->stream));
        SMESH_HIP(hipStreamWaitEvent(ctx->raster_stream, r->ev_main_fence, 0));
        r->main_pending = false;
      }
      if (!r->bank_used[bank ^ 1]) SMESH_TRY(prepare_group_slots(r, &cams[i], gn, ctx->raster_stream, (bank ^ 1) * kMaxGroup));
      SMESH_TRY(render_group_into(r, &cams[i], gn, ctx->raster_stream, base, -1, tri_path));
      SMESH_HIP(hipEventRecord(r->ev_bank_rendered[bank], ctx->raster_stream));
      SMESH_HIP(hipStreamWaitEvent(ctx->stream, r->ev_bank_rendered[bank], 0));
      r->bank_used[bank] = true;
      r->raster_pending = true;
    } else if (grouped) {
      SMESH_TRY(render_group_into(r, &cams[i], gn, ctx->stream, 0, -1, tri_path));
    } else {
      gn = 2;
      SMESH_HIP(alloc_side(r, 1));
      for (int v = 0; v < 2; v++) {
        const uint64_t N = (uint64_t)cams[i + v].width * cams[i + v].height;
        if (r->fused[v].bytes < N * 8) {
          SMESH_HIP(hipStreamSynchronize(ctx->stream));
          SMESH_TRY(r->fused[v].reserve(N * 8));
        }
        r->last_idx[v] = nullptr; r->rec_valid[v] = false;
        SMESH_TRY(render_into(r, &cams[i + v], static_cast<uint32_t*>(r->fused[v].ptr), nullptr, ctx->stream, v));
      }
    }
    static const bool texel_multi_off = env_int("SMESH_TEXEL_MULTI", 1) == 0;
    bool texel_multi = false;
    if (grouped && !pairable && r->texels && !texel_multi_off) texel_multi = smesh_aggregator_can_fuse_texels(a, r->num_primitives);
    if (texel_multi) {
      ProfScope fuse_region(ctx, SMESH_PROF_FUSE_SCATTER);
      RenderedView rv[kMaxGroup];
      for (int j = 0; j < gn; j++) {
        const smesh_renderer::Side& sd = r->side[base + j];
        const uint64_t k = i + (uint64_t)j;
        rv[j] = RenderedView{sd.frags, sd.big_queue, sd.big_count, static_cast<const uint32_t*>(r->fused[base + j].ptr), probs[k],
                             weights ? weights[k] : nullptr, cams[k].width, cams[k].height};
        rv[j].no_big = no_big_possible(r, &cams[k]);
        rv[j].kinds = sd.kinds;
      }
      SMESH_TRY(smesh_aggregator_fuse_texels_multi(a, r->F, r->tex_first, r->tex_res, r->big_capacity, rv, gn));
      smesh_note_fuse("k_fuse_texel", "render-records");
    }
    for (int j = 0; j < gn && !pairable && !texel_multi; j++) {
      const uint64_t k = i + (uint64_t)j;
      SMESH_TRY(fuse_rendered(r, a, base + j, static_cast<const uint32_t*>(r->fused[base + j].ptr), probs[k], weights ? weights[k] : nullptr,
                              SMESH_MEM_DEVICE, cams[k].width, cams[k].height, 0, 0, label_bytes));
    }
    if (pairable) {
      ProfScope fuse_region(ctx, SMESH_PROF_FUSE_SCATTER);
      static const int label_views_cap = std::max(1, env_int("SMESH_FUSE_VIEWS", 8));
      const int max_nv = label_bytes ? std::min(8, label_views_cap) : smesh_aggregator_max_fused_views(a);
      for (int j = 0; j < gn;) {
        int nv = 1;
        while (nv * 2 <= std::min(max_nv, gn - j)) nv *= 2;
        RenderedView rv[kMaxGroup];
        for (int v = 0; v < nv; v++) {
          const smesh_renderer::Side& sd = r->side[base + j + v];
          const uint64_t k = i + (uint64_t)(j + v);
          rv[v] = RenderedView{sd.frags, sd.big_queue, sd.big_count, static_cast<const uint32_t*>(r->fused[base + j + v].ptr), probs[k],
                               weights ? weights[k] : nullptr, cams[k].width, cams[k].height, 0, 0, true};
          rv[v].no_big = no_big_possible(r, &cams[k]);
          rv[v].fine = box_extent_bound(r->bounds, &cams[k]) <= 48.0;
          if (label_bytes) { rv[v].labels = probs[k]; rv[v].probs = nullptr; }
        }
        if (label_bytes) SMESH_TRY(smesh_labels_fuse_triangles(a, r->F, r->big_capacity, rv, nv, label_bytes));
        else SMESH_TRY(smesh_aggregator_fuse_triangles(a, r->F, r->prim_id, r->big_capacity, rv, nv));
        j += nv;
      }
    }
    if (pairable) smesh_note_fuse(label_bytes ? "k_fuse_tri_labels" : smesh_aggregator_fuse_kernel_name(a, r->prim_id != nullptr), "render-records");
    if (grouped && group_pipeline) SMESH_HIP(hipEventRecord(r->ev_bank_consumed[base / kMaxGroup], ctx->stream));
    r->fused_seq += (uint64_t)gn;
    i += (uint64_t)gn;
  }
  return SMESH_OK;
}

int smesh_fuse_views(smesh_renderer_t* r, smesh_aggregator_t* a, const smesh_camera_t* cams, uint64_t n,
                     const float* const* probs, const float* const* weights, int memkind) {
  return fuse_views_impl(r, a, cams, n, probs, weights, memkind, 0);
}

}

DeviceCtx* smesh_renderer_ctx(smesh_renderer* r) { return r->ctx; }

int smesh_renderer_fuse_views_labels(smesh_renderer* r, smesh_aggregator* a, const smesh_camera_t* cams, uint64_t n, const void* const* planes,
                                     const float* const* weights, int label_bytes) {
  bool native = true;
  {
    std::lock_guard<std::mutex> g2(smesh_aggregator_mutex(a));
    for (uint64_t i = 0; i < n; i++) native = native && labels_native(r, a, cams[i].width * cams[i].height);
  }
  const float* const* p = reinterpret_cast<const float* const*>(planes);
  if (native) return fuse_views_impl(r, a, cams, n, p, weights, SMESH_MEM_DEVICE, label_bytes);
  for (uint64_t i = 0; i < n; i++) SMESH_TRY(fuse_view_impl(r, a, &cams[i], p[i], weights ? weights[i] : nullptr, SMESH_MEM_DEVICE, label_bytes));
  return SMESH_OK;
}

int smesh_renderer_with_index_planes(smesh_renderer* r, const smesh_camera_t* cams, int n, uint64_t P, DeviceCtx* want_ctx,
                                     const std::function<int(int view, const uint32_t* idx, uint64_t W, uint64_t H)>& use) {
  if (!r || (n && !cams) || n < 0 || n > kMaxGroup) return fail(SMESH_ERR_INVALID, "bad argument");
  for (int v = 0; v < n; v++) SMESH_TRY(check_camera(&cams[v]));
  DeviceCtx* ctx = r->ctx;
  if (ctx != want_ctx) return fail(SMESH_ERR_INVALID, "confusion matrix and renderer live on different devices");
  if (P != r->num_primitives)
    return fail(SMESH_ERR_INVALID, "the label table has " + std::to_string(P) + " entries, the renderer " + std::to_string(r->num_primitives) + " primitives");
  if (n == 0) return SMESH_OK;
// ... 282 lines not shown
```

Before: 16400 views/s.

## Fuse vertex projection into rasterization via 256-triangle meshlets with LDS-staged vertices

Adds meshlet tables (per-block unique vertex lists, packed 10-bit local triangle indices and gathered vertex positions) built at renderer creation. When the raster mode is one-triangle-per-lane, a new group kernel projects each meshlet's vertices into shared memory and rasterizes from there, replacing the separate whole-mesh vertex projection pass and the screen-vertex buffer round trip. Paths that still need screen vertices (clipped, medium and huge queues) now project on the fly when the buffer is absent. The cost is redundant projection of vertices shared across meshlets, extra LDS use and reduced flexibility, since the triangles-per-wave and grouping heuristics are forced to fixed values.

```diff
diff --git a/include/smesh_meshlets.h b/include/smesh_meshlets.h
--- /dev/null
+++ b/include/smesh_meshlets.h
@@ -0,0 +1,22 @@
+#ifndef SMESH_MESHLETS_H
+#define SMESH_MESHLETS_H
+
+#include "smesh.h"
+
+#ifdef __cplusplus
+extern "C" {
+#endif
+
+#define SMESH_MESHLET_TRIS      256
+#define SMESH_MESHLET_MAX_VERTS 384
+
+int smesh_meshlets_build(const int32_t* faces, uint64_t F, uint64_t V, uint32_t* first, uint32_t* ids, uint64_t ids_capacity,
+                         uint32_t* tris, uint64_t* ids_used, int* has_meshlets);
+
+const char* smesh_last_raster_path(void);
+
+#ifdef __cplusplus
+}
+#endif
+
+#endif
diff --git a/semantic_meshes_amd/_lib.py b/semantic_meshes_amd/_lib.py
--- a/semantic_meshes_amd/_lib.py
+++ b/semantic_meshes_amd/_lib.py
@@ -111,6 +111,12 @@
     "smesh_memcpy": (c_int, [c_void_p, c_void_p, c_u64, c_int, c_int, c_int]),
 }
 
+MESHLET_SIGNATURES = {
+    "smesh_meshlets_build": (c_int, [c_void_p, c_u64, c_u64, c_void_p, c_void_p, c_u64, c_void_p, P(c_u64), P(c_int)]),
+    "smesh_last_raster_path": (ctypes.c_char_p, []),
+}
+MESHLET_TRIS, MESHLET_MAX_VERTS = 256, 384
+
 LBL_CODES = {"uint8": 0, "int8": 1, "uint16": 2, "int16": 3, "uint32": 4, "int32": 5, "uint64": 6, "int64": 7}
 
 VTX_SUMS, VTX_ANNOTATIONS = 0, 1
@@ -270,7 +276,7 @@
                         "(or `python -c 'import __graft_entry__ as g; g.build()'`). There is no CPU fallback." % LIB_PATH)
                 _preload_hip_runtime()
                 L = ctypes.CDLL(LIB_PATH)
-                for name, (res, args) in list(SIGNATURES.items()) + list(EXT_SIGNATURES.items()) + list(VERTEX_SIGNATURES.items()) + list(EVAL_SIGNATURES.items()) + list(LABEL_IMAGE_SIGNATURES.items()):
+                for name, (res, args) in list(SIGNATURES.items()) + list(EXT_SIGNATURES.items()) + list(VERTEX_SIGNATURES.items()) + list(EVAL_SIGNATURES.items()) + list(LABEL_IMAGE_SIGNATURES.items()) + list(MESHLET_SIGNATURES.items()):
                     fn = getattr(L, name)
                     fn.restype = res
                     fn.argtypes = args
@@ -311,6 +317,21 @@
     return lib().smesh_last_add_path().decode()
 
 
+def last_raster_path():
+    flush_pending()
+    return lib().smesh_last_raster_path().decode()
+
+
+def set_option(name, value):
+    check(lib().smesh_set_option(name.encode(), int(value)))
+
+
+def get_option(name):
+    v = ctypes.c_int64(0)
+    check(lib().smesh_get_option(name.encode(), ctypes.byref(v)))
+    return v.value
+
+
 def synchronize(device=0):
     flush_pending(device)
     check(lib().smesh_synchronize(device))
diff --git a/semantic_meshes_amd/csrc/common.hpp b/semantic_meshes_amd/csrc/common.hpp
--- a/semantic_meshes_amd/csrc/common.hpp
+++ b/semantic_meshes_amd/csrc/common.hpp
@@ -78,6 +78,8 @@
 void dev_cache_stats(uint64_t* live_blocks, uint64_t* cached_blocks, uint64_t* cached_bytes);
 
 bool opt_group_pipeline();
+constexpr int kRasterMeshletsDefault = 1;
+bool opt_raster_meshlets();
 bool opt_confusion_wave_aggregate();
 
 constexpr uint32_t kConfusionLdsMaxC = 180;
diff --git a/semantic_meshes_amd/csrc/context.cpp b/semantic_meshes_amd/csrc/context.cpp
--- a/semantic_meshes_amd/csrc/context.cpp
+++ b/semantic_meshes_amd/csrc/context.cpp
@@ -38,6 +38,17 @@
     const char* e = getenv("SMESH_GROUP_PIPELINE");
     v = e ? (atoi(e) != 0 ? 1 : 0) : 1;
     g_group_pipeline.store(v);
+  }
+  return v != 0;
+}
+
+static std::atomic<int> g_raster_meshlets{-1};
+bool opt_raster_meshlets() {
+  int v = g_raster_meshlets.load();
+  if (v < 0) {
+    const char* e = getenv("SMESH_RASTER_MESHLETS");
+    v = e ? (atoi(e) != 0 ? 1 : 0) : kRasterMeshletsDefault;
+    g_raster_meshlets.store(v);
   }
   return v != 0;
 }
@@ -292,12 +303,14 @@
 int smesh_set_option(const char* name, int64_t value) {
   if (!name) return fail(SMESH_ERR_INVALID, "option name is NULL");
   if (!strcmp(name, "group_pipeline")) { g_group_pipeline.store(value != 0 ? 1 : 0); return SMESH_OK; }
+  if (!strcmp(name, "raster_meshlets")) { g_raster_meshlets.store(value != 0 ? 1 : 0); return SMESH_OK; }
   if (!strcmp(name, "confusion_wave_aggregate")) { g_confusion_wave_aggregate.store(value != 0 ? 1 : 0); return SMESH_OK; }
   return fail(SMESH_ERR_INVALID, std::string("unknown option: ") + name);
 }
 int smesh_get_option(const char* name, int64_t* value) {
   if (!name || !value) return fail(SMESH_ERR_INVALID, "NULL argument");
   if (!strcmp(name, "group_pipeline")) { *value = opt_group_pipeline() ? 1 : 0; return SMESH_OK; }
+  if (!strcmp(name, "raster_meshlets")) { *value = opt_raster_meshlets() ? 1 : 0; return SMESH_OK; }
   if (!strcmp(name, "labels_lds_max_classes")) { *value = (int64_t)kLabelsLdsMaxC; return SMESH_OK; }
   if (!strcmp(name, "confusion_lds_max_classes")) { *value = (int64_t)kConfusionLdsMaxC; return SMESH_OK; }
   if (!strcmp(name, "confusion_wave_aggregate")) { *value = opt_confusion_wave_aggregate() ? 1 : 0; return SMESH_OK; }
diff --git a/semantic_meshes_amd/csrc/meshlets.cpp b/semantic_meshes_amd/csrc/meshlets.cpp
--- /dev/null
+++ b/semantic_meshes_amd/csrc/meshlets.cpp
@@ -0,0 +1,60 @@
+#include "meshlets.hpp"
+
+#include <algorithm>
+
+#include "../../include/smesh_meshlets.h"
+
+namespace smesh {
+
+static_assert(kMeshletMaxVerts <= (1u << kMeshletIndexBits), "a local index must fit its field of the packed word");
+static_assert(kMeshletTris == SMESH_MESHLET_TRIS && kMeshletMaxVerts == SMESH_MESHLET_MAX_VERTS, "the header documents these");
+
+bool build_meshlets(const int32_t* faces, uint64_t F, uint64_t V, MeshletTables& out) {
+  const uint64_t blocks = (F + kMeshletTris - 1) / kMeshletTris;
+  out.first.assign(blocks + 1, 0u);
+  out.ids.clear();
+  out.tris.assign(F, 0u);
+  uint32_t used[3 * kMeshletTris];
+  for (uint64_t b = 0; b < blocks; b++) {
+    const uint64_t f0 = b * kMeshletTris, f1 = std::min<uint64_t>(F, f0 + kMeshletTris);
+    const uint32_t n = (uint32_t)(3 * (f1 - f0));
+    for (uint32_t k = 0; k < n; k++) {
+      const int32_t i = faces[3 * f0 + k];
+      if (i < 0 || (uint64_t)i >= V) return false;
+      used[k] = (uint32_t)i;
+    }
+    std::sort(used, used + n);
+    const uint32_t count = (uint32_t)(std::unique(used, used + n) - used);
+    if (count > kMeshletMaxVerts) return false;
+    if (out.ids.size() + count > 0xFFFFFFFFull) return false;
+    for (uint64_t f = f0; f < f1; f++) {
+      uint32_t word = 0u;
+      for (int k = 0; k < 3; k++) {
+        const uint32_t local = (uint32_t)(std::lower_bound(used, used + count, (uint32_t)faces[3 * f + k]) - used);
+        word |= local << (kMeshletIndexBits * k);
+      }
+      out.tris[f] = word;
+    }
+    out.ids.insert(out.ids.end(), used, used + count);
+    out.first[b + 1] = (uint32_t)out.ids.size();
+  }
+  return true;
+}
+
+}
+
+extern "C" int smesh_meshlets_build(const int32_t* faces, uint64_t F, uint64_t V, uint32_t* first, uint32_t* ids, uint64_t ids_capacity,
+                                    uint32_t* tris, uint64_t* ids_used, int* has_meshlets) {
+  if (!has_meshlets || !ids_used || (F && (!faces || !tris)) || !first || (ids_capacity && !ids)) return SMESH_ERR_INVALID;
+  *has_meshlets = 0;
+  *ids_used = 0;
+  smesh::MeshletTables t;
+  if (!smesh::build_meshlets(faces, F, V, t)) return SMESH_OK;
+  if (t.ids.size() > ids_capacity) return SMESH_ERR_INVALID;
+  std::copy(t.first.begin(), t.first.end(), first);
+  std::copy(t.ids.begin(), t.ids.end(), ids);
+  std::copy(t.tris.begin(), t.tris.end(), tris);
+  *ids_used = t.ids.size();
+  *has_meshlets = 1;
+  return SMESH_OK;
+}
diff --git a/semantic_meshes_amd/csrc/meshlets.hpp b/semantic_meshes_amd/csrc/meshlets.hpp
--- /dev/null
+++ b/semantic_meshes_amd/csrc/meshlets.hpp
@@ -0,0 +1,20 @@
+#pragma once
+
+#include <cstdint>
+#include <vector>
+
+namespace smesh {
+
+constexpr uint32_t kMeshletTris = 256;
+constexpr uint32_t kMeshletMaxVerts = 384;
+constexpr uint32_t kMeshletIndexBits = 10;
+
+struct MeshletTables {
+  std::vector<uint32_t> first;
+  std::vector<uint32_t> ids;
+  std::vector<uint32_t> tris;
+};
+
+bool build_meshlets(const int32_t* faces, uint64_t F, uint64_t V, MeshletTables& out);
+
+}
diff --git a/semantic_meshes_amd/csrc/raster.hip b/semantic_meshes_amd/csrc/raster.hip
--- a/semantic_meshes_amd/csrc/raster.hip
+++ b/semantic_meshes_amd/csrc/raster.hip
@@ -1,4 +1,6 @@
 #include "common.hpp"
+#include "meshlets.hpp"
+#include "../../include/smesh_meshlets.h"
 
 #include <algorithm>
 #include <cmath>
@@ -250,6 +252,11 @@
 
 __device__ __forceinline__ uint64_t key_index(uint32_t x, uint32_t y, uint32_t H) { return (uint64_t)x * H + y; }
 
+__device__ __forceinline__ ScreenVertex screen_vertex(const RasterArgs& a, const int32_t i) {
+  if (a.sv) return a.sv[i];
+  return project_point(a.cam, a.verts[3 * (uint64_t)i + 0], a.verts[3 * (uint64_t)i + 1], a.verts[3 * (uint64_t)i + 2]);
+}
+
 __device__ __forceinline__ bool load_tri(const RasterArgs& a, uint64_t f, Tri& t, const int32_t i0, const int32_t i1, const int32_t i2);
 __device__ __forceinline__ bool load_tri(const RasterArgs& a, uint64_t f, Tri& t) {
   return load_tri(a, f, t, a.faces[3 * f + 0], a.faces[3 * f + 1], a.faces[3 * f + 2]);
@@ -257,7 +264,7 @@
 __device__ __forceinline__ bool load_tri(const RasterArgs& a, uint64_t f, Tri& t, const int32_t i0, const int32_t i1, const int32_t i2) {
   if ((uint64_t)max((uint32_t)i0, max((uint32_t)i1, (uint32_t)i2)) >= a.V) return false;
   if (a.tex_res && a.tex_res[f] == 0) return false;
-  const ScreenVertex va = a.sv[i0], vb = a.sv[i1], vc = a.sv[i2];
+  const ScreenVertex va = screen_vertex(a, i0), vb = screen_vertex(a, i1), vc = screen_vertex(a, i2);
   return setup_tri(va, vb, vc, a.W, a.H, t);
 }
 
@@ -346,7 +353,7 @@
   const int32_t i0 = a.faces[3 * f + 0], i1 = a.faces[3 * f + 1], i2 = a.faces[3 * f + 2];
   if ((uint64_t)max((uint32_t)i0, max((uint32_t)i1, (uint32_t)i2)) >= a.V) return false;
   if (a.tex_res && a.tex_res[f] == 0) return false;
-  const ScreenVertex va = a.sv[i0], vb = a.sv[i1], vc = a.sv[i2];
+  const ScreenVertex va = screen_vertex(a, i0), vb = screen_vertex(a, i1), vc = screen_vertex(a, i2);
   const int cls = clip_class(va, vb, vc);
   pc.clipped = cls > 0;
   if (cls < 0) return false;
@@ -385,14 +392,31 @@
   return ((unsigned long long)__float_as_uint(zf) << 32) | prim;
 }
 
+template <bool NULLABLE_SV = false>
 __device__ __forceinline__ int load_tri_ex(const RasterArgs& a, uint64_t f, Tri& t, const int32_t i0, const int32_t i1, const int32_t i2) {
   if ((uint64_t)max((uint32_t)i0, max((uint32_t)i1, (uint32_t)i2)) >= a.V) return 0;
   if (a.tex_res && a.tex_res[f] == 0) return 0;
-  const ScreenVertex va = a.sv[i0], vb = a.sv[i1], vc = a.sv[i2];
+  ScreenVertex va, vb, vc;
+  if constexpr (NULLABLE_SV) { va = screen_vertex(a, i0); vb = screen_vertex(a, i1); vc = screen_vertex(a, i2); }
+  else { va = a.sv[i0]; vb = a.sv[i1]; vc = a.sv[i2]; }
   const int cls = clip_class(va, vb, vc);
   if (cls == 0) return setup_tri(va, vb, vc, a.W, a.H, t) ? 1 : 0;
   if (cls < 0) return 0;
   return clip_bbox(a, i0, i1, i2, va, vb, vc, cls, t.x0, t.y0, t.x1, t.y1) ? 2 : 0;
+}
+
+struct MeshletTri {
+  ScreenVertex va, vb, vc;
+  const uint32_t* ids;
+  uint32_t l0, l1, l2;
+};
+__device__ __forceinline__ int load_tri_ml(const RasterArgs& a, uint64_t f, Tri& t, const MeshletTri& m) {
+  if (a.tex_res && a.tex_res[f] == 0) return 0;
+  const int cls = clip_class(m.va, m.vb, m.vc);
+  if (cls == 0) return setup_tri(m.va, m.vb, m.vc, a.W, a.H, t) ? 1 : 0;
+  if (cls < 0) return 0;
+  const int32_t i0 = (int32_t)m.ids[m.l0], i1 = (int32_t)m.ids[m.l1], i2 = (int32_t)m.ids[m.l2];
+  return clip_bbox(a, i0, i1, i2, m.va, m.vb, m.vc, cls, t.x0, t.y0, t.x1, t.y1) ? 2 : 0;
 }
 
 __device__ __forceinline__ unsigned long long shade_key(const RasterArgs& a, uint64_t f, const Tri& t, int x, int y) {
@@ -421,7 +445,7 @@
   TriFrag rec;
   rec.x0 = 0; rec.y0 = 0; rec.kind = 0; rec.pad = 0; rec.mask = 0ull;
   Tri t;
-  const int have = load_tri_ex(a, f, t, a.faces[3 * f + 0], a.faces[3 * f + 1], a.faces[3 * f + 2]);
+  const int have = load_tri_ex<>(a, f, t, a.faces[3 * f + 0], a.faces[3 * f + 1], a.faces[3 * f + 2]);
   if (have) {
     const int bw = t.x1 - t.x0 + 1, bh = t.y1 - t.y0 + 1;
     rec.x0 = (uint16_t)t.x0; rec.y0 = (uint16_t)t.y0;
@@ -662,9 +686,10 @@
     }
 }
 
-template <int MODE>
+template <int MODE, bool ML = false, bool NULLABLE_SV = false>
 __device__ __forceinline__ void raster_frag_64(const RasterArgs& a, const uint64_t f, const int32_t i0, const int32_t i1, const int32_t i2,
-                                               const uint32_t sub, const int part_in = -1, const bool listed = false) {
+                                               const uint32_t sub, const int part_in = -1, const bool listed = false,
+                                               const MeshletTri* ml = nullptr) {
   constexpr bool kWgPush = (MODE & 1) != 0, kSpreadMode = (MODE & 2) != 0, kTex = (MODE & 4) != 0;
   const int lane = threadIdx.x & 63;
   const int part = kSpreadMode ? part_in : -1;
@@ -678,7 +703,9 @@
   bool medium = false, lanebox = false, small = false;
   bool q_big = false, q_mid = false, q_huge = false;
   const uint32_t pid = (a.prim_id && f < a.F) ? a.prim_id[f] : (uint32_t)f;
-  const int have = f < a.F ? load_tri_ex(a, f, t, i0, i1, i2) : 0;
+  int have = 0;
+  if constexpr (ML) { if (f < a.F) have = load_tri_ml(a, f, t, *ml); }
+  else { if (f < a.F) have = load_tri_ex<NULLABLE_SV>(a, f, t, i0, i1, i2); }
   if (have) {
     const int bw = t.x1 - t.x0 + 1, bh = t.y1 - t.y0 + 1;
     rec.x0 = (uint16_t)t.x0; rec.y0 = (uint16_t)t.y0;
@@ -822,7 +849,7 @@
     if (g >= a.F) continue;
     const int32_t g0 = a.faces[3 * (uint64_t)g + 0], g1 = a.faces[3 * (uint64_t)g + 1], g2 = a.faces[3 * (uint64_t)g + 2];
     Tri t;
-    if (load_tri_ex(a, g, t, g0, g1, g2) != 1) continue;
+    if (load_tri_ex<true>(a, g, t, g0, g1, g2) != 1) continue;
     uint32_t rb[6] = {0u, 0u, 0u, 0u, 0u, 0u};
     if (lane == 0) coop_reserve(a, t, i & (kQSub - 1), rb);
     coop_walk<TEX>(a, t, rb, 0, g, a.prim_id ? a.prim_id[g] : g, i & (kQSub - 1));
@@ -837,7 +864,7 @@
     if (tri < kTris && e < nl) fs = a.med_queue[a.big_capacity - 1u - e];
     int32_t s0 = 0, s1 = 0, s2 = 0;
     if (fs < a.F) { s0 = a.faces[3 * fs + 0]; s1 = a.faces[3 * fs + 1]; s2 = a.faces[3 * fs + 2]; }
-    raster_frag_64<TEX ? 6 : 2>(a, fs, s0, s1, s2, i & (kQSub - 1), lane % kLanes, true);
+    raster_frag_64<TEX ? 6 : 2, false, true>(a, fs, s0, s1, s2, i & (kQSub - 1), lane % kLanes, true);
   }
 }
 template <bool TEX>
@@ -891,6 +918,10 @@
   uint32_t tile_end[kMaxGroup];
   uint32_t n, blocks_per_view;
   uint32_t chunk;
+  const uint32_t* ml_first;
+  const uint32_t* ml_ids;
+  const float* ml_pos;
+  const uint32_t* ml_tris;
 };
 template <int MODE>
 __global__ __launch_bounds__(256) __attribute__((amdgpu_waves_per_eu((MODE & 3) ? 4 : 5, 5))) void k_raster_frag_group(RasterGroup g) {
@@ -905,6 +936,54 @@
     tb = blockIdx.x - v * g.blocks_per_view;
   }
   raster_frag_wave<true, MODE>(g.view[v], ((uint64_t)tb * blockDim.x + threadIdx.x) >> 6);
+}
+template <int MODE>
+__global__ __launch_bounds__(256) __attribute__((amdgpu_waves_per_eu(5, 5))) void k_raster_frag_group_ml(RasterGroup g) {
+  static_assert((MODE & 3) == 0, "one triangle per lane only");
+  __shared__ double s_u[kMeshletMaxVerts], s_v[kMeshletMaxVerts], s_iz[kMeshletMaxVerts];
+  uint32_t v, tb;
+  if (g.chunk) {
+    const uint32_t k = blockIdx.x >> 3, sq = k / g.n;
+    v = k - sq * g.n;
+    tb = xcd_block(blockIdx.x & 7u, sq, g.chunk);
+    if (tb >= g.blocks_per_view) return;
+  } else {
+    v = blockIdx.x / g.blocks_per_view;
+    tb = blockIdx.x - v * g.blocks_per_view;
+  }
+  const RasterArgs& a = g.view[v];
+  const uint32_t id0 = g.ml_first[tb];
+  const uint32_t nv = min(g.ml_first[tb + 1] - id0, kMeshletMaxVerts);
+  const uint32_t* __restrict__ ids = g.ml_ids + id0;
+  const float* __restrict__ pos = g.ml_pos + 3u * (uint64_t)id0;
+  for (uint32_t i = threadIdx.x; i < nv; i += 256u) {
+    const ScreenVertex s = project_point(a.cam, pos[3u * i + 0u], pos[3u * i + 1u], pos[3u * i + 2u]);
+    s_u[i] = s.u; s_v[i] = s.v; s_iz[i] = s.iz;
+  }
+  __syncthreads();
+  const uint64_t f = (uint64_t)tb * 256u + threadIdx.x;
+  MeshletTri m;
+  m.ids = ids;
+  m.l0 = 0u; m.l1 = 0u; m.l2 = 0u;
+  if (f < a.F) {
+    const uint32_t w = g.ml_tris[f];
+    constexpr uint32_t kMask = (1u << kMeshletIndexBits) - 1u;
+    m.l0 = min(w & kMask, kMeshletMaxVerts - 1u); m.l1 = min((w >> kMeshletIndexBits) & kMask, kMeshletMaxVerts - 1u);
+    m.l2 = min((w >> (2u * kMeshletIndexBits)) & kMask, kMeshletMaxVerts - 1u);
+  }
+  m.va.u = s_u[m.l0]; m.va.v = s_v[m.l0]; m.va.iz = s_iz[m.l0];
+  m.vb.u = s_u[m.l1]; m.vb.v = s_v[m.l1]; m.vb.iz = s_iz[m.l1];
+  m.vc.u = s_u[m.l2]; m.vc.v = s_v[m.l2]; m.vc.iz = s_iz[m.l2];
+  const uint64_t wave_id = ((uint64_t)tb * 256u + threadIdx.x) >> 6;
+  raster_frag_64<MODE, true>(a, f < a.F ? f : a.F, 0, 0, 0, (uint32_t)wave_id & (kQSub - 1), -1, false, &m);
+}
+struct CountGroup {
+  uint32_t* big_count[kMaxGroup];
+  uint32_t n;
+};
+__global__ void k_reset_big_counts(CountGroup g) {
+  const uint32_t v = threadIdx.x / 6u, k = threadIdx.x - v * 6u;
+  if (v < g.n) g.big_count[v][k] = 0u;
 }
 template <bool TEX>
 __global__ __launch_bounds__(256) void k_raster_medium_group(RasterGroup g, uint32_t blocks_per_view) {
@@ -1178,6 +1257,7 @@
   int32_t* faces = nullptr;
   struct Bounds { bool valid = false; double lo[3] = {0, 0, 0}, hi[3] = {0, 0, 0}, max_edge = 0, mean_edge = 0; } bounds;
   uint32_t* prim_id = nullptr;
+  struct Meshlets { uint32_t* first = nullptr; uint32_t* ids = nullptr; uint32_t* tris = nullptr; float* pos = nullptr; } ml;
   struct ViewScratch {
     ScreenVertex* sv = nullptr;
     uint32_t* huge_queue = nullptr;
@@ -1487,11 +1567,12 @@
 }
 
 hipError_t alloc_side(smesh_renderer* r, int i);
-
-hipError_t alloc_scratch(smesh_renderer* r, int i) {
+thread_local const char* g_last_raster_path = "none";
+
+hipError_t alloc_scratch(smesh_renderer* r, int i, bool need_sv) {
   smesh_renderer::ViewScratch& vs = r->vs[i];
   hipError_t e = hipSuccess;
-  if (!vs.sv) e = dev_malloc(reinterpret_cast<void**>(&vs.sv), std::max<uint64_t>(r->V * sizeof(ScreenVertex), 16));
+  if (!vs.sv && need_sv) e = dev_malloc(reinterpret_cast<void**>(&vs.sv), std::max<uint64_t>(r->V * sizeof(ScreenVertex), 16));
   if (e == hipSuccess && !vs.huge_queue) e = dev_malloc(reinterpret_cast<void**>(&vs.huge_queue), (size_t)r->big_capacity * 4);
   if (e == hipSuccess && !vs.med_queue) e = dev_malloc(reinterpret_cast<void**>(&vs.med_queue), (size_t)r->big_capacity * 4);
   return e;
@@ -1509,7 +1590,7 @@
   for (int v = 0; v < n; v++) {
     const uint64_t W = cams[v].width, H = cams[v].height, N = W * H;
     SMESH_HIP(alloc_side(r, base + v));
-    SMESH_HIP(alloc_scratch(r, base + v));
+    SMESH_HIP(alloc_scratch(r, base + v, !(r->ml.tris && opt_raster_meshlets())));
     smesh_renderer::ViewScratch& vs = r->vs[base + v];
     SMESH_TRY(ensure_keys(vs, W, H, st));
     int qs = SMESH_OK;
@@ -1536,7 +1617,7 @@
   for (int v = 0; v < n; v++) {
     const uint64_t W = cams[v].width, H = cams[v].height, N = W * H;
     SMESH_HIP(alloc_side(r, side_base + v));
-    SMESH_HIP(alloc_scratch(r, base + v));
+    SMESH_HIP(alloc_scratch(r, base + v,  false));
     smesh_renderer::ViewScratch& vs = r->vs[base + v];
     SMESH_TRY(ensure_keys(vs, W, H, st));
     int qs = SMESH_OK;
@@ -1575,14 +1656,39 @@
     for (int v = 0; v < n; v++) rg.view[v].balance = 2 * balance_votes >= n && balance_votes > 0 ? (n > 1 ? 1u : 2u) : 0u;
   }
   for (int v = 0; v < n; v++) rg.view[v].groups = frag_groups(r->F, n, rg.view[0].tpw);
+  const int mode = raster_mode(rg.view[0]);
+  const bool meshlets = (mode & 3) == 0 && r->ml.tris != nullptr && opt_raster_meshlets();
+  if (meshlets) {
+    for (int v = 0; v < n; v++) { rg.view[v].tpw = 64u; rg.view[v].groups = 1u; rg.view[v].sv = nullptr; }
+    rg.ml_first = r->ml.first; rg.ml_ids = r->ml.ids; rg.ml_tris = r->ml.tris; rg.ml_pos = r->ml.pos;
+  } else {
+    for (int v = 0; v < n; v++) {
+      SMESH_HIP(alloc_scratch(r, base + v, true));
+      pg.sv[v] = r->vs[base + v].sv;
+      rg.view[v].sv = r->vs[base + v].sv;
+    }
+  }
+  g_last_raster_path = meshlets ? "meshlets" : "vertex-stage";
   rg.blocks_per_view = (uint32_t)div_up(div_up(r->F, rg.view[0].tpw * rg.view[0].groups), 4);
   ProfScope prof(ctx, SMESH_PROF_RASTER, st);
-  hipLaunchKernelGGL(k_project_vertices_group, dim3((uint32_t)div_up(r->V, 256)), dim3(256), 0, st, pg);
+  if (meshlets) {
+    CountGroup cg;
+    memset(&cg, 0, sizeof cg);
+    for (int v = 0; v < n; v++) cg.big_count[v] = pg.big_count[v];
+    cg.n = (uint32_t)n;
+    hipLaunchKernelGGL(k_reset_big_counts, dim3(1), dim3(64), 0, st, cg);
+  } else {
+    hipLaunchKernelGGL(k_project_vertices_group, dim3((uint32_t)div_up(r->V, 256)), dim3(256), 0, st, pg);
+  }
   SMESH_HIP(hipGetLastError());
   {
     rg.chunk = rg.blocks_per_view >= 64u ? kRasterXcdRun : 0u;
     const dim3 grid(rg.chunk ? 8u * xcd_slots(rg.blocks_per_view, rg.chunk) * (uint32_t)n : (uint32_t)n * rg.blocks_per_view);
-    switch (raster_mode(rg.view[0])) {
+    if (meshlets) {
+      if (mode & 4) hipLaunchKernelGGL(k_raster_frag_group_ml<4>, grid, dim3(256), 0, st, rg);
+      else hipLaunchKernelGGL(k_raster_frag_group_ml<0>, grid, dim3(256), 0, st, rg);
+    } else
+    switch (mode) {
       case 7:  hipLaunchKernelGGL(k_raster_frag_group<7>, grid, dim3(256), 0, st, rg); break;
       case 5:  hipLaunchKernelGGL(k_raster_frag_group<5>, grid, dim3(256), 0, st, rg); break;
       case 4:  hipLaunchKernelGGL(k_raster_frag_group<4>, grid, dim3(256), 0, st, rg); break;
@@ -1737,6 +1843,21 @@
   if (e == hipSuccess) e = dev_malloc(reinterpret_cast<void**>(&r->vs[0].med_queue), (size_t)r->big_capacity * 4);
   if (e == hipSuccess && V) e = hipMemcpyAsync(r->verts, vertices, V * 12, hipMemcpyHostToDevice, ctx->stream);
   if (e == hipSuccess && F) e = hipMemcpyAsync(r->faces, faces, F * 12, hipMemcpyHostToDevice, ctx->stream);
+  MeshletTables mt;
+  std::vector<float> ml_pos;
+  if (e == hipSuccess && F && V && build_meshlets(faces, F, V, mt)) {
+    e = dev_malloc(reinterpret_cast<void**>(&r->ml.first), mt.first.size() * 4);
+    if (e == hipSuccess) e = dev_malloc(reinterpret_cast<void**>(&r->ml.ids), std::max<uint64_t>(mt.ids.size() * 4, 16));
+    if (e == hipSuccess) e = dev_malloc(reinterpret_cast<void**>(&r->ml.tris), mt.tris.size() * 4);
+    if (e == hipSuccess) e = hipMemcpyAsync(r->ml.first, mt.first.data(), mt.first.size() * 4, hipMemcpyHostToDevice, ctx->stream);
+    if (e == hipSuccess && !mt.ids.empty()) e = hipMemcpyAsync(r->ml.ids, mt.ids.data(), mt.ids.size() * 4, hipMemcpyHostToDevice, ctx->stream);
+    if (e == hipSuccess) e = hipMemcpyAsync(r->ml.tris, mt.tris.data(), mt.tris.size() * 4, hipMemcpyHostToDevice, ctx->stream);
+    ml_pos.resize(3 * mt.ids.size());
+    for (size_t k = 0; k < mt.ids.size(); k++)
+      for (int d = 0; d < 3; d++) ml_pos[3 * k + d] = vertices[3 * (uint64_t)mt.ids[k] + d];
+    if (e == hipSuccess) e = dev_malloc(reinterpret_cast<void**>(&r->ml.pos), std::max<uint64_t>(ml_pos.size() * 4, 16));
+    if (e == hipSuccess && !ml_pos.empty()) e = hipMemcpyAsync(r->ml.pos, ml_pos.data(), ml_pos.size() * 4, hipMemcpyHostToDevice, ctx->stream);
+  }
   if (e == hipSuccess) e = hipStreamSynchronize(ctx->stream);
   if (e != hipSuccess) {
     smesh_renderer_destroy(r);
@@ -1863,6 +1984,7 @@
 
 const char* smesh_last_fuse_kernel(void) { return g_last_fuse_kernel; }
 const char* smesh_last_add_path(void) { return g_last_add_path; }
+const char* smesh_last_raster_path(void) { return g_last_raster_path; }
 
 int smesh_renderer_create_triangles(const float* vertices, uint64_t V, const int32_t* faces, uint64_t F, int device,
                                     smesh_renderer_t** out) {
@@ -1976,7 +2098,7 @@
   (void)hipSetDevice(r->ctx->device);
   (void)hipStreamSynchronize(r->ctx->raster_stream);
   (void)hipStreamSynchronize(r->ctx->stream);
-  for (void* p : {(void*)r->prim_id, (void*)r->verts, (void*)r->faces, (void*)r->tex_res, (void*)r->tex_first})
+  for (void* p : {(void*)r->prim_id, (void*)r->verts, (void*)r->faces, (void*)r->tex_res, (void*)r->tex_first, (void*)r->ml.first, (void*)r->ml.ids, (void*)r->ml.tris, (void*)r->ml.pos})
     if (p) (void)dev_free(p);
   for (auto& sd : r->side)
     for (void* p : {(void*)sd.big_queue, (void*)sd.big_count, (void*)sd.frags, (void*)sd.kinds})
```

Result: faster. 17460 views/s (median of 6 runs) (+6.5%).
